# calad0i/da4ml

Measured on AMD Instinct MI355X. Metric: CMVM solves/sec, 256x256 int8 matrix, higher is better.
Workload: dtype u32; 1 GPU; c3_256x256_int8_batch64_single_chain; matrix=256x256 int8 (default_rng(seed).integers(-128,128)), batch_per_gpu=64, parallelism=1 x independent-instance shard, no data-path collective

## Files before the change

da4ml_amd/_binary/__init__.py:

```python

from __future__ import annotations

import ctypes as C
from pathlib import Path
from types import SimpleNamespace

import numpy as np

from .._marshal import pipeline_from_stages, stage_from_arrays

import os as _os

_LIB_PATH = Path(_os.environ['DA4ML_HIP_LIB']).resolve() if _os.environ.get('DA4ML_HIP_LIB') else Path(__file__).resolve().parent.parent / 'libda4ml_hip.so'
_lib = None

_f32p = np.ctypeslib.ndpointer(np.float32, flags='C_CONTIGUOUS')
_i64p = np.ctypeslib.ndpointer(np.int64, flags='C_CONTIGUOUS')
_i32p = np.ctypeslib.ndpointer(np.int32, flags='C_CONTIGUOUS')

EXPORTS = (
    'da_last_error da_last_error_code da_version da_device_count da_set_device da_get_lsb_loc da_iceil_log2 da_cost_add da_int_arr_to_csd '
    'da_csd_decompose da_kernel_decompose da_solve da_solve_batch da_solve_sharded da_rccl_unique_id da_rccl_shutdown da_solve_sharded_rccl da_comm_abort da_shard_exchanged_elements da_n_stages da_picked da_stage_info da_stage_copy '
    'da_result_stats da_free da_timings da_engine_stats da_dais_run da_dais_last_error da_dais_run_on'
).split()
# ... 60 lines not shown
        L.da_shard_exchanged_elements.restype = C.c_int64
        L.da_shard_exchanged_elements.argtypes = []
    L.da_solve_sharded_rccl.restype = C.c_void_p
    L.da_solve_sharded_rccl.argtypes = [_f32p, C.c_int64, C.c_int64, C.c_char_p, C.c_char_p, C.c_int, C.c_int, C.c_void_p, C.c_void_p, C.c_int, C.c_int, C.c_int,
                                        C.c_int, C.c_int, C.c_char_p, _i64p]
    L.da_timings.argtypes = [np.ctypeslib.ndpointer(np.float64, flags='C_CONTIGUOUS'), C.c_int]
    L.da_engine_stats.argtypes = [np.ctypeslib.ndpointer(np.float64, flags='C_CONTIGUOUS'), C.c_int]
    _lib = L
    return L


def _raise(rc: int):
    msg = lib().da_last_error().decode()
    if rc == -2:
        raise ValueError(msg)
    raise RuntimeError(msg)


def _kernel(kernel) -> np.ndarray:
    if not isinstance(kernel, np.ndarray) or kernel.dtype != np.float32:
        raise TypeError('kernel must be a numpy.ndarray of dtype float32 (no implicit conversion)')
    return np.ascontiguousarray(kernel)


def device_count() -> int:
    return int(lib().da_device_count())


def set_device(device: int) -> None:
    if lib().da_set_device(int(device)) != 0:
        _raise(-1)


def get_lsb_loc(x: float) -> int:
    return int(lib().da_get_lsb_loc(float(x)))


def iceil_log2(x: float) -> int:
    return int(lib().da_iceil_log2(float(x)))


def cost_add(q0, q1, shift: int, sub: bool, adder_size: int, carry_size: int) -> tuple[float, float]:
    out = np.zeros(2, np.float32)
    lib().da_cost_add(np.asarray(q0, np.float32), np.asarray(q1, np.float32), int(shift), int(bool(sub)), int(adder_size), int(carry_size), out)
    return float(out[0]), float(out[1])


def int_arr_to_csd(inp) -> np.ndarray:
    if not isinstance(inp, np.ndarray) or inp.dtype != np.int32:
        raise TypeError('inp must be a numpy.ndarray of dtype int32 (no implicit conversion)')
    x = np.ascontiguousarray(inp)
    N = lib().da_int_arr_to_csd(x.ravel(), x.size, None)
    if N < 0:
        _raise(N)
    out = np.zeros(x.shape + (N,), np.int8)
    rc = lib().da_int_arr_to_csd(x.ravel(), x.size, out.ctypes.data)
    if rc < 0:
        _raise(rc)
    return out


def csd_decompose(inp, center: bool = True):
    k = _kernel(inp)
    if k.ndim != 2:
        raise RuntimeError('csd_decompose only supports 2D arrays.')
    n_in, n_out = k.shape
    N = lib().da_csd_decompose(k, n_in, n_out, int(center), None, None, None)
    if N < 0:
        _raise(N)
    csd = np.zeros((n_in, n_out, N), np.int8)
    s0, s1 = np.zeros(n_in, np.int8), np.zeros(n_out, np.int8)
    rc = lib().da_csd_decompose(k, n_in, n_out, int(center), csd.ctypes.data, s0.ctypes.data, s1.ctypes.data)
    if rc < 0:
        _raise(rc)
    return csd, s0, s1


def kernel_decompose(kernel, dc: int = -2):
    k = _kernel(kernel)
    if k.ndim != 2:
        raise RuntimeError('csd_decompose only supports 2D arrays.')
    n_in, n_out = k.shape
    m0, m1 = np.zeros((n_in, n_out), np.float32), np.zeros((n_out, n_out), np.float32)
    rc = lib().da_kernel_decompose(k, n_in, n_out, int(dc), m0, m1)
    if rc < 0:
        _raise(rc)
    return m0, m1


def _collect(h, with_stats=False):
    L = lib()
    try:
        stages = []
        for s in range(L.da_n_stages(h)):
            info = np.zeros(5, np.int64)
            L.da_stage_info(h, s, info)
            n_in, n_out, n_ops, carry, adder = (int(v) for v in info)
            arr = [np.zeros(n, np.int64) for n in (n_in, n_out, n_out, n_out)]
            oi, of = np.zeros((n_ops, 4), np.int64), np.zeros((n_ops, 5), np.float32)
            L.da_stage_copy(h, s, *arr, oi, of)
            stages.append(stage_from_arrays(n_in, n_out, *arr, oi, of, carry, adder))
        pipe = pipeline_from_stages(stages)
        if not with_stats:
            return pipe
        st = np.zeros(8, np.int64)
        L.da_result_stats(h, st)
        names = ('iterations', 'digits0', 'blocks0', 'select_rounds', 'table_peak', 'scan_slots', 'partners', 'matches')
        return pipe, dict(zip(names, st.tolist()), picked=int(L.da_picked(h)))
    finally:
        L.da_free(h)


def _opt_arrays(qintervals, latencies, n_in):
    q = l = None
    if qintervals is not None:
        q = np.ascontiguousarray(np.asarray([tuple(float(v) for v in t) for t in qintervals], np.float32).reshape(n_in, 3))
    if latencies is not None:
        l = np.ascontiguousarray(np.asarray([float(v) for v in latencies], np.float32).reshape(n_in))
    return q, l


def solve(
    kernel,
    method0: str = 'wmc',
    method1: str = 'auto',
    hard_dc: int = -1,
    decompose_dc: int = -2,
    qintervals=None,
    latencies=None,
    adder_size: int = -1,
    carry_size: int = -1,
    search_all_decompose_dc: bool = True,
    _stats: bool = False,
):
    k = _kernel(kernel)
    if k.ndim != 2:
        raise RuntimeError('csd_decompose only supports 2D arrays.')
    n_in, n_out = k.shape
    q, l = _opt_arrays(qintervals, latencies, n_in)
    h = lib().da_solve(k, n_in, n_out, method0.encode(), method1.encode(), int(hard_dc), int(decompose_dc),
                       None if q is None else q.ctypes.data, None if l is None else l.ctypes.data,
                       int(adder_size), int(carry_size), int(bool(search_all_decompose_dc)))
    if not h:
        _raise(lib().da_last_error_code())
    return _collect(h, _stats)


def solve_sharded(kernel, method0: str = 'wmc', method1: str = 'auto', hard_dc: int = -1, decompose_dc: int = -2, qintervals=None, latencies=None,
                  adder_size: int = -1, carry_size: int = -1, search_all_decompose_dc: bool = True, rank: int = 0, world: int = 1, allreduce=None):
    k = _kernel(kernel)
    if k.ndim != 2:
        raise RuntimeError('csd_decompose only supports 2D arrays.')
    n_in, n_out = k.shape
    q, l = _opt_arrays(qintervals, latencies, n_in)
    st = np.zeros(3, np.int64)
    h = lib().da_solve_sharded(k, n_in, n_out, method0.encode(), method1.encode(), int(hard_dc), int(decompose_dc),
                               None if q is None else q.ctypes.data, None if l is None else l.ctypes.data, int(adder_size), int(carry_size),
                               int(bool(search_all_decompose_dc)), int(rank), int(world), C.cast(allreduce, C.c_void_p) if allreduce is not None else None, None, st)
    if not h:
        _raise(lib().da_last_error_code())
    return _collect(h), dict(zip(('sharded_chains', 'greedy_steps', 'allreduce_calls'), st.tolist()))


def rccl_unique_id() -> bytes:
    buf = C.create_string_buffer(128)
    rc = lib().da_rccl_unique_id(buf)
    if rc != 0:
        _raise(rc)
    return buf.raw


def rccl_shutdown() -> int:
    n = lib().da_rccl_shutdown()
    if n < 0:
        _raise(1)
    return n


def solve_sharded_rccl(kernel, unique_id: bytes, method0: str = 'wmc', method1: str = 'auto', hard_dc: int = -1, decompose_dc: int = -2, qintervals=None,
                       latencies=None, adder_size: int = -1, carry_size: int = -1, search_all_decompose_dc: bool = True, rank: int = 0, world: int = 1):
    k = _kernel(kernel)
    if k.ndim != 2:
        raise RuntimeError('csd_decompose only supports 2D arrays.')
    if len(unique_id) != 128:
        raise ValueError('unique_id must be the 128 bytes of rccl_unique_id()')
    n_in, n_out = k.shape
    q, l = _opt_arrays(qintervals, latencies, n_in)
    st = np.zeros(3, np.int64)
    h = lib().da_solve_sharded_rccl(k, n_in, n_out, method0.encode(), method1.encode(), int(hard_dc), int(decompose_dc),
                                    None if q is None else q.ctypes.data, None if l is None else l.ctypes.data, int(adder_size), int(carry_size),
                                    int(bool(search_all_decompose_dc)), int(rank), int(world), unique_id, st)
    if not h:
        _raise(lib().da_last_error_code())
    return _collect(h), dict(zip(('sharded_chains', 'greedy_steps', 'allreduce_calls'), st.tolist()))


def shard_exchanged_elements() -> int:
    return int(lib().da_shard_exchanged_elements())


def comm_abort():
    lib().da_comm_abort()


def solve_many(
    kernels,
    method0: str = 'wmc',
    method1: str = 'auto',
    hard_dc: int = -1,
    decompose_dc: int = -2,
    qintervals=None,
    latencies=None,
    adder_size: int = -1,
    carry_size: int = -1,
    search_all_decompose_dc: bool = True,
    _stats: bool = False,
):
    ks = [_kernel(k) for k in kernels]
    n = len(ks)
    if n == 0:
        return []
    n_in = np.array([k.shape[0] for k in ks], np.int64)
    n_out = np.array([k.shape[1] for k in ks], np.int64)
    kptr = (C.c_void_p * n)(*[k.ctypes.data for k in ks])
    keep, qptr, lptr = [], None, None
    if qintervals is not None or latencies is not None:
        qs, ls = [], []
        for i in range(n):
            q, l = _opt_arrays(None if qintervals is None else qintervals[i], None if latencies is None else latencies[i], int(n_in[i]))
            keep += [q, l]
            qs.append(None if q is None else q.ctypes.data)
            ls.append(None if l is None else l.ctypes.data)
        qptr, lptr = (C.c_void_p * n)(*qs), (C.c_void_p * n)(*ls)
    res = (C.c_void_p * n)()
    rc = lib().da_solve_batch(n, kptr, n_in, n_out, method0.encode(), method1.encode(), int(hard_dc), int(decompose_dc), qptr, lptr,
                              int(adder_size), int(carry_size), int(bool(search_all_decompose_dc)), res)
    if rc != 0:
        _raise(rc)
    return [_collect(res[i], _stats) for i in range(n)]


class RawBatch:

    def __init__(self, handles):
        self.handles = list(handles)

    def __len__(self):
        return len(self.handles)

    def summary(self, i: int) -> dict:
        L, h = lib(), self.handles[i]
        cost, adders, n_ops = 0.0, 0, []
        for s in range(L.da_n_stages(h)):
            info = np.zeros(5, np.int64)
            L.da_stage_info(h, s, info)
            n_in, n_out, n = int(info[0]), int(info[1]), int(info[2])
            arr = [np.zeros(k, np.int64) for k in (n_in, n_out, n_out, n_out)]
            oi, of = np.zeros((n, 4), np.int64), np.zeros((n, 5), np.float32)
            L.da_stage_copy(h, s, *arr, oi, of)
            cost += float(of[:, 4].astype(np.float64).sum())
            adders += int(np.isin(oi[:, 2], (0, 1)).sum())
            n_ops.append(n)
        st = np.zeros(8, np.int64)
        L.da_result_stats(h, st)
        return dict(cost=cost, adders=adders, n_ops=n_ops, iterations=int(st[0]))

    def pipeline(self, i: int):
        h, self.handles[i] = self.handles[i], None
        return _collect(h)

    def free(self):
        for h in self.handles:
            if h:
                lib().da_free(h)
        self.handles = []


def solve_many_raw(kernels, method0='wmc', method1='auto', hard_dc=-1, decompose_dc=-2, adder_size=-1, carry_size=-1,
                   search_all_decompose_dc=True) -> RawBatch:
    ks = [_kernel(k) for k in kernels]
    n = len(ks)
    n_in = np.array([k.shape[0] for k in ks], np.int64)
    n_out = np.array([k.shape[1] for k in ks], np.int64)
    kptr = (C.c_void_p * n)(*[k.ctypes.data for k in ks])
    res = (C.c_void_p * n)()
    rc = lib().da_solve_batch(n, kptr, n_in, n_out, method0.encode(), method1.encode(), int(hard_dc), int(decompose_dc), None, None,
                              int(adder_size), int(carry_size), int(bool(search_all_decompose_dc)), res)
    if rc != 0:
        _raise(rc)
    return RawBatch([res[i] for i in range(n)])


def timings(reset: bool = False) -> dict:
    t = np.zeros(32, np.float64)
    e = np.zeros(16, np.float64)
    lib().da_engine_stats(e, 16)
    rc = lib().da_timings(t, int(reset))
    if rc != 0:
        _raise(rc)
    names = ('loop_ms', 'dist_ms', 'total_ms', 'lockstep_iters', 'iterations', 'rescans', 'partners', 'chains', 'table_bytes', 'arena_bytes',
             'select_ms_sampled', 'update_ms_sampled', 'samples', 'found', 'inserts', 'cell_reads', 'block_bytes', 'cell_bytes',
             'sel_load_bounds', 'sel_argmax', 'sel_newrow', 'sel_substitute', 'sel_prefix', 'sel_claims', 'sel_special',
             'upd_fetch', 'upd_probe', 'upd_cells', 'upd_blocks', 'upd_create', 'retries', 'sampled_chain_launches')
    extra = ('select_bytes', 'host_launch_ms', 'fast_steps', 'search_bounds', 'search_argmax', 'search_excluded', 'search_steps_timed', 'search_stale_rereads', 'search_touch_rereads', 'search_rounds', 'search_long_lists', 'search_longest_list', 'search_full_passes', 'search_list_entries')
    return {**dict(zip(names, t.tolist())), **dict(zip(extra, e.tolist()))}


_DAIS_EXECUTORS = {'host': 0, 'cpu': 0, 'device': 1, 'gpu': 1, 'host-scalar': 2}


def dais_interp_run(bin_logic, data, n_threads: int = 1, executor: str = 'host'):
    prog = np.ascontiguousarray(np.ravel(bin_logic), dtype=np.int32)
    if prog.size < 4:
        raise RuntimeError('Invalid binary logic data')
    n_in, n_out = int(prog[2]), int(prog[3])
    x = np.ascontiguousarray(np.ravel(data), dtype=np.float64)
    assert n_in > 0 and x.size % n_in == 0, f'Input size {x.size} is not divisible by {n_in}'
    n_samples = x.size // n_in
    out = np.zeros((n_samples, max(n_out, 0)), dtype=np.float64)
    L = lib()
    L.da_dais_run_on.argtypes = [C.c_void_p, C.c_int64, C.c_void_p, C.c_int64, C.c_void_p, C.c_int, C.c_int]
    L.da_dais_last_error.restype = C.c_char_p
    if executor not in _DAIS_EXECUTORS:
        raise ValueError(f'unknown DAIS executor {executor!r} (one of {sorted(_DAIS_EXECUTORS)})')
    if L.da_dais_run_on(prog.ctypes.data, prog.size, x.ctypes.data, n_samples, out.ctypes.data, int(n_threads), _DAIS_EXECUTORS[executor]) != 0:
        raise RuntimeError(L.da_dais_last_error().decode())
    return out


cmvm_bin = SimpleNamespace(
    solve=solve, kernel_decompose=kernel_decompose, csd_decompose=csd_decompose, int_arr_to_csd=int_arr_to_csd,
    get_lsb_loc=get_lsb_loc, iceil_log2=iceil_log2, cost_add=cost_add,
)

__all__ = ['dais_interp_run', 'int_arr_to_csd', 'csd_decompose', 'get_lsb_loc', 'kernel_decompose', 'solve', 'iceil_log2', 'solve_many', 'cost_add']
```

da4ml_amd/csrc/cmvm_capi.cc:

```cpp

#include <cstdlib>
#include <chrono>
#include <cstdio>
#include <pthread.h>

#include <algorithm>
#include <atomic>
#include <cstring>
#include <memory>
#include <mutex>
#include <new>
#include <string>
#include <vector>

#include "../../include/da4ml_hip.h"
#include "cmvm_gpu.h"
#include "cmvm_host.h"
#include "cmvm_rccl.h"
#include "cmvm_shard.h"

namespace {

thread_local std::string g_err;
thread_local int g_err_code = DA_OK;
// ... 67 lines not shown
    }
}

}

struct da_result {
    da::PipeResult pipe;
    da::ChainStats stats;
};

extern "C" {

const char *da_last_error(void) { return g_err.c_str(); }
int da_last_error_code(void) { return g_err_code; }
const char *da_version(void) { return "da4ml_hip 0.1 (gfx950)"; }
int da_device_count(void) { return da::gpu::device_count(); }
int da_set_device(int device) {
    std::lock_guard<LibraryMutex> lk(g_mutex);
    if (device < 0 || device >= da::gpu::device_count()) {
        g_err = "invalid device index " + std::to_string(device);
        return g_err_code = DA_ERR_NO_DEVICE;
    }
    g_device = device;
    return DA_OK;
}

int da_get_lsb_loc(float x) { return da::lsb_loc(x); }
int da_iceil_log2(float x) { return da::iceil_log2(x); }
int da_cost_add(const float *q0, const float *q1, int64_t shift, int sub, int adder_size, int carry_size, float *out2) {
    da::cost_add(da::QInt{q0[0], q0[1], q0[2]}, da::QInt{q1[0], q1[1], q1[2]}, shift, sub != 0, adder_size, carry_size, out2[0], out2[1]);
    return DA_OK;
}

int da_int_arr_to_csd(const int32_t *x, int64_t n, int8_t *out) {
    std::lock_guard<LibraryMutex> lk(g_mutex);
    try {
        std::vector<int8_t> csd;
        int N = backend().int_to_csd(x, n, csd);
        if (out) std::memcpy(out, csd.data(), csd.size());
        return N;
    } catch (const std::exception &e) {
        return fail(e);
    }
}

int da_csd_decompose(const float *kernel, int64_t n_in, int64_t n_out, int center, int8_t *csd, int8_t *shift0, int8_t *shift1) {
    std::lock_guard<LibraryMutex> lk(g_mutex);
    try {
        std::vector<int8_t> c, a, b;
        int N = backend().csd_decompose(kernel, (int)n_in, (int)n_out, center != 0, c, a, b);
        if (csd) std::memcpy(csd, c.data(), c.size());
        if (shift0) std::memcpy(shift0, a.data(), a.size());
        if (shift1) std::memcpy(shift1, b.data(), b.size());
        return N;
    } catch (const std::exception &e) {
        return fail(e);
    }
}

int da_kernel_decompose(const float *kernel, int64_t n_in, int64_t n_out, int dc, float *m0, float *m1) {
    std::lock_guard<LibraryMutex> lk(g_mutex);
    try {
        std::vector<float> a, b;
        da::kernel_decompose(backend(), kernel, (int)n_in, (int)n_out, dc, a, b);
        std::memcpy(m0, a.data(), a.size() * 4);
        std::memcpy(m1, b.data(), b.size() * 4);
        return DA_OK;
    } catch (const std::exception &e) {
        return fail(e);
    }
}

int da_solve_batch(int count, const float *const *kernels, const int64_t *n_in, const int64_t *n_out, const char *method0,
                   const char *method1, int hard_dc, int decompose_dc, const float *const *qintervals,
                   const float *const *latencies, int adder_size, int carry_size, int search_all_decompose_dc,
                   da_result **results) {
    std::lock_guard<LibraryMutex> lk(g_mutex);
    try {
        std::vector<da::Problem> probs((size_t)count);
        for (int i = 0; i < count; ++i) {
            da::Problem &p = probs[i];
            p.kernel = kernels[i];
            p.n_in = (int)n_in[i];
            p.n_out = (int)n_out[i];
            if (p.n_in <= 0 || p.n_out <= 0) throw std::invalid_argument("kernel must be a non-empty 2-D matrix");
            p.opt.method0 = method0;
            p.opt.method1 = method1;
            p.opt.hard_dc = hard_dc;
            p.opt.decompose_dc = decompose_dc;
            const float *q = qintervals ? qintervals[i] : nullptr;
            const float *l = latencies ? latencies[i] : nullptr;
            check_dyadic_steps(q, p.n_in);
            if (q)
                for (int r = 0; r < p.n_in; ++r) p.opt.qints.push_back(da::QInt{q[3 * r], q[3 * r + 1], q[3 * r + 2]});
            if (l) p.opt.lats.assign(l, l + p.n_in);
            p.opt.adder_size = adder_size;
            p.opt.carry_size = carry_size;
            p.opt.search_all = search_all_decompose_dc != 0;
        }
        std::vector<da::ChainStats> stats;
        const auto t0 = std::chrono::steady_clock::now();
        std::vector<da::PipeResult> res = da::solve_batch(backend(), probs, &stats);
        for (int i = 0; i < count; ++i) results[i] = new da_result{std::move(res[i]), i < (int)stats.size() ? stats[i] : da::ChainStats{}};
        if (std::getenv("DA4ML_HIP_VERBOSE"))
            std::fprintf(stderr, "[da4ml_hip] da_solve_batch(%d): %.2f ms\n", count, std::chrono::duration<double, std::milli>(std::chrono::steady_clock::now() - t0).count());
        return DA_OK;
    } catch (const std::exception &e) {
        return fail(e);
    }
}

da_result *da_solve(const float *kernel, int64_t n_in, int64_t n_out, const char *method0, const char *method1, int hard_dc,
                    int decompose_dc, const float *qintervals, const float *latencies, int adder_size, int carry_size,
                    int search_all_decompose_dc) {
    da_result *r = nullptr;
    const float *q[1] = {qintervals}, *l[1] = {latencies};
    int rc = da_solve_batch(1, &kernel, &n_in, &n_out, method0, method1, hard_dc, decompose_dc, qintervals ? q : nullptr,
                            latencies ? l : nullptr, adder_size, carry_size, search_all_decompose_dc, &r);
    return rc == DA_OK ? r : nullptr;
}

static std::atomic<int> g_comm_aborted{0};
void da_comm_abort(void) { g_comm_aborted.store(1); }
static std::atomic<long long> g_shard_elements{0};
int64_t da_shard_exchanged_elements(void) { return (int64_t)g_shard_elements.load(); }

static std::unique_ptr<da::ShardEngine> make_hip_shard(const da::ChainJob &job, int c0, int c1, double capacity_scale, void *ctx) {
    return static_cast<da::gpu::HipBackend *>(ctx)->make_shard_engine(job, c0, c1, capacity_scale);
}

static da_result *solve_sharded_impl(const float *kernel, int64_t n_in, int64_t n_out, const char *method0, const char *method1, int hard_dc,
                                     int decompose_dc, const float *qintervals, const float *latencies, int adder_size, int carry_size,
                                     int search_all_decompose_dc, int rank, int world, da_allreduce_i32 allreduce, void *ctx, int64_t *stats3,
                                     bool stream_ordered);

static void rccl_allreduce_cb(void *ctx, void *buf, int64_t count, int on_device) {
    if (!static_cast<da::gpu::RcclTransport *>(ctx)->allreduce(buf, count, on_device != 0)) g_comm_aborted.store(1);
}

int da_rccl_unique_id(void *id128) {
    try {
        if (!id128) throw std::invalid_argument("id128 must point to 128 bytes");
        da::gpu::rccl_unique_id(id128);
        return DA_OK;
    } catch (const std::exception &e) {
        return fail(e);
    }
}

int da_rccl_shutdown(void) {
    std::lock_guard<LibraryMutex> lk(g_mutex);
    try {
        return da::gpu::rccl_shutdown();
    } catch (const std::exception &e) {
        fail(e);
        return -1;
    }
}

da_result *da_solve_sharded_rccl(const float *kernel, int64_t n_in, int64_t n_out, const char *method0, const char *method1, int hard_dc,
                                 int decompose_dc, const float *qintervals, const float *latencies, int adder_size, int carry_size,
                                 int search_all_decompose_dc, int rank, int world, const void *id128, int64_t *stats3) {
    std::shared_ptr<da::gpu::RcclTransport> tr;
    {
        std::lock_guard<LibraryMutex> lk(g_mutex);
        try {
            if (world < 1 || rank < 0 || rank >= world) throw std::invalid_argument("rank must be in [0, world)");
            if (!id128) throw std::invalid_argument("id128 (the 128-byte RCCL unique id of rank 0) must be given");
            da::gpu::HipBackend &inner = backend();
            tr = da::gpu::RcclTransport::open(id128, rank, world, g_device, inner.stream());
        } catch (const std::exception &e) {
            fail(e);
            return nullptr;
        }
    }
    da_result *r = solve_sharded_impl(kernel, n_in, n_out, method0, method1, hard_dc, decompose_dc, qintervals, latencies, adder_size, carry_size,
                                      search_all_decompose_dc, rank, world, rccl_allreduce_cb, tr.get(), stats3, true);
    if (!r && tr->last_error()[0]) g_err += std::string(" [") + tr->last_error() + "]";
    return r;
}

static da_result *solve_sharded_impl(const float *kernel, int64_t n_in, int64_t n_out, const char *method0, const char *method1, int hard_dc,
                                     int decompose_dc, const float *qintervals, const float *latencies, int adder_size, int carry_size,
                                     int search_all_decompose_dc, int rank, int world, da_allreduce_i32 allreduce, void *ctx, int64_t *stats3,
                                     bool stream_ordered) {
    std::lock_guard<LibraryMutex> lk(g_mutex);
    try {
        if (world < 1 || rank < 0 || rank >= world) throw std::invalid_argument("rank must be in [0, world)");
        if (world > 255) throw std::invalid_argument("at most 255 ranks (8-bit flag fields)");
        if (world > 1 && !allreduce) throw std::invalid_argument("an all-reduce callback must be given for world > 1");
        if (n_in <= 0 || n_out <= 0) throw std::invalid_argument("kernel must be a non-empty 2-D matrix");
        da::Problem p;
        p.kernel = kernel;
        p.n_in = (int)n_in;
        p.n_out = (int)n_out;
        p.opt.method0 = method0;
        p.opt.method1 = method1;
        p.opt.hard_dc = hard_dc;
        p.opt.decompose_dc = decompose_dc;
        check_dyadic_steps(qintervals, p.n_in);
        if (qintervals)
            for (int r = 0; r < p.n_in; ++r) p.opt.qints.push_back(da::QInt{qintervals[3 * r], qintervals[3 * r + 1], qintervals[3 * r + 2]});
        if (latencies) p.opt.lats.assign(latencies, latencies + p.n_in);
        p.opt.adder_size = adder_size;
        p.opt.carry_size = carry_size;
        p.opt.search_all = search_all_decompose_dc != 0;
        da::gpu::HipBackend &inner = backend();
        da::ShardComm comm;
        comm.rank = rank;
        comm.world = world;
        comm.allreduce = allreduce;
        comm.ctx = ctx;
        g_comm_aborted.store(0);
        comm.aborted = &g_comm_aborted;
        comm.stream_ordered = stream_ordered || std::getenv("DA4ML_SHARD_STREAM_ORDERED") != nullptr;
        da::ShardedBackend be(inner, comm, make_hip_shard, &inner);
        be.force_single = std::getenv("DA4ML_SHARD_FORCE") != nullptr;
        be.force_comm(std::getenv("DA4ML_SHARD_FORCE_COMM") != nullptr);
        std::vector<da::ChainStats> stats;
        std::vector<da::PipeResult> res = da::solve_batch(be, {p}, &stats);
        if (stats3) {
            stats3[0] = be.sharded_chains;
            stats3[1] = be.sharded_steps;
            stats3[2] = be.comm().calls;
        }
        g_shard_elements.store(be.comm().elements);
        return new da_result{std::move(res[0]), stats.empty() ? da::ChainStats{} : stats[0]};
    } catch (const std::exception &e) {
        fail(e);
        return nullptr;
    }
}

da_result *da_solve_sharded(const float *kernel, int64_t n_in, int64_t n_out, const char *method0, const char *method1, int hard_dc,
                            int decompose_dc, const float *qintervals, const float *latencies, int adder_size, int carry_size,
                            int search_all_decompose_dc, int rank, int world, da_allreduce_i32 allreduce, void *ctx, int64_t *stats3) {
    return solve_sharded_impl(kernel, n_in, n_out, method0, method1, hard_dc, decompose_dc, qintervals, latencies, adder_size, carry_size,
                              search_all_decompose_dc, rank, world, allreduce, ctx, stats3, false);
}

int da_n_stages(const da_result *r) { return (int)r->pipe.stages.size(); }
int da_picked(const da_result *r) { return r->pipe.picked; }
int da_stage_info(const da_result *r, int stage, int64_t *info) {
    const da::StageResult &s = r->pipe.stages[stage];
    info[0] = s.n_in;
    info[1] = s.n_out;
    info[2] = (int64_t)s.ops.size();
    info[3] = s.carry_size;
    info[4] = s.adder_size;
    return DA_OK;
}
int da_stage_copy(const da_result *r, int stage, int64_t *inp_shifts, int64_t *out_idxs, int64_t *out_shifts, int64_t *out_negs,
                  int64_t *ops_i, float *ops_f) {
    const da::StageResult &s = r->pipe.stages[stage];
    std::memcpy(inp_shifts, s.inp_shifts.data(), s.inp_shifts.size() * 8);
    std::memcpy(out_idxs, s.out_idxs.data(), s.out_idxs.size() * 8);
    std::memcpy(out_shifts, s.out_shifts.data(), s.out_shifts.size() * 8);
    std::memcpy(out_negs, s.out_negs.data(), s.out_negs.size() * 8);
    for (size_t k = 0; k < s.ops.size(); ++k) {
        const da::OpRec &o = s.ops[k];
        int64_t *oi = ops_i + 4 * k;
        float *of = ops_f + 5 * k;
        oi[0] = o.id0, oi[1] = o.id1, oi[2] = o.opcode, oi[3] = o.data;
        of[0] = o.q.lo, of[1] = o.q.hi, of[2] = o.q.step, of[3] = o.latency, of[4] = o.cost;
    }
    return DA_OK;
}
int da_result_stats(const da_result *r, int64_t *s) {
    const da::ChainStats &t = r->stats;
    int64_t v[8] = {t.iterations, t.digits0, t.blocks0, t.rebuilds, t.table_peak, t.scan_slots, t.partners, t.matches};
    std::memcpy(s, v, sizeof v);
    return DA_OK;
}
void da_free(da_result *r) {
    if (!r) return;
    for (da::StageResult &st : r->pipe.stages) da::recycle_op_list(std::move(st.ops));
    delete r;
}

int da_timings(double *t, int reset) {
    std::lock_guard<LibraryMutex> lk(g_mutex);
    try {
        da::gpu::HipBackend &be = backend();
        const da::gpu::GpuTimings &g = be.timings();
        double v[32] = {g.loop_ms,          g.dist_ms,         g.total_ms,         (double)g.lockstep_iters, (double)g.iterations,
                        (double)g.rescans, (double)g.partners, (double)g.chains, g.table_bytes,            g.arena_bytes,
                        g.select_ms_sampled, g.update_ms_sampled, (double)g.samples, (double)g.found, (double)g.inserts,
                        (double)g.cell_reads, g.key_bytes, g.cell_bytes};
        for (int q = 0; q < 12; ++q) v[18 + q] = g.phase_cycles[q];
        v[30] = (double)g.retries;
        v[31] = g.sampled_chain_launches;
        std::memcpy(t, v, sizeof v);
        if (reset) be.reset_timings();
        return DA_OK;
    } catch (const std::exception &e) {
        return fail(e);
    }
}

int da_engine_stats(double *out, int n) {
    std::lock_guard<LibraryMutex> lk(g_mutex);
    try {
        const da::gpu::GpuTimings &g = backend().timings();
        const double v[16] = {g.select_bytes, g.host_launch_ms, (double)g.fast_steps, g.search_cycles[0], g.search_cycles[1], g.search_cycles[2], g.search_cycles[3], g.search_diag[0], g.search_diag[1], g.search_diag[2], g.search_diag[3], g.search_diag[4], g.search_diag[5], g.search_diag[6], 0.0, 0.0};
        const int m = n < 16 ? (n < 0 ? 0 : n) : 16;
        for (int i = 0; i < m; ++i) out[i] = v[i];
        return m;
    } catch (const std::exception &e) {
        fail(e);
        return 0;
    }
}

}
```

da4ml_amd/csrc/cmvm_engine.hip:

```cpp

#include <hip/hip_runtime.h>

#include <algorithm>
#include <atomic>
#include <chrono>
#include <cmath>
#include <cstdio>
#include <cstdlib>
#include <cstring>
#include <memory>
#include <mutex>
#include <numeric>
#include <stdexcept>
#include <string>
#include <thread>
#include <vector>

#include "cmvm_core.h"
#include "cmvm_geometry.h"
#include "cmvm_gpu.h"
#include "cmvm_host.h"

namespace da {
namespace gpu {

#define HIP_CHECK(expr)                                                                                          \
    do {                                                                                                         \
        hipError_t _e = (expr);                                                                                  \
        if (_e != hipSuccess)                                                                                    \
            throw std::runtime_error(std::string("HIP error: ") + hipGetErrorString(_e) + " at " #expr);         \
    } while (0)

constexpr uint64_t KEY_EMPTY = ~0ull;
constexpr uint64_t KEY_TOMB = ~0ull - 1;
constexpr uint64_t KEY_TOMB_LO = KEY_TOMB - 3;
constexpr int WAVE = 64;
constexpr int UPD_THREADS = 256;
constexpr int UPD_WAVES = UPD_THREADS / WAVE;
#ifndef DA_MAX_GROUPS
#define DA_MAX_GROUPS 2048
#endif
constexpr int MAX_GROUPS = DA_MAX_GROUPS;
#ifndef DA_IDS_LDS
#define DA_IDS_LDS 2048
#endif

#ifdef DA_PHASE_TIMERS
#define UPD_TIMER_DECL long long up[5] = {0, 0, 0, 0, 0}, u0 = clock64(), u1;
#define UPD_TIMER_MARK(i) \
    u1 = clock64();       \
    up[i] += u1 - u0;     \
    u0 = u1;
#ifndef DA_TIMER_STEP_LO
#define DA_TIMER_STEP_LO 0
#endif
#ifndef DA_TIMER_STEP_HI
#define DA_TIMER_STEP_HI 0x7FFFFFFF
#endif
#define DA_TIMED_STEP(t) ((t) >= DA_TIMER_STEP_LO && (t) < DA_TIMER_STEP_HI)
#define UPD_TIMER_FLUSH \
    if (lane == 0 && DA_TIMED_STEP(g->iter - 1))      \
        for (int q = 0; q < 5; ++q) atomicAdd(&g->st_phase[7 + q], (unsigned long long)up[q]);
#define SEL_TIMER_DECL long long tp[8];
#define SEL_TIMER_MARK(i) tp[i] = clock64();
#define SEL_TIMER_FLUSH \
    if (DA_TIMED_STEP(iter)) for (int q = 0; q < 7; ++q) g->st_phase[q] += (unsigned long long)(tp[q + 1] - tp[q]);
#define UPD_TIMER_PASS_END UPD_TIMER_MARK(4)
#elif defined(DA_UPD_TAIL)
#ifndef DA_TIMER_STEP_LO
#define DA_TIMER_STEP_LO 0
#endif
#ifndef DA_TIMER_STEP_HI
#define DA_TIMER_STEP_HI 0x7FFFFFFF
#endif
#define DA_TIMED_STEP(t) ((t) >= DA_TIMER_STEP_LO && (t) < DA_TIMER_STEP_HI)
#define UPD_TIMER_DECL long long up[9] = {0, 0, 0, 0, 0, 0, 0, 0, 0}, u0 = clock64(), u1;
#define UPD_TIMER_MARK(i)
#define UPD_TIMER_PASS_END                                                        \
    {                                                                             \
        u1 = clock64();                                                           \
        const long long dt = u1 - u0;                                             \
        const bool cr = __ballot(gnew) != 0;                                      \
        up[0] += dt, up[1] += 1;                                                  \
        if (rare) up[2] += dt, up[3] += 1, up[8] += __popcll(rare);               \
        if (!rare && cr) up[4] += 1, up[5] += dt;                                 \
        up[6] += dt > 20000, up[7] += dt > 40000;                                 \
        u0 = clock64();                                                           \
    }
#define UPD_TIMER_FLUSH                                                           \
    if (lane == 0 && DA_TIMED_STEP(g->iter - 1)) {                                \
        for (int q = 0; q < 5; ++q) atomicAdd(&g->st_phase[7 + q], (unsigned long long)up[q]); \
        atomicAdd(&g->st_qdiag[0], (unsigned long long)up[5]);                    \
        atomicAdd(&g->st_qdiag[1], (unsigned long long)up[6]);                    \
        atomicAdd(&g->st_qdiag[4], (unsigned long long)up[7]);                    \
        atomicAdd(&g->st_qdiag[5], (unsigned long long)up[8]);                    \
    }
#define SEL_TIMER_DECL
#define SEL_TIMER_MARK(i)
#define SEL_TIMER_FLUSH
#else
#define UPD_TIMER_DECL
#define UPD_TIMER_MARK(i)
#define UPD_TIMER_PASS_END
#define UPD_TIMER_FLUSH
#define SEL_TIMER_DECL
#define SEL_TIMER_MARK(i)
#define SEL_TIMER_FLUSH
#endif

#ifdef DA_STEP_CLOCKS
#define CLK_NOW() ((unsigned long long)__builtin_amdgcn_s_memrealtime())
#define CLK_MARK(g, par, slot, inverted) atomicMax(&(g)->clk[par][slot], (inverted) ? ~CLK_NOW() : CLK_NOW())
#ifndef DA_CLK_STEP_LO
#define DA_CLK_STEP_LO 0
#endif
#ifndef DA_CLK_STEP_HI
#define DA_CLK_STEP_HI 0x7FFFFFFF
#endif
#define CLK_TIMED_STEP(t) ((t) >= DA_CLK_STEP_LO && (t) < DA_CLK_STEP_HI)
#else
#define CLK_MARK(g, par, slot, inverted)
#endif

struct BlkHdr {
    int ov;
    float dl;
    uint32_t rank;
    uint32_t idx;
};

#define DA_GLOBAL __attribute__((address_space(1)))
template <class T> __device__ __forceinline__ T *gen(DA_GLOBAL T *p) { return (T *)p; }
template <class T> __device__ __forceinline__ T da_uniform(T v) {
    static_assert(sizeof(T) == 4 || sizeof(T) == 8, "pinned descriptor fields are 32- or 64-bit values");
    if constexpr (sizeof(T) == 4) {
        const int r = __builtin_amdgcn_readfirstlane(__builtin_bit_cast(int, v));
        return __builtin_bit_cast(T, r);
    } else {
        const unsigned long long u = __builtin_bit_cast(unsigned long long, v);
        const unsigned int lo = (unsigned int)__builtin_amdgcn_readfirstlane((int)(unsigned int)u), hi = (unsigned int)__builtin_amdgcn_readfirstlane((int)(unsigned int)(u >> 32));
        return __builtin_bit_cast(T, ((unsigned long long)hi << 32) | lo);
    }
}
#define DA_PIN_ASM(x) do { x = da_uniform(x); asm volatile("" : "+s"(x)); } while (0)
template <class T> __device__ __forceinline__ void pin_one(T &v) { DA_PIN_ASM(v); }
template <class... T> __device__ __forceinline__ void pin_sgpr(T &...v) { (pin_one(v), ...); }
#define DA_PIN_VASM(x) asm volatile("" : "+v"(x))
template <class T> __device__ __forceinline__ void pin_vone(T &v) { DA_PIN_VASM(v); }
template <class... T> __device__ __forceinline__ void pin_vgpr(T &...v) { (pin_vone(v), ...); }
__device__ __forceinline__ void load_fence() {
    asm volatile("" ::: "memory");
    __builtin_amdgcn_sched_barrier(0);
}
__host__ __device__ __forceinline__ size_t align16(size_t v) { return (v + 15) & ~(size_t)15; }
typedef float da_f4 __attribute__((ext_vector_type(4)));
typedef int da_i4 __attribute__((ext_vector_type(4)));
typedef unsigned int da_u2 __attribute__((ext_vector_type(2)));
typedef unsigned long long da_ul2 __attribute__((ext_vector_type(2)));
__device__ __forceinline__ RowInfo load_row(const DA_GLOBAL RowInfo *rows, size_t i) {
    const da_f4 v = *reinterpret_cast<const DA_GLOBAL da_f4 *>(rows + i);
    return RowInfo{v.x, v.y, v.z, v.w};
}
__device__ __forceinline__ RowInfo pick_row(bool first, const RowInfo &a, const RowInfo &b) {
    return RowInfo{first ? a.lo : b.lo, first ? a.hi : b.hi, first ? a.step : b.step, first ? a.lat : b.lat};
}
__device__ __forceinline__ void store_row(DA_GLOBAL RowInfo *rows, size_t i, const RowInfo &r) {
    *reinterpret_cast<DA_GLOBAL da_f4 *>(rows + i) = da_f4{r.lo, r.hi, r.step, r.lat};
}

template <class Cell> struct RowFmt;
template <> struct RowFmt<uint32_t> {
    using Entry = uint32_t;
    static __device__ __forceinline__ Entry pack(uint32_t col, uint32_t cell) { return (col << 24) | ((cell >> 16) << 12) | (cell & 0xFFFu); }
    static __device__ __forceinline__ uint32_t col(Entry e) { return e >> 24; }
    static __device__ __forceinline__ uint32_t cell(Entry e) { return (((e >> 12) & 0xFFFu) << 16) | (e & 0xFFFu); }
    static __device__ __forceinline__ Entry none() { return 0u; }
};
template <> struct RowFmt<uint64_t> {
    using Entry = da_ul2;
    static __device__ __forceinline__ Entry pack(uint32_t col, uint64_t cell) { return Entry{(unsigned long long)cell, (unsigned long long)col}; }
    static __device__ __forceinline__ uint32_t col(Entry e) { return (uint32_t)e.y; }
    static __device__ __forceinline__ uint64_t cell(Entry e) { return (uint64_t)e.x; }
    static __device__ __forceinline__ Entry none() { return Entry{0ull, 0ull}; }
};
constexpr int REF_ROW_BITS = 24, REF_LEN_BITS = 12, REF_OFF_BITS = 28;
__host__ __device__ __forceinline__ unsigned long long ref_pack(uint32_t row, uint32_t len, uint32_t off) {
    return (unsigned long long)row | ((unsigned long long)len << REF_ROW_BITS) | ((unsigned long long)off << (REF_ROW_BITS + REF_LEN_BITS));
}
__device__ __forceinline__ uint32_t ref_row(unsigned long long r) { return (uint32_t)r & ((1u << REF_ROW_BITS) - 1u); }
__device__ __forceinline__ uint32_t ref_len(unsigned long long r) { return (uint32_t)(r >> REF_ROW_BITS) & ((1u << REF_LEN_BITS) - 1u); }
__device__ __forceinline__ uint32_t ref_off(unsigned long long r) { return (uint32_t)(r >> (REF_ROW_BITS + REF_LEN_BITS)); }

struct SpecPick {
    unsigned long long word;
    unsigned long long tie;
    da_u2 refA, refB;
    RowInfo ra, rb;
};
static_assert(sizeof(SpecPick) == 64, "SpecPick is read as sixteen words");
struct CandEntry {
    unsigned long long rank, tie;
};
#ifndef DA_CAND_CAP
#define DA_CAND_CAP 16
#endif
constexpr int CAND_CAP = DA_CAND_CAP, TOUCH_CAP = DA_CAND_CAP;

struct alignas(32) GroupRec {
    unsigned long long ub;
    unsigned long long glow;
    unsigned long long gtie;
    uint32_t dirty;
    uint32_t pad;
};
static_assert(sizeof(GroupRec) == 32, "group record");
struct ChainDev {
    int n_in, n_out, n_bits, K, Kpad, method, adder_size, carry_size;
    int rcap, lcap, gs_log2, n_groups;
    uint32_t C, cmask;
    const float *kernel;
    const float *qints;
    const float *lats;
    int32_t *xint;
    int8_t *shift0, *shift1;
    void *rlist;
    da_u2 *rowoff;
    uint32_t rl_cap, rl_used;
    RowInfo *rows;
    uint32_t *stamp;
    unsigned long long *collist;
    int *collen;
    unsigned long long *hkey;
    uint32_t *hrank;
    unsigned char *hblk;
    int pb_log2;
    GroupRec *grec;
    int *mcol;
    uint16_t *cmap;
    uint32_t *colbits;
    int cb_words;
    uint32_t *pl_ids;
    void *mA, *mB;
    unsigned long long *plist;
    int m, n_partners;
    int claim_words;
    uint32_t A, B, Nw;
    int pk_shift, pk_sub;
    int n_rows, iter, done, error, unknown_hit;
    unsigned int n_live, n_used, live_peak;
    int4 *picks;
    int prep_nbits, prep_maxdcol;
    long long prep_digits, prep_pairs;
    uint32_t *fin_row;
    unsigned long long *fin_cell;
    uint32_t *fin_count;
    uint32_t *fin_start;
    uint32_t *pk_row;
    unsigned long long *pk_cell;
    float *pk_lat;
    int pk_cap;
    uint32_t pk_total;
    int pn_out, col0;
    int32_t *cs_init;
    int32_t *cs_flags;
    uint32_t *cs_uni;
    int cs_nuni;
    int32_t *cs_slab;
    unsigned long long st_rescans, st_partners, st_matches, st_found, st_inserts, st_cells;
    const uint32_t *step_mant;
    const float *step_tab;
    int n_step_mant;
    unsigned long long st_sel_bytes;
    unsigned long long st_phase[12];
    SpecPick spec[2];
    unsigned int c_n[2], l_n[2];
    CandEntry c_list[2][CAND_CAP];
    CandEntry l_list[2][TOUCH_CAP];
    uint32_t *sp_cnt;
    unsigned long long st_fast;
    unsigned long long st_qphase[4];
#ifdef DA_STEP_CLOCKS
    unsigned long long clk[2][4];
#endif
    unsigned long long st_qdiag[9];
};

__constant__ Log2Table c_log2;

__device__ __forceinline__ int lane_id() { return threadIdx.x & (WAVE - 1); }
__device__ __forceinline__ int wave_id() { return threadIdx.x / WAVE; }

template <int CTRL, int ROW_MASK> __device__ __forceinline__ uint32_t dpp_u32(uint32_t identity, uint32_t v) {
    return (uint32_t)__builtin_amdgcn_update_dpp((int)identity, (int)v, CTRL, ROW_MASK, 0xF, false);
}
constexpr int DPP_ROW_SHR1 = 0x111, DPP_ROW_SHR2 = 0x112, DPP_ROW_SHR4 = 0x114, DPP_ROW_SHR8 = 0x118, DPP_ROW_BCAST15 = 0x142, DPP_ROW_BCAST31 = 0x143;
#define DA_DPP_REDUCE32(v, ident, OP)                                   \
    v = OP(v, dpp_u32<DPP_ROW_SHR1, 0xF>(ident, v));                    \
    v = OP(v, dpp_u32<DPP_ROW_SHR2, 0xF>(ident, v));                    \
    v = OP(v, dpp_u32<DPP_ROW_SHR4, 0xF>(ident, v));                    \
    v = OP(v, dpp_u32<DPP_ROW_SHR8, 0xF>(ident, v));                    \
    v = OP(v, dpp_u32<DPP_ROW_BCAST15, 0xA>(ident, v));                 \
    v = OP(v, dpp_u32<DPP_ROW_BCAST31, 0xC>(ident, v));
__device__ __forceinline__ uint32_t uadd32(uint32_t a, uint32_t b) { return a + b; }
__device__ __forceinline__ uint32_t wave_scan_add_u32(uint32_t v) {
    DA_DPP_REDUCE32(v, 0u, uadd32)
    return v;
}
__device__ __forceinline__ uint32_t umax32(uint32_t a, uint32_t b) { return a > b ? a : b; }
__device__ __forceinline__ uint32_t smin32(uint32_t a, uint32_t b) { return (int)a < (int)b ? a : b; }
__device__ __forceinline__ int wave_min_i32(int v) {
    uint32_t x = (uint32_t)v;
    DA_DPP_REDUCE32(x, 0x7FFFFFFFu, smin32)
// ... 1823 lines not shown
        else
            for_pairs_part<Cell>(mb, x, B < r, nb, [&](int k) { atomicAdd(&dB[k], 1u); });
        for_pairs_cross<Cell>(x, ma, nb, [&](int k) { atomicAdd(&cN[k], 1u); });
    }
    lds_fence();
    int32_t *out = g->cs_slab + (size_t)(6 + 3 * u) * K;
    for (int k = lane; k < K; k += WAVE) {
        out[k] = (int32_t)dA[k];
        out[K + k] = (int32_t)dB[k];
        out[2 * K + k] = (int32_t)cN[k];
    }
}

template <class Cell> __global__ void __launch_bounds__(256) k_cs_apply(ChainDev *g) {
    Ctx c = make_ctx(g, 2 * g->iter - 1);
    c.rword = g->spec[(g->iter - 1) & 1].word;
    c.cn = &g->c_n[(g->iter - 1) & 1];
    c.cl = &g->c_list[(g->iter - 1) & 1][0];
    const int K = c.K;
    const int w = (int)blockIdx.x * 4 + wave_id();
    const uint32_t A = g->A, B = g->B, Nw = g->Nw;
    const bool same = A == B;
    if (w == 5 && c.rword) {
        const int nl = (int)g->l_n[(g->iter - 1) & 1];
        const CandEntry *ll = &g->l_list[(g->iter - 1) & 1][0];
        if (lane_id() == 0)
            for (int e = 0; e < nl; ++e) {
                const unsigned long long tw = ll[e].tie;
                const uint32_t i0 = (uint32_t)((tw >> 7) & 0xFFFFFFu), i1 = (uint32_t)(tw >> 31);
                const uint32_t r = (i0 == A || i0 == B) ? i1 : i0;
                if (((g->cs_flags[r >> 2] >> (8 * (r & 3))) & 0xFF) == 0) fold_entry(c, (uint32_t)ll[e].rank, tw);
            }
    }
    if (w < 6) {
        uint32_t lo = A, hi = A;
        bool active = true, existed = false;
        switch (w) {
        case 0: lo = A, hi = A, existed = true; break;
        case 1: lo = A, hi = B, existed = true, active = !same; break;
        case 2: lo = B, hi = B, existed = true, active = !same; break;
        case 3: lo = A, hi = Nw; break;
        case 4: lo = B, hi = Nw, active = !same; break;
        default: lo = Nw, hi = Nw; break;
        }
        if (!active) return;
        const int32_t *cnt = g->cs_slab + (size_t)w * K;
        const unsigned long long key = pack_pair(lo, hi);
        const int slot = existed ? table_find(c, key, hash_pair(lo, hi)) : -1;
        if (slot >= 0)
            table_update(c, slot, key, [&](int k, uint32_t) { return (uint32_t)cnt[k]; });
        else {
            int f = 0;
            for (int k = lane_id(); k < K; k += WAVE) f |= cnt[k] >= 2;
            if (__any(f)) table_insert(c, lo, hi, load_row(c.rows, lo), load_row(c.rows, hi), [&](int k) { return (uint32_t)cnt[k]; });
        }
        return;
    }
    const int u = w - 6;
    if (u >= g->cs_nuni) return;
    const uint32_t r = g->cs_uni[u];
    const int32_t *dA = g->cs_slab + (size_t)(6 + 3 * u) * K, *dB = dA + K, *cN = dB + K;
    {
        const uint32_t lo = min(A, r), hi = max(A, r);
        const int slot = table_find(c, pack_pair(lo, hi), hash_pair(lo, hi));
        if (slot >= 0) table_update(c, slot, pack_pair(lo, hi), [&](int k, uint32_t old) { return old - (uint32_t)dA[k]; });
    }
    if (!same) {
        const uint32_t lo = min(B, r), hi = max(B, r);
        const int slot = table_find(c, pack_pair(lo, hi), hash_pair(lo, hi));
        if (slot >= 0) table_update(c, slot, pack_pair(lo, hi), [&](int k, uint32_t old) { return old - (uint32_t)dB[k]; });
    }
    int f = 0;
    for (int k = lane_id(); k < K; k += WAVE) f |= cN[k] >= 2;
    if (__any(f)) table_insert(c, r, Nw, load_row(c.rows, r), load_row(c.rows, Nw), [&](int k) { return (uint32_t)cN[k]; });
    if (lane_id() == 0) atomicAdd(&g->st_partners, 1ull);
}

template <class Cell> __global__ void __launch_bounds__(256) k_extract(ChainDev *chains) {
    using O = CellOps<Cell>;
    using F = RowFmt<Cell>;
    ChainDev &ch = chains[blockIdx.y];
    int j = blockIdx.x * (blockDim.x / WAVE) + wave_id();
    if (j >= ch.n_out) return;
    const auto *rl = reinterpret_cast<const typename F::Entry *>(ch.rlist);
    int lane = lane_id(), len = ch.collen[j], out = 0;
    for (int base = 0; base < len; base += WAVE) {
        int e = base + lane;
        Cell c = 0;
        uint32_t r = 0;
        if (e < len) {
            const unsigned long long ref = ch.collist[(size_t)j * ch.lcap + e];
            r = ref_row(ref);
            const auto *row = rl + ref_off(ref);
            if ((int)r < ch.n_in)
                c = F::cell(row[j]);
            else {
                int lo = 0, hi = (int)ref_len(ref) - 1;
                while (lo < hi) {
                    int mid = (lo + hi) >> 1;
                    if (F::col(row[mid]) < (uint32_t)j)
                        lo = mid + 1;
                    else
                        hi = mid;
                }
                const auto en = row[lo];
                c = F::col(en) == (uint32_t)j ? F::cell(en) : (Cell)0;
            }
        }
        unsigned long long nz = __ballot(c != 0);
        if (c != 0) {
            size_t at = (size_t)j * ch.lcap + out + __popcll(nz & ((1ull << lane) - 1));
            ch.fin_row[at] = r;
            ch.fin_cell[at] = (unsigned long long)O::plus(c) | ((unsigned long long)O::minus(c) << 32);
        }
        out += __popcll(nz);
    }
    if (lane == 0) ch.fin_count[j] = (uint32_t)out;
}

__global__ void __launch_bounds__(256) k_pack(ChainDev *chains) {
    ChainDev &ch = chains[blockIdx.x];
    __shared__ uint32_t s_total;
    const int n_out = ch.n_out, tid = threadIdx.x, lane = lane_id(), nw = blockDim.x / WAVE;
    if (tid < WAVE) {
        uint32_t run = 0;
        for (int base = 0; base < n_out; base += WAVE) {
            int j = base + lane;
            uint32_t v = j < n_out ? ch.fin_count[j] : 0u, inc = v;
            for (int o = 1; o < WAVE; o <<= 1) {
                uint32_t t = (uint32_t)__shfl_up((int)inc, o);
                if (lane >= o) inc += t;
            }
            if (j < n_out) ch.fin_start[j] = run + inc - v;
            run += (uint32_t)__shfl((int)inc, WAVE - 1);
        }
        if (lane == 0) {
            ch.fin_start[n_out] = run;
            ch.pk_total = run;
            s_total = run;
        }
    }
    __syncthreads();
    if (s_total > (uint32_t)ch.pk_cap) {
        if (tid == 0) ch.error = E_LIST_CAPACITY;
        return;
    }
    for (int j = wave_id(); j < n_out; j += nw) {
        const uint32_t cnt = ch.fin_count[j], dst = ch.fin_start[j];
        const size_t src = (size_t)j * ch.lcap;
        for (uint32_t e = lane; e < cnt; e += WAVE) {
            ch.pk_row[dst + e] = ch.fin_row[src + e];
            ch.pk_cell[dst + e] = ch.fin_cell[src + e];
        }
    }
    for (int r = tid; r < ch.n_rows; r += blockDim.x) ch.pk_lat[r] = ch.rows[r].lat;
}

struct GatherPiece {
    const void *src;
    unsigned long long dst_off, bytes;
};
__global__ void __launch_bounds__(256) k_gather(const GatherPiece *pieces, unsigned char *dst) {
    const GatherPiece pc = pieces[blockIdx.y];
    const size_t t0 = (size_t)blockIdx.x * blockDim.x + threadIdx.x, stride = (size_t)gridDim.x * blockDim.x;
    const size_t n16 = (size_t)pc.bytes / 16;
    const da_i4 *s16 = reinterpret_cast<const da_i4 *>(pc.src);
    da_i4 *d16 = reinterpret_cast<da_i4 *>(dst + pc.dst_off);
    for (size_t i = t0; i < n16; i += stride) d16[i] = s16[i];
    const unsigned char *s1 = reinterpret_cast<const unsigned char *>(pc.src);
    unsigned char *d1 = dst + pc.dst_off;
    for (size_t i = n16 * 16 + t0; i < (size_t)pc.bytes; i += stride) d1[i] = s1[i];
}

__global__ void __launch_bounds__(256) k_col_dist(const int32_t *aug, int n_in, int W, long long *d0, long long *d1) {
    __shared__ int32_t sa[64][17], sb[64][17];
    int ta = threadIdx.y, tb = threadIdx.x;
    int a = blockIdx.y * 16 + ta, b = blockIdx.x * 16 + tb;
    int tid = ta * 16 + tb;
    long long acc0 = 0, acc1 = 0;
    for (int base = 0; base < n_in; base += 64) {
        for (int q = tid; q < 64 * 16; q += 256) {
            int i = base + q / 16, c = q % 16;
            int ca = blockIdx.y * 16 + c, cb = blockIdx.x * 16 + c;
            sa[q / 16][c] = (i < n_in && ca < W) ? aug[(size_t)i * W + ca] : 0;
            sb[q / 16][c] = (i < n_in && cb < W) ? aug[(size_t)i * W + cb] : 0;
        }
        __syncthreads();
        int rows = min(64, n_in - base);
        for (int i = 0; i < rows; ++i) {
            int32_t x = sa[i][ta], y = sb[i][tb];
            acc0 += naf_weight(x - y);
            acc1 += naf_weight(x + y);
        }
        __syncthreads();
    }
    if (a < W && b < W) {
        d0[(size_t)a * W + b] = acc0;
        d1[(size_t)a * W + b] = acc1;
    }
}

__global__ void __launch_bounds__(256) k_naf_digits(const int32_t *x, long long n, int N, int8_t *out) {
    long long i = (long long)blockIdx.x * blockDim.x + threadIdx.x;
    if (i >= n) return;
    uint32_t p, m;
    naf_masks(x[i], p, m);
    for (int b = 0; b < N; ++b) out[i * N + b] = (int8_t)(((p >> b) & 1) - ((m >> b) & 1));
}
__global__ void __launch_bounds__(256) k_absmax(const int32_t *x, long long n, unsigned int *out) {
    unsigned int mx = 0;
    for (long long i = (long long)blockIdx.x * blockDim.x + threadIdx.x; i < n; i += (long long)gridDim.x * blockDim.x) {
        int32_t v = x[i];
        mx = max(mx, (unsigned int)(v < 0 ? -v : v));
    }
    mx = wave_max_u32(mx);
    if (lane_id() == 0) atomicMax(out, mx);
}


namespace {

struct DeviceBuffer {
    void *ptr = nullptr;
    size_t cap = 0;
    void *get(size_t bytes) {
        if (bytes > cap) {
            if (ptr) (void)hipFree(ptr);
            ptr = nullptr;
            cap = 0;
            size_t want = bytes + bytes / 8;
            HIP_CHECK(hipMalloc(&ptr, want));
            cap = want;
        }
        return ptr;
    }
    ~DeviceBuffer() {
        if (ptr) (void)hipFree(ptr);
    }
};

inline size_t align_up(size_t v, size_t a) { return (v + a - 1) / a * a; }

inline void spin_wait_step(unsigned &polls) {
    if (++polls < 4096u) {
#if defined(__x86_64__) || defined(__i386__)
        __builtin_ia32_pause();
#elif defined(__aarch64__)
        asm volatile("yield");
#endif
    } else if (polls < 8192u)
        std::this_thread::yield();
    else
        std::this_thread::sleep_for(std::chrono::microseconds(50));
}

struct EventGuard {
    std::vector<hipEvent_t> all;
    hipEvent_t make(unsigned flags = 0) {
        hipEvent_t e = nullptr;
        HIP_CHECK(flags ? hipEventCreateWithFlags(&e, flags) : hipEventCreate(&e));
        all.push_back(e);
        return e;
    }
    ~EventGuard() {
        for (hipEvent_t e : all) (void)hipEventDestroy(e);
    }
};

struct Carver {
    unsigned char *base;
    size_t off = 0;
    explicit Carver(unsigned char *b) : base(b) {}
    template <class T> T *take(size_t count) {
        off = align_up(off, 256);
        T *p = base ? reinterpret_cast<T *>(base + off) : nullptr;
        off += count * sizeof(T);
        return p;
    }
};

}

struct PinnedBuffer {
    void *ptr = nullptr;
    size_t cap = 0;
    void *get(size_t bytes) {
        if (bytes > cap) {
            if (ptr) (void)hipHostFree(ptr);
            ptr = nullptr;
            cap = 0;
            size_t want = bytes + bytes / 4 + 4096;
            HIP_CHECK(hipHostMalloc(&ptr, want, hipHostMallocDefault));
            cap = want;
        }
        return ptr;
    }
    ~PinnedBuffer() {
        if (ptr) (void)hipHostFree(ptr);
    }
};

struct HipBackend::Impl {
    int device = 0;
    PinnedBuffer pinned, pinned_up;
    hipStream_t stream = nullptr;
    static constexpr int MAX_LANES = 8;
    hipStream_t lanes[MAX_LANES] = {nullptr, nullptr, nullptr, nullptr, nullptr, nullptr, nullptr, nullptr};
    int launch_threads = 2;
    int n_lanes = 4;
    int upd_total_blocks = 2560;
    DeviceBuffer arena, desc_buf, io_buf, gather_buf, piece_buf;
    unsigned int *d_done = nullptr;
    unsigned int *h_done = nullptr;
    hipStream_t poll_stream = nullptr;
    GpuTimings timings;
    double table_scale = 1.0;
};

HipBackend::HipBackend(int device) : impl_(new Impl) {
    impl_->device = device;
    HIP_CHECK(hipSetDevice(device));
    HIP_CHECK(hipStreamCreateWithFlags(&impl_->stream, hipStreamNonBlocking));
    impl_->lanes[0] = impl_->stream;
    for (int l = 1; l < Impl::MAX_LANES; ++l) HIP_CHECK(hipStreamCreateWithFlags(&impl_->lanes[l], hipStreamNonBlocking));
    if (const char *e = std::getenv("DA4ML_HIP_TABLE_SCALE")) impl_->table_scale = std::max(1e-4, std::atof(e));
    if (const char *e = std::getenv("DA4ML_HIP_ROW_SCALE")) row_scale_ = std::max(1e-4, std::atof(e));
    if (const char *e = std::getenv("DA4ML_HIP_UPD_BLOCKS")) impl_->upd_total_blocks = std::max(2, std::atoi(e));
    if (const char *e = std::getenv("DA4ML_HIP_LAUNCH_THREADS")) impl_->launch_threads = std::max(1, std::atoi(e));
    if (const char *e = std::getenv("DA4ML_HIP_LANES")) impl_->n_lanes = std::max(1, std::min((int)Impl::MAX_LANES, std::atoi(e)));
    HIP_CHECK(hipMalloc(&impl_->d_done, sizeof(unsigned int)));
    HIP_CHECK(hipHostMalloc(&impl_->h_done, 2 * sizeof(unsigned int), hipHostMallocDefault));
    HIP_CHECK(hipStreamCreateWithFlags(&impl_->poll_stream, hipStreamNonBlocking));
    Log2Table t = measure_log2_table();
    HIP_CHECK(hipMemcpyToSymbol(HIP_SYMBOL(c_log2), &t, sizeof t));
}
HipBackend::~HipBackend() {
    (void)hipSetDevice(impl_->device);
    if (impl_->d_done) (void)hipFree(impl_->d_done);
    if (impl_->h_done) (void)hipHostFree(impl_->h_done);
    if (impl_->poll_stream) (void)hipStreamDestroy(impl_->poll_stream);
    if (impl_->stream) (void)hipStreamDestroy(impl_->stream);
    for (int l = 1; l < Impl::MAX_LANES; ++l)
        if (impl_->lanes[l]) (void)hipStreamDestroy(impl_->lanes[l]);
}
const GpuTimings &HipBackend::timings() const { return impl_->timings; }
void HipBackend::reset_timings() { impl_->timings = GpuTimings{}; }
void *HipBackend::stream() const { return impl_->stream; }

namespace {

struct Geometry {
    bool wide;
    int n_mant = 0;
    int n_bits, K, Kpad, rcap, lcap, gs_log2, n_groups, pk_cap, pb_log2;
    uint32_t C, rl_cap;
};

size_t sel2_fixed_lds(const ChainJob &job, const Geometry &g) {
    const size_t no = (size_t)job.n_out, entb = g.wide ? 16 : 4;
    return no * entb + 6 * (size_t)g.Kpad * 4 + (5 * no + 1) * 4;
}
size_t sel2_lds_budget(int device, bool wide) {
    static std::mutex mu;
    static size_t cached[2] = {0, 0};
    std::lock_guard<std::mutex> lk(mu);
    if (!cached[wide]) {
        hipFuncAttributes fa;
        const void *fn = wide ? reinterpret_cast<const void *>(&k_iter_select2<uint64_t>) : reinterpret_cast<const void *>(&k_iter_select2<uint32_t>);
        HIP_CHECK(hipFuncGetAttributes(&fa, fn));
        int limit = 0;
        HIP_CHECK(hipDeviceGetAttribute(&limit, hipDeviceAttributeMaxSharedMemoryPerBlock, device));
        if (limit < 64 * 1024) limit = 64 * 1024;
        const size_t used = fa.sharedSizeBytes + 256;
        cached[wide] = (size_t)limit > used ? (size_t)limit - used : 1;
    }
    return cached[wide];
}
int claim_words_for(const ChainJob &job, const Geometry &g, size_t budget) {
    const size_t words = ((size_t)g.rcap + 31) / 32, fixed = align_up(sel2_fixed_lds(job, g), 16);
    return words * 4 <= 64 * 1024 && fixed + words * 4 + 16 <= budget ? (int)words : 0;
}

size_t carve_chain(unsigned char *base, const ChainJob &job, const Geometry &g, ChainDev &d) {
    Carver c(base);
    size_t cell = g.wide ? 8 : 4, entry = g.wide ? 16 : 4;
    size_t n_out = job.n_out;
    d.rlist = c.take<unsigned char>((size_t)g.rl_cap * entry);
    d.rowoff = c.take<da_u2>(g.rcap);
    d.rows = c.take<RowInfo>(g.rcap);
    d.stamp = c.take<uint32_t>(g.rcap);
    d.collist = c.take<unsigned long long>(n_out * (size_t)g.lcap);
    d.collen = c.take<int>(n_out);
    d.hkey = c.take<unsigned long long>(g.C);
    d.hrank = c.take<uint32_t>((size_t)g.C + ((size_t)g.C + 3) / 4);
    d.hblk = c.take<unsigned char>((size_t)g.C << g.pb_log2);
    d.grec = c.take<GroupRec>(g.n_groups);
    d.mcol = c.take<int>(n_out);
    d.cmap = c.take<uint16_t>(n_out);
    d.colbits = c.take<uint32_t>(n_out * (size_t)((g.rcap + 31) / 32));
    d.pl_ids = c.take<uint32_t>(g.rcap);
    d.mA = c.take<unsigned char>(n_out * cell);
    d.mB = c.take<unsigned char>(n_out * cell);
    d.plist = c.take<unsigned long long>(g.rcap);
    d.sp_cnt = c.take<uint32_t>((size_t)6 * g.Kpad);
    d.picks = c.take<int4>(g.rcap);
    d.fin_row = c.take<uint32_t>(n_out * (size_t)g.lcap);
    d.fin_cell = c.take<unsigned long long>(n_out * (size_t)g.lcap);
    d.fin_count = c.take<uint32_t>(n_out);
    d.fin_start = c.take<uint32_t>(n_out + 1);
    d.pk_cap = g.pk_cap;
    d.pk_row = c.take<uint32_t>((size_t)g.pk_cap);
    d.pk_cell = c.take<unsigned long long>((size_t)g.pk_cap);
    d.pk_lat = c.take<float>(g.rcap);
    d.step_mant = c.take<uint32_t>((size_t)std::max(g.n_mant, 1));
    d.step_tab = c.take<float>((size_t)std::max(g.n_mant, 1) * 256);
    return align_up(c.off, 256);
}

}

void HipBackend::run_chains(const ChainJob *jobs, ChainOut *outs, int n) {
    if (n <= 0) return;
    Impl &im = *impl_;
    HIP_CHECK(hipSetDevice(im.device));
    hipStream_t st = im.stream;
    auto t_begin = std::chrono::steady_clock::now();
    const bool verbose = std::getenv("DA4ML_HIP_VERBOSE") != nullptr;
    auto lap = [&, last = t_begin](const char *what) mutable {
        auto now = std::chrono::steady_clock::now();
        if (verbose) std::fprintf(stderr, "[da4ml_hip] %-28s %8.2f ms\n", what, std::chrono::duration<double, std::milli>(now - last).count());
        last = now;
    };

    std::vector<size_t> in_off(n);
    size_t in_bytes = 0;
    for (int i = 0; i < n; ++i) {
        in_off[i] = in_bytes;
        size_t e = (size_t)jobs[i].n_in * jobs[i].n_out;
        in_bytes += align_up(e * 4, 256) + align_up((size_t)jobs[i].n_in * 12, 256) + align_up((size_t)jobs[i].n_in * 4, 256) +
                    align_up(e * 4, 256) + align_up(jobs[i].n_in, 256) + align_up(jobs[i].n_out, 256);
    }
    unsigned char *io = static_cast<unsigned char *>(im.io_buf.get(std::max<size_t>(in_bytes, 256)));
    std::vector<ChainDev> desc(n);
    unsigned char *stage_ptr = static_cast<unsigned char *>(im.pinned_up.get(std::max<size_t>(in_bytes, 256)));
    for (int i = 0; i < n; ++i) {
        const ChainJob &j = jobs[i];
        size_t e = (size_t)j.n_in * j.n_out, o = in_off[i];
        ChainDev &d = desc[i];
        std::memset(&d, 0, sizeof d);
        d.n_in = j.n_in;
        d.n_out = j.n_out;
        d.pn_out = j.n_out;
        d.method = j.method;
        d.adder_size = j.adder_size;
        d.carry_size = j.carry_size;
        d.kernel = reinterpret_cast<const float *>(io + o);
        o += align_up(e * 4, 256);
        d.qints = reinterpret_cast<const float *>(io + o);
        o += align_up((size_t)j.n_in * 12, 256);
        d.lats = reinterpret_cast<const float *>(io + o);
        o += align_up((size_t)j.n_in * 4, 256);
        d.xint = reinterpret_cast<int32_t *>(io + o);
        o += align_up(e * 4, 256);
        d.shift0 = reinterpret_cast<int8_t *>(io + o);
        o += align_up(j.n_in, 256);
        d.shift1 = reinterpret_cast<int8_t *>(io + o);
    }
    {
        auto stage = [&](int i) {
            const ChainJob &j = jobs[i];
            const size_t e = (size_t)j.n_in * j.n_out;
            size_t o = in_off[i];
            std::memcpy(stage_ptr + o, j.kernel, e * 4);
            o += align_up(e * 4, 256);
            std::memcpy(stage_ptr + o, j.qints, (size_t)j.n_in * 12);
            o += align_up((size_t)j.n_in * 12, 256);
            std::memcpy(stage_ptr + o, j.lats, (size_t)j.n_in * 4);
        };
        const int workers = (int)std::min<size_t>({(size_t)n, (size_t)8, in_bytes / (1u << 20) + 1});
        std::atomic<int> next{0};
        auto work = [&] {
            for (int i = next++; i < n; i = next++) stage(i);
        };
        std::vector<std::thread> pool;
        for (int t = 1; t < workers; ++t) pool.emplace_back(work);
        work();
        for (auto &t : pool) t.join();
    }
    HIP_CHECK(hipMemcpyAsync(io, stage_ptr, in_bytes, hipMemcpyHostToDevice, st));
    ChainDev *d_desc = static_cast<ChainDev *>(im.desc_buf.get(sizeof(ChainDev) * (size_t)n));
    HIP_CHECK(hipMemcpyAsync(d_desc, desc.data(), sizeof(ChainDev) * (size_t)n, hipMemcpyHostToDevice, st));
    int max_n_out = 0, max_n_in = 0;
    for (int i = 0; i < n; ++i) {
        max_n_out = std::max(max_n_out, jobs[i].n_out);
        max_n_in = std::max(max_n_in, jobs[i].n_in);
    }
    hipLaunchKernelGGL(k_prepare, dim3(n), dim3(256), (size_t)max_n_out * 4, st, d_desc);
    HIP_CHECK(hipGetLastError());
    HIP_CHECK(hipMemcpyAsync(desc.data(), d_desc, sizeof(ChainDev) * (size_t)n, hipMemcpyDeviceToHost, st));
    HIP_CHECK(hipStreamSynchronize(st));

    lap("upload + k_prepare");
    std::vector<StepLog2Host> step_tabs(n);
    for (int i = 0; i < n; ++i)
        if (jobs[i].adder_size >= 0 || jobs[i].carry_size >= 0) step_tabs[i].build(jobs[i].qints, jobs[i].n_in);
    std::vector<Geometry> geo(n);
    std::vector<size_t> a_off(n);
    size_t arena_bytes = 0;
    for (int i = 0; i < n; ++i) {
        const ChainDev &d = desc[i];
        Geometry &g = geo[i];
        g.n_bits = d.prep_nbits;
        if (g.n_bits > 30) throw std::runtime_error("kernel needs more than 30 CSD digits per entry (the reference overflows int32 there); unsupported");
        g.wide = g.n_bits > 12 || jobs[i].n_out > 256;
        g.n_mant = (int)step_tabs[i].mant.size();
        g.K = key_count(g.n_bits);
        g.Kpad = (g.K + 3) & ~3;
        g.pb_log2 = 5;
        while ((1 << g.pb_log2) < 16 + 2 * g.Kpad) ++g.pb_log2;
        long long D0 = d.prep_digits;
        const TableGeometry tg = table_geometry(jobs[i], d.prep_pairs, D0, im.table_scale, row_scale_, MAX_GROUPS);
        g.rcap = tg.rcap < (1 << REF_ROW_BITS) ? (int)tg.rcap : (1 << REF_ROW_BITS);
        g.lcap = jobs[i].n_in + d.prep_maxdcol + 1;
        g.pk_cap = (int)std::min<long long>(D0 + 1, (long long)1 << 30);
        const long long rl_want = (long long)jobs[i].n_in * jobs[i].n_out + D0 + jobs[i].n_out + 64;
        if (rl_want >= (1ll << REF_OFF_BITS) || g.rcap >= (1 << REF_ROW_BITS) || jobs[i].n_out >= (1 << REF_LEN_BITS))
            throw std::runtime_error("problem too large for the row-reference format (rows < 2^24, columns < 4096, list entries < 2^28)");
        g.rl_cap = (uint32_t)rl_want;
        g.C = tg.C;
        g.gs_log2 = tg.gs_log2;
        g.n_groups = tg.n_groups;
        ChainDev tmp;
        a_off[i] = arena_bytes;
        arena_bytes += carve_chain(nullptr, jobs[i], g, tmp);
    }
    {
        size_t free_b = 0, total_b = 0;
        HIP_CHECK(hipMemGetInfo(&free_b, &total_b));
        size_t budget = (size_t)(0.85 * (double)(free_b + im.arena.cap));
        if (const char *e = std::getenv("DA4ML_HIP_MEM_BUDGET_MB")) budget = (size_t)std::atoll(e) << 20;
        if (arena_bytes > budget) {
            if (n == 1)
                throw std::runtime_error("a single chain needs " + std::to_string(arena_bytes >> 20) + " MiB of device memory (pair table of " +
                                         std::to_string(geo[0].C) + " slots), " + std::to_string(free_b >> 20) + " MiB are free (budget " +
                                         std::to_string(budget >> 20) + " MiB)");
            const int half_n = n / 2;
            run_chains(jobs, outs, half_n);
            run_chains(jobs + half_n, outs + half_n, n - half_n);
            return;
        }
    }
    unsigned char *arena = static_cast<unsigned char *>(im.arena.get(arena_bytes));
    for (int i = 0; i < n; ++i) {
        ChainDev &d = desc[i];
        const Geometry &g = geo[i];
        carve_chain(arena + a_off[i], jobs[i], g, d);
        d.n_bits = g.n_bits;
        d.K = g.K;
        d.Kpad = g.Kpad;
        d.rcap = g.rcap;
        d.lcap = g.lcap;
        d.gs_log2 = g.gs_log2;
        d.n_groups = g.n_groups;
        d.C = g.C;
        d.cmask = g.C - 1;
        d.pb_log2 = g.pb_log2;
        d.rl_cap = g.rl_cap;
        d.rl_used = (uint32_t)jobs[i].n_in * (uint32_t)jobs[i].n_out;
        d.n_rows = jobs[i].n_in;
        d.claim_words = claim_words_for(jobs[i], g, sel2_lds_budget(im.device, g.wide));
        d.iter = 0;
        d.done = (jobs[i].method == M_DUMMY || jobs[i].method < 0) ? 1 : 0;
        d.cb_words = (g.rcap + 31) / 32;
    }
    for (int i = 0; i < n; ++i) {
        desc[i].n_step_mant = (int)step_tabs[i].mant.size();
        if (desc[i].n_step_mant) {
            HIP_CHECK(hipMemcpyAsync(const_cast<uint32_t *>(desc[i].step_mant), step_tabs[i].mant.data(), step_tabs[i].mant.size() * 4, hipMemcpyHostToDevice, st));
            HIP_CHECK(hipMemcpyAsync(const_cast<float *>(desc[i].step_tab), step_tabs[i].tab.data(), step_tabs[i].tab.size() * 4, hipMemcpyHostToDevice, st));
        }
    }
    HIP_CHECK(hipMemcpyAsync(d_desc, desc.data(), sizeof(ChainDev) * (size_t)n, hipMemcpyHostToDevice, st));
    HIP_CHECK(hipMemsetAsync(im.d_done, 0, sizeof(unsigned int), st));
    hipLaunchKernelGGL(k_init_state, dim3(128, n), dim3(256), 0, st, d_desc);
    HIP_CHECK(hipGetLastError());

    std::vector<int> order(n);
    std::iota(order.begin(), order.end(), 0);
    std::stable_sort(order.begin(), order.end(), [&](int a, int b) { return geo[a].wide < geo[b].wide; });
    bool permuted = false;
    for (int i = 0; i < n; ++i) permuted |= order[i] != i;
    if (permuted) {
        std::vector<ChainDev> sorted(n);
        for (int i = 0; i < n; ++i) sorted[i] = desc[order[i]];
        HIP_CHECK(hipMemcpyAsync(d_desc, sorted.data(), sizeof(ChainDev) * (size_t)n, hipMemcpyHostToDevice, st));
        HIP_CHECK(hipStreamSynchronize(st));
    }
    int n_narrow = 0;
    for (int i = 0; i < n; ++i) n_narrow += !geo[i].wide;
    struct Range {
        int first, count;
        bool wide;
    } ranges[2] = {{0, n_narrow, false}, {n_narrow, n - n_narrow, true}};
    int active = 0;
    for (int i = 0; i < n; ++i) active += desc[i].done ? 0 : 1;

    size_t sel_lds[2] = {0, 0}, upd_lds[2] = {0, 0}, pair_lds[2] = {0, 0};
    int upd_blocks[2] = {1, 1};
    long long max_pairs[2] = {0, 0};
    for (int i = 0; i < n; ++i) {
        int w = geo[i].wide;
        const size_t no = (size_t)jobs[i].n_out, cellb = geo[i].wide ? 8 : 4;
        const size_t s = align_up(sel2_fixed_lds(jobs[i], geo[i]) + (size_t)desc[i].claim_words * 4, 16);
        if (s > sel2_lds_budget(im.device, geo[i].wide))
            throw std::runtime_error("selection kernel needs " + std::to_string(s) + " bytes of dynamic LDS, the device leaves it " + std::to_string(sel2_lds_budget(im.device, geo[i].wide)) +
                                     " beside the kernel's static arrays (n_out too large)");
        sel_lds[w] = std::max(sel_lds[w], s);
        upd_lds[w] = std::max(upd_lds[w], align_up(2 * no * cellb + no * 6, 16) + align_up((size_t)UPD_WAVES * (QN * 3 + 1) * (size_t)geo[i].Kpad * 4, 16));
        pair_lds[w] = std::max(pair_lds[w], (size_t)4 * geo[i].Kpad * 4);
        max_pairs[w] = std::max(max_pairs[w], (long long)jobs[i].n_in * (jobs[i].n_in + 1) / 2);
    }
    for (int w = 0; w < 2; ++w) {
        int cnt = ranges[w].count;
        if (cnt == 0) continue;
        upd_blocks[w] = std::max(2, std::min(64, (im.upd_total_blocks + cnt - 1) / std::max(cnt, 1)));
    }
    for (int w = 0; w < 2; ++w) {
        const Range &r = ranges[w];
        if (r.count == 0) continue;
        ChainDev *base = d_desc + r.first;
        dim3 colgrid((max_n_out + 3) / 4, r.count);
        dim3 pairgrid((unsigned)((max_pairs[w] + 3) / 4), r.count);
        if (!r.wide) {
            hipLaunchKernelGGL(k_init_cells<uint32_t>, colgrid, dim3(256), 0, st, base);
            hipLaunchKernelGGL(k_init_pairs<uint32_t>, pairgrid, dim3(256), pair_lds[w], st, base);
        } else {
            hipLaunchKernelGGL(k_init_cells<uint64_t>, colgrid, dim3(256), 0, st, base);
            hipLaunchKernelGGL(k_init_pairs<uint64_t>, pairgrid, dim3(256), pair_lds[w], st, base);
        }
        HIP_CHECK(hipGetLastError());
    }
    if (ranges[0].count)
        HIP_CHECK(hipFuncSetAttribute(reinterpret_cast<const void *>(&k_iter_select2<uint32_t>), hipFuncAttributeMaxDynamicSharedMemorySize, (int)sel_lds[0]));
    if (ranges[1].count)
        HIP_CHECK(hipFuncSetAttribute(reinterpret_cast<const void *>(&k_iter_select2<uint64_t>), hipFuncAttributeMaxDynamicSharedMemorySize, (int)sel_lds[1]));

    HIP_CHECK(hipStreamSynchronize(st));
    lap("arena + init kernels");
    EventGuard events;
    hipEvent_t ev0 = events.make(), ev1 = events.make();
    HIP_CHECK(hipEventRecord(ev0, st));
    HIP_CHECK(hipStreamSynchronize(st));
    struct Group {
        int first, count, w;
        hipStream_t stream;
    };
    std::vector<Group> groups;
    for (int w = 0; w < 2; ++w) {
        const Range &r = ranges[w];
        if (r.count == 0) continue;
        int parts = std::max(1, std::min(im.n_lanes, r.count / 8));
        if (ranges[0].count && ranges[1].count) parts = std::max(1, parts / 2);
        for (int p = 0; p < parts; ++p) {
            int lo = r.first + (int)((long long)r.count * p / parts), hi = r.first + (int)((long long)r.count * (p + 1) / parts);
            groups.push_back(Group{lo, hi - lo, w, im.lanes[groups.size() % Impl::MAX_LANES]});
        }
    }
    const char *stats_env = std::getenv("DA4ML_HIP_STATS");
    const bool with_stats = stats_env && std::atoi(stats_env) != 0;
    auto launch_pair = [&](const Group &gr, hipEvent_t *se, int step) {
        ChainDev *base = d_desc + gr.first;
        const dim3 sel_grid((gr.count + 7) & ~7, 2);
        if (se) HIP_CHECK(hipEventRecord(se[0], gr.stream));
        if (gr.w == 0)
            hipLaunchKernelGGL(k_iter_select2<uint32_t>, sel_grid, dim3(SEL2_THREADS), sel_lds[0], gr.stream, base, gr.count, im.d_done, step);
        else
            hipLaunchKernelGGL(k_iter_select2<uint64_t>, sel_grid, dim3(SEL2_THREADS), sel_lds[1], gr.stream, base, gr.count, im.d_done, step);
        if (se) HIP_CHECK(hipEventRecord(se[1], gr.stream));
        const dim3 upd_grid((gr.count + 7) & ~7, upd_blocks[gr.w] + 2);
        if (gr.w == 0 && !with_stats)
            hipLaunchKernelGGL((k_iter_update<uint32_t, false>), upd_grid, dim3(UPD_THREADS), upd_lds[0], gr.stream, base, gr.count);
        else if (gr.w == 0)
            hipLaunchKernelGGL((k_iter_update<uint32_t, true>), upd_grid, dim3(UPD_THREADS), upd_lds[0], gr.stream, base, gr.count);
        else if (!with_stats)
            hipLaunchKernelGGL((k_iter_update<uint64_t, false>), upd_grid, dim3(UPD_THREADS), upd_lds[1], gr.stream, base, gr.count);
        else
            hipLaunchKernelGGL((k_iter_update<uint64_t, true>), upd_grid, dim3(UPD_THREADS), upd_lds[1], gr.stream, base, gr.count);
        if (se) HIP_CHECK(hipEventRecord(se[2], gr.stream));
    };
    constexpr int WINDOW_ITERS = 63, MAX_SAMPLES = 4096;
    std::vector<hipEvent_t> sample_ev;
    int n_samples = 0;
    long long launched_iters = 0, iter_cap = 0;
    for (int i = 0; i < n; ++i) iter_cap = std::max<long long>(iter_cap, geo[i].rcap - jobs[i].n_in + 2);
    const int poll_every = WINDOW_ITERS + 1;
    int pre_done = 0;
    for (int i = 0; i < n; ++i) pre_done += (jobs[i].method == M_DUMMY || jobs[i].method < 0) ? 1 : 0;
    hipEvent_t win_ev[2][Impl::MAX_LANES], copy_ev[2];
    for (int p = 0; p < 2; ++p) {
        copy_ev[p] = events.make(hipEventDisableTiming);
        for (size_t gi = 0; gi < groups.size(); ++gi) win_ev[p][gi] = events.make(hipEventDisableTiming);
    }
    im.h_done[0] = im.h_done[1] = 0;
    long long window = 0;
    double host_launch_ms = 0;
    struct DrainOnError {
        const std::vector<Group> &g;
        hipStream_t poll;
        bool armed = true;
        ~DrainOnError() {
            if (!armed) return;
            for (const Group &gr : g) (void)hipStreamSynchronize(gr.stream);
            (void)hipStreamSynchronize(poll);
        }
    } drain{groups, im.poll_stream};
    struct Helper {
        std::atomic<long long> seq{0}, ack{0};
        std::atomic<bool> quit{false};
        long long first_step = 0;
        int iters = 0, parity = 0;
        std::exception_ptr err;
        std::thread th;
    } helper;
    const bool two_threads = im.launch_threads >= 2 && groups.size() >= 2;
    auto mine = [&](size_t gi, int who) { return !two_threads || (int)(gi & 1) == who; };
    auto window_launches = [&](int who, long long first_step, int iters, int parity, hipEvent_t *se0) {
        for (int it = 0; it < iters; ++it)
            for (size_t gi = 0; gi < groups.size(); ++gi)
                if (mine(gi, who)) launch_pair(groups[gi], it == 0 && gi == 0 ? se0 : nullptr, (int)(first_step + it));
        HIP_CHECK(hipGetLastError());
        for (size_t gi = 0; gi < groups.size(); ++gi)
            if (mine(gi, who)) HIP_CHECK(hipEventRecord(win_ev[parity][gi], groups[gi].stream));
    };
    if (two_threads)
        helper.th = std::thread([&] {
            long long seen = 0;
            try {
                HIP_CHECK(hipSetDevice(im.device));
                while (true) {
                    long long s;
                    unsigned polls = 0;
                    while ((s = helper.seq.load(std::memory_order_acquire)) == seen && !helper.quit.load(std::memory_order_acquire)) spin_wait_step(polls);
                    if (s == seen) break;
                    seen = s;
                    if (!helper.err) window_launches(1, helper.first_step, helper.iters, helper.parity, nullptr);
                    helper.ack.store(seen, std::memory_order_release);
                }
            } catch (...) {
                helper.err = std::current_exception();
                helper.ack.store(helper.seq.load(), std::memory_order_release);
                unsigned polls = 0;
                while (!helper.quit.load(std::memory_order_acquire)) {
                    helper.ack.store(helper.seq.load(), std::memory_order_release);
                    spin_wait_step(polls);
                }
            }
        });
    struct JoinHelper {
        Helper &h;
        ~JoinHelper() {
            h.quit.store(true, std::memory_order_release);
            if (h.th.joinable()) h.th.join();
        }
    } join_helper{helper};
    while (active > 0) {
        const auto t_q0 = std::chrono::steady_clock::now();
        if (launched_iters > iter_cap + 2 * poll_every) throw std::runtime_error("greedy loop did not terminate within its row capacity (internal error)");
        const int this_window = (int)std::min<long long>(WINDOW_ITERS, (8ll << std::min<long long>(window, 8)) - 1);
        const int p = (int)(window & 1);
        if (two_threads) {
            helper.first_step = launched_iters, helper.iters = this_window + 1, helper.parity = p;
            helper.seq.fetch_add(1, std::memory_order_release);
        }
        hipEvent_t se[3];
        const bool sample = n_samples < MAX_SAMPLES;
        if (sample) {
            for (auto &e : se) {
                e = events.make();
                sample_ev.push_back(e);
            }
            ++n_samples;
        }
        window_launches(0, launched_iters, this_window + 1, p, sample ? se : nullptr);
        launched_iters += this_window + 1;
        if (two_threads) {
            const long long want = helper.seq.load(std::memory_order_relaxed);
            unsigned polls = 0;
            while (helper.ack.load(std::memory_order_acquire) != want) spin_wait_step(polls);
            if (helper.err) std::rethrow_exception(helper.err);
        }
        for (size_t gi = 0; gi < groups.size(); ++gi) HIP_CHECK(hipStreamWaitEvent(im.poll_stream, win_ev[p][gi], 0));
        HIP_CHECK(hipMemcpyAsync(&im.h_done[p], im.d_done, sizeof(unsigned int), hipMemcpyDeviceToHost, im.poll_stream));
        HIP_CHECK(hipEventRecord(copy_ev[p], im.poll_stream));
        host_launch_ms += std::chrono::duration<double, std::milli>(std::chrono::steady_clock::now() - t_q0).count();
        if (window > 0) {
            HIP_CHECK(hipEventSynchronize(copy_ev[p ^ 1]));
            active = n - pre_done - (int)im.h_done[p ^ 1];
        }
        ++window;
    }
    for (const Group &gr : groups) HIP_CHECK(hipStreamSynchronize(gr.stream));
    HIP_CHECK(hipStreamSynchronize(im.poll_stream));
    drain.armed = false;
    HIP_CHECK(hipEventRecord(ev1, st));

    lap("greedy loop");
    for (int w = 0; w < 2; ++w) {
        const Range &r = ranges[w];
        if (r.count == 0) continue;
        dim3 colgrid((max_n_out + 3) / 4, r.count);
        if (!r.wide)
            hipLaunchKernelGGL(k_extract<uint32_t>, colgrid, dim3(256), 0, st, d_desc + r.first);
        else
            hipLaunchKernelGGL(k_extract<uint64_t>, colgrid, dim3(256), 0, st, d_desc + r.first);
    }
    hipLaunchKernelGGL(k_pack, dim3(n), dim3(256), 0, st, d_desc);
    HIP_CHECK(hipGetLastError());
    std::vector<ChainDev> fin(n);
    HIP_CHECK(hipMemcpyAsync(fin.data(), d_desc, sizeof(ChainDev) * (size_t)n, hipMemcpyDeviceToHost, st));
    HIP_CHECK(hipStreamSynchronize(st));
    float loop_ms = 0;
    HIP_CHECK(hipEventElapsedTime(&loop_ms, ev0, ev1));
    for (int k = 0; k < n_samples; ++k) {
        float a = 0, b = 0;
        HIP_CHECK(hipEventElapsedTime(&a, sample_ev[3 * k], sample_ev[3 * k + 1]));
        HIP_CHECK(hipEventElapsedTime(&b, sample_ev[3 * k + 1], sample_ev[3 * k + 2]));
        im.timings.select_ms_sampled += a;
        im.timings.update_ms_sampled += b;
    }
    im.timings.samples += n_samples;
    im.timings.sampled_chain_launches += (double)n_samples * (groups.empty() ? 0 : groups[0].count);

    bool need_retry = false;
    for (int s = 0; s < n; ++s) {
        const ChainDev &d = fin[s];
        int i = order[s];
        ChainOut &o = outs[i];
        o = ChainOut{};
        o.error = d.error;
        o.unknown_method_hit = d.unknown_hit != 0;
        o.n_bits = d.n_bits;
        if (d.error == E_TABLE_CAPACITY || d.error == E_ROW_CAPACITY) need_retry = true;
    }
    if (need_retry && retry_depth_ < 4) {
        ++retry_depth_;
        im.timings.retries += 1;
        double keep_t = im.table_scale, keep_r = row_scale_;
        im.table_scale *= 4.0;
        row_scale_ *= 4.0;
        try {
            run_chains(jobs, outs, n);
        } catch (...) {
            im.table_scale = keep_t;
            row_scale_ = keep_r;
            --retry_depth_;
            throw;
        }
        im.table_scale = keep_t;
        row_scale_ = keep_r;
        --retry_depth_;
        return;
    }
    struct ResultOffsets {
        size_t st, s0, s1, pk, lat, row, cell;
        uint32_t total;
    };
    std::vector<ResultOffsets> roff(n);
    std::vector<GatherPiece> pieces;
    pieces.reserve((size_t)n * 7);
    size_t gather_bytes = 0;
    auto piece = [&](const void *src, size_t bytes) {
        const size_t at = gather_bytes;
        if (bytes) pieces.push_back(GatherPiece{src, (unsigned long long)at, (unsigned long long)bytes});
        gather_bytes += align_up(bytes, 64);
        return at;
    };
    for (int s = 0; s < n; ++s) {
        const ChainDev &d = fin[s];
        const ChainJob &j = jobs[order[s]];
        ResultOffsets &ro = roff[s];
        ro.total = d.error == E_OK ? d.pk_total : 0u;
        ro.st = piece(d.fin_start, ((size_t)j.n_out + 1) * 4);
        ro.s0 = piece(d.shift0, (size_t)j.n_in);
        ro.s1 = piece(d.shift1, (size_t)j.n_out);
        ro.pk = piece(d.picks, (size_t)d.iter * sizeof(int4));
        ro.lat = piece(d.pk_lat, (size_t)d.n_rows * 4);
        ro.row = piece(d.pk_row, (size_t)ro.total * 4);
        ro.cell = piece(d.pk_cell, (size_t)ro.total * 8);
    }
    unsigned char *pin = static_cast<unsigned char *>(im.pinned.get(std::max<size_t>(gather_bytes, 64)));
    {
        unsigned char *gbuf = static_cast<unsigned char *>(im.gather_buf.get(std::max<size_t>(gather_bytes, 64)));
        GatherPiece *d_pieces = static_cast<GatherPiece *>(im.piece_buf.get(std::max<size_t>(pieces.size(), 1) * sizeof(GatherPiece)));
        HIP_CHECK(hipMemcpyAsync(d_pieces, pieces.data(), pieces.size() * sizeof(GatherPiece), hipMemcpyHostToDevice, st));
        for (size_t first = 0; first < pieces.size(); first += 32768) {
            const unsigned cnt = (unsigned)std::min<size_t>(32768, pieces.size() - first);
            hipLaunchKernelGGL(k_gather, dim3(16, cnt), dim3(256), 0, st, d_pieces + first, gbuf);
        }
        HIP_CHECK(hipGetLastError());
        HIP_CHECK(hipMemcpyAsync(pin, gbuf, gather_bytes, hipMemcpyDeviceToHost, st));
        HIP_CHECK(hipStreamSynchronize(st));
    }
    auto unpack = [&](int s) {
        const ChainDev &d = fin[s];
        const ChainJob &j = jobs[order[s]];
        const ResultOffsets &ro = roff[s];
        ChainOut &o = outs[order[s]];
        const uint32_t *cs = reinterpret_cast<const uint32_t *>(pin + ro.st);
        o.col_start.assign(cs, cs + j.n_out + 1);
        o.shift0.assign(reinterpret_cast<const int8_t *>(pin + ro.s0), reinterpret_cast<const int8_t *>(pin + ro.s0) + j.n_in);
        o.shift1.assign(reinterpret_cast<const int8_t *>(pin + ro.s1), reinterpret_cast<const int8_t *>(pin + ro.s1) + j.n_out);
        const int32_t *pk = reinterpret_cast<const int32_t *>(pin + ro.pk);
        o.picks.assign(pk, pk + (size_t)d.iter * 4);
        const float *lat = reinterpret_cast<const float *>(pin + ro.lat);
        o.row_lat.assign(lat, lat + d.n_rows);
        const uint32_t *pr = reinterpret_cast<const uint32_t *>(pin + ro.row);
        const unsigned long long *pc = reinterpret_cast<const unsigned long long *>(pin + ro.cell);
        o.dig_row.assign(pr, pr + ro.total);
        o.dig_cell.assign(pc, pc + ro.total);
    };
    {
        const int workers = (int)std::min<size_t>({(size_t)n, (size_t)8, gather_bytes / (1u << 20) + 1});
        std::atomic<int> next{0};
        std::exception_ptr err;
        std::mutex err_mu;
        auto work = [&] {
            try {
                for (int s = next++; s < n; s = next++) unpack(s);
            } catch (...) {
                std::lock_guard<std::mutex> lk(err_mu);
                if (!err) err = std::current_exception();
            }
        };
        std::vector<std::thread> pool;
        for (int t = 1; t < workers; ++t) pool.emplace_back(work);
        work();
        for (auto &t : pool) t.join();
        if (err) std::rethrow_exception(err);
    }
    for (int s = 0; s < n; ++s) {
        const ChainDev &d = fin[s];
        const int i = order[s];
        ChainOut &o = outs[i];
        o.stats.iterations = d.iter;
        o.stats.digits0 = d.prep_digits;
        o.stats.table_peak = d.live_peak;
        o.stats.scan_slots = (long long)d.st_rescans << d.gs_log2;
        o.stats.partners = (long long)d.st_partners;
        o.stats.matches = (long long)d.st_matches;
        for (int q = 0; q < 12; ++q) im.timings.phase_cycles[q] += (double)d.st_phase[q];
        for (int q = 0; q < 4; ++q) im.timings.search_cycles[q] += (double)d.st_qphase[q];
        im.timings.search_diag[0] += (double)d.st_qdiag[0], im.timings.search_diag[1] += (double)d.st_qdiag[1], im.timings.search_diag[2] += (double)d.st_qdiag[4];
        im.timings.search_diag[3] += (double)d.st_qdiag[5], im.timings.search_diag[4] = std::max(im.timings.search_diag[4], (double)d.st_qdiag[6]), im.timings.search_diag[5] += (double)d.st_qdiag[7], im.timings.search_diag[6] += (double)d.st_qdiag[8];
        im.timings.fast_steps += (long long)d.st_fast;
        im.timings.found += (long long)d.st_found;
        im.timings.inserts += (long long)d.st_inserts;
        im.timings.cell_reads += (long long)d.st_cells;
        im.timings.key_bytes += 2.0 * d.K * (double)(d.st_found + d.st_inserts);
        im.timings.cell_bytes += (geo[i].wide ? 8.0 : 4.0) * (double)d.st_cells;
        im.timings.iterations += d.iter;
        im.timings.rescans += (long long)d.st_rescans;
        im.timings.select_bytes += (double)d.st_sel_bytes + 32.0 * (double)d.n_groups * (double)d.iter + (double)d.st_rescans * ((double)(4u << d.gs_log2) + 24.0);
        im.timings.partners += (long long)d.st_partners;
        im.timings.table_bytes += (double)d.C * (8.0 + 4.0 + (double)(1 << d.pb_log2));
    }
    lap("extract + download + unpack");
    im.timings.loop_ms += loop_ms;
    im.timings.host_launch_ms += host_launch_ms;
    im.timings.lockstep_iters += launched_iters;
    im.timings.chains += n;
    im.timings.arena_bytes = std::max(im.timings.arena_bytes, (double)arena_bytes);
    im.timings.total_ms += std::chrono::duration<double, std::milli>(std::chrono::steady_clock::now() - t_begin).count();
    (void)max_n_in;
}

namespace {

class HipShardEngine : public ShardEngine {
  public:
    HipShardEngine(hipStream_t st, int device, const ChainJob &job, int c0, int c1, double table_scale, double row_scale)
        : st_(st), device_(device), job_(job), n_loc_(c1 - c0) {
        HIP_CHECK(hipSetDevice(device_));
        const size_t e = (size_t)job.n_in * job.n_out;
        const size_t kb = align_up(e * 4, 256), qb = align_up((size_t)job.n_in * 12, 256), lb = align_up((size_t)job.n_in * 4, 256);
        io_.get(2 * kb + qb + lb + align_up(job.n_in, 256) + align_up(job.n_out, 256) + 256);
        unsigned char *io = static_cast<unsigned char *>(io_.ptr);
        std::memset(&d_, 0, sizeof d_);
        d_.n_in = job.n_in;
        d_.n_out = n_loc_;
        d_.pn_out = job.n_out;
        d_.col0 = c0;
        d_.method = job.method;
        d_.adder_size = job.adder_size;
        d_.carry_size = job.carry_size;
        d_.kernel = reinterpret_cast<const float *>(io);
        d_.qints = reinterpret_cast<const float *>(io + kb);
        d_.lats = reinterpret_cast<const float *>(io + kb + qb);
        d_.xint = reinterpret_cast<int32_t *>(io + kb + qb + lb);
        d_.shift0 = reinterpret_cast<int8_t *>(io + 2 * kb + qb + lb);
        d_.shift1 = d_.shift0 + align_up(job.n_in, 256);
        HIP_CHECK(hipMemcpyAsync(io, job.kernel, e * 4, hipMemcpyHostToDevice, st_));
        HIP_CHECK(hipMemcpyAsync(io + kb, job.qints, (size_t)job.n_in * 12, hipMemcpyHostToDevice, st_));
        HIP_CHECK(hipMemcpyAsync(io + kb + qb, job.lats, (size_t)job.n_in * 4, hipMemcpyHostToDevice, st_));
        desc_.get(sizeof(ChainDev));
        dd_ = static_cast<ChainDev *>(desc_.ptr);
        push();
        hipLaunchKernelGGL(k_prepare, dim3(1), dim3(256), (size_t)job.n_out * 4, st_, dd_);
        HIP_CHECK(hipGetLastError());
        pull();
        Geometry &g = geo_;
        g.n_bits = d_.prep_nbits;
        if (g.n_bits > 30) throw std::runtime_error("kernel needs more than 30 CSD digits per entry; unsupported");
        g.wide = g.n_bits > 12 || n_loc_ > 256;
        if (job.adder_size >= 0 || job.carry_size >= 0) step_tab_.build(job.qints, job.n_in);
        g.n_mant = (int)step_tab_.mant.size();
        g.K = key_count(g.n_bits);
        g.Kpad = (g.K + 3) & ~3;
        g.pb_log2 = 5;
        while ((1 << g.pb_log2) < 16 + 2 * g.Kpad) ++g.pb_log2;
        const long long D0 = d_.prep_digits;
        const TableGeometry tg = table_geometry(job, d_.prep_pairs, D0, table_scale, row_scale, MAX_GROUPS);
        g.rcap = tg.rcap < (1 << REF_ROW_BITS) ? (int)tg.rcap : (1 << REF_ROW_BITS);
        g.lcap = job.n_in + d_.prep_maxdcol + 1;
        g.pk_cap = (int)std::min<long long>(D0 + 1, (long long)1 << 30);
        const long long rl_want = (long long)job.n_in * n_loc_ + D0 + n_loc_ + 64;
        if (rl_want >= (1ll << REF_OFF_BITS) || g.rcap >= (1 << REF_ROW_BITS) || n_loc_ >= (1 << REF_LEN_BITS))
            throw std::runtime_error("problem too large for the row-reference format");
        g.rl_cap = (uint32_t)rl_want;
        g.C = tg.C;
        g.gs_log2 = tg.gs_log2;
        g.n_groups = tg.n_groups;
        n_pairs_ = (long long)job.n_in * (job.n_in + 1) / 2;
        ChainJob local = job;
        local.n_out = n_loc_;
        ChainDev tmp;
        const size_t chain_bytes = carve_chain(nullptr, local, g, tmp);
        const size_t init_b = align_up((size_t)n_pairs_ * g.K * 4, 256), flag_b = align_up((((size_t)g.rcap + 3) / 4 + SHARD_TRAILER) * 4 + 64, 256),
                     uni_b = align_up((size_t)g.rcap * 4, 256), slab_b = align_up((size_t)(6 + 3 * (size_t)g.rcap) * g.K * 4, 256);
        const size_t need = chain_bytes + init_b + flag_b + uni_b + slab_b;
        {
            size_t free_b = 0, total_b = 0;
            HIP_CHECK(hipMemGetInfo(&free_b, &total_b));
            if (need > free_b)
                throw std::runtime_error("a column-sharded chain needs " + std::to_string(need >> 20) + " MiB of device memory (pair table of " +
                                         std::to_string(g.C) + " slots), " + std::to_string(free_b >> 20) + " MiB are free");
        }
        arena_.get(need);
        unsigned char *a = static_cast<unsigned char *>(arena_.ptr);
        carve_chain(a, local, g, d_);
        d_.cs_init = reinterpret_cast<int32_t *>(a + chain_bytes);
        d_.cs_flags = reinterpret_cast<int32_t *>(a + chain_bytes + init_b);
        d_.cs_uni = reinterpret_cast<uint32_t *>(a + chain_bytes + init_b + flag_b);
        d_.cs_slab = reinterpret_cast<int32_t *>(a + chain_bytes + init_b + flag_b + uni_b);
        d_.n_bits = g.n_bits;
        d_.K = g.K;
        d_.Kpad = g.Kpad;
        d_.rcap = g.rcap;
        d_.lcap = g.lcap;
        d_.gs_log2 = g.gs_log2;
        d_.n_groups = g.n_groups;
        d_.C = g.C;
        d_.cmask = g.C - 1;
        d_.pb_log2 = g.pb_log2;
        d_.rl_cap = g.rl_cap;
        d_.rl_used = (uint32_t)job.n_in * (uint32_t)n_loc_;
        d_.n_rows = job.n_in;
        d_.claim_words = claim_words_for(local_job(), g, sel2_lds_budget(device_, g.wide));
        HIP_CHECK(hipMemsetAsync(d_.stamp, 0, sizeof(uint32_t) * (size_t)g.rcap, st_));
        HIP_CHECK(hipMemsetAsync(d_.hkey, 0xFF, sizeof(unsigned long long) * (size_t)g.C, st_));
        HIP_CHECK(hipMemsetAsync(d_.hrank, 0, sizeof(uint32_t) * (size_t)g.C, st_));
        HIP_CHECK(hipMemsetAsync(d_.grec, 0, sizeof(GroupRec) * (size_t)g.n_groups, st_));
        d_.cb_words = (g.rcap + 31) / 32;
        HIP_CHECK(hipMemsetAsync(d_.colbits, 0, sizeof(uint32_t) * (size_t)n_loc_ * d_.cb_words, st_));
        {
            d_.n_step_mant = (int)step_tab_.mant.size();
            if (d_.n_step_mant) {
                HIP_CHECK(hipMemcpyAsync(const_cast<uint32_t *>(d_.step_mant), step_tab_.mant.data(), step_tab_.mant.size() * 4, hipMemcpyHostToDevice, st_));
                HIP_CHECK(hipMemcpyAsync(const_cast<float *>(d_.step_tab), step_tab_.tab.data(), step_tab_.tab.size() * 4, hipMemcpyHostToDevice, st_));
            }
        }
        push();
        report_ = static_cast<volatile int *>(report_buf_.get(64));
        for (int q = 0; q < 5; ++q) report_[q] = 0;
        d_done_ = static_cast<unsigned int *>(done_buf_.get(sizeof(unsigned int)));
        HIP_CHECK(hipMemsetAsync(d_done_, 0, sizeof(unsigned int), st_));
        dim3 colgrid((n_loc_ + 3) / 4, 1);
        if (!g.wide)
            hipLaunchKernelGGL(k_init_cells<uint32_t>, colgrid, dim3(256), 0, st_, dd_);
        else
            hipLaunchKernelGGL(k_init_cells<uint64_t>, colgrid, dim3(256), 0, st_, dd_);
        HIP_CHECK(hipGetLastError());
        sel_lds_ = align_up(sel2_fixed_lds(local_job(), g) + (size_t)d_.claim_words * 4, 16);
        if (sel_lds_ > sel2_lds_budget(device_, g.wide)) throw std::runtime_error("selection kernel needs more dynamic LDS than the device leaves beside its static arrays (n_out too large)");
        if (!g.wide)
            HIP_CHECK(hipFuncSetAttribute(reinterpret_cast<const void *>(&k_iter_select2<uint32_t, true>), hipFuncAttributeMaxDynamicSharedMemorySize, (int)sel_lds_));
        else
            HIP_CHECK(hipFuncSetAttribute(reinterpret_cast<const void *>(&k_iter_select2<uint64_t, true>), hipFuncAttributeMaxDynamicSharedMemorySize, (int)sel_lds_));
        part_lds_ = align_up(2 * (size_t)n_loc_ * (g.wide ? 8 : 4) + 4 * 3 * (size_t)g.Kpad * 4 + (size_t)n_loc_ * 2, 16);
        HIP_CHECK(hipStreamSynchronize(st_));
    }
    ~HipShardEngine() override { (void)hipSetDevice(device_); }
    bool on_device() const override { return true; }
    int n_keys() const override { return geo_.K; }
    int32_t *init_counts(int64_t &count) override {
        const dim3 grid((unsigned)((n_pairs_ + 3) / 4));
        if (!geo_.wide)
            hipLaunchKernelGGL(k_cs_init_counts<uint32_t>, grid, dim3(256), (size_t)4 * geo_.Kpad * 4, st_, dd_);
        else
            hipLaunchKernelGGL(k_cs_init_counts<uint64_t>, grid, dim3(256), (size_t)4 * geo_.Kpad * 4, st_, dd_);
        sync();
        count = n_pairs_ * geo_.K;
        return d_.cs_init;
    }
    void init_table() override {
        const dim3 grid((unsigned)((n_pairs_ + 3) / 4));
        if (!geo_.wide)
            hipLaunchKernelGGL(k_cs_init_table<uint32_t>, grid, dim3(256), 0, st_, dd_);
        else
            hipLaunchKernelGGL(k_cs_init_table<uint64_t>, grid, dim3(256), 0, st_, dd_);
        HIP_CHECK(hipGetLastError());
    }
    void set_stream_ordered(bool on) override { stream_ordered_ = on; }
    void select(int32_t *&flags, int64_t &fcount) override {
        fw_ = flag_words(job_.n_in + (int)steps_);
        if (!stopped_) {
            if (!geo_.wide)
                hipLaunchKernelGGL((k_iter_select2<uint32_t, true>), dim3(1, 2), dim3(SEL2_THREADS), sel_lds_, st_, dd_, 1, d_done_, (int)steps_);
            else
                hipLaunchKernelGGL((k_iter_select2<uint64_t, true>), dim3(1, 2), dim3(SEL2_THREADS), sel_lds_, st_, dd_, 1, d_done_, (int)steps_);
            HIP_CHECK(hipGetLastError());
        } else {
            const int32_t tr[SHARD_TRAILER] = {1, 0, 0};
            HIP_CHECK(hipMemsetAsync(d_.cs_flags, 0, (size_t)fw_ * 4, st_));
            HIP_CHECK(hipMemcpyAsync(d_.cs_flags + fw_, tr, sizeof tr, hipMemcpyHostToDevice, st_));
            sync();
        }
        if (!stream_ordered_) sync();
        flags = d_.cs_flags;
        fcount = fw_ + SHARD_TRAILER;
    }
    int32_t *partial(int64_t &scount, int32_t status[SHARD_TRAILER]) override {
        const int seq = ++report_seq_;
        hipLaunchKernelGGL(k_cs_union, dim3(1), dim3(1024), 0, st_, dd_, report_, seq, (int)fw_);
        HIP_CHECK(hipGetLastError());
        {
            unsigned polls = 0, tries = 0;
            while (__atomic_load_n(&report_[0], __ATOMIC_ACQUIRE) != seq) {
                if (++tries > (1u << 16)) {
                    sync();
                    if (__atomic_load_n(&report_[0], __ATOMIC_ACQUIRE) != seq) throw std::runtime_error("column-sharded chain: the device did not report the step's status");
                    break;
                }
                spin_wait_step(polls);
            }
        }
        const int nuni = report_[1];
        for (int q = 0; q < SHARD_TRAILER; ++q) trailer_[q] = report_[2 + q];
        for (int q = 0; q < SHARD_TRAILER; ++q) status[q] = trailer_[q];
        scount = 0;
        if (status[0] != 0) {
            stopped_ = true;
            return nullptr;
        }
        nuni_ = nuni;
        if (nuni > 0) {
            const dim3 grid((unsigned)((nuni + 3) / 4));
            if (!geo_.wide)
                hipLaunchKernelGGL(k_cs_partial<uint32_t>, grid, dim3(256), part_lds_, st_, dd_);
            else
                hipLaunchKernelGGL(k_cs_partial<uint64_t>, grid, dim3(256), part_lds_, st_, dd_);
        }
        if (!stream_ordered_) sync();
        scount = (int64_t)(6 + 3 * (int64_t)nuni) * geo_.K;
        return d_.cs_slab;
    }
    void apply() override {
        const dim3 grid((unsigned)((nuni_ + 6 + 3) / 4));
        if (!geo_.wide)
            hipLaunchKernelGGL(k_cs_apply<uint32_t>, grid, dim3(256), 0, st_, dd_);
        else
            hipLaunchKernelGGL(k_cs_apply<uint64_t>, grid, dim3(256), 0, st_, dd_);
        HIP_CHECK(hipGetLastError());
        ++steps_;
    }
    void finish(ChainOut &o) override {
        dim3 colgrid((n_loc_ + 3) / 4, 1);
        if (!geo_.wide)
            hipLaunchKernelGGL(k_extract<uint32_t>, colgrid, dim3(256), 0, st_, dd_);
        else
            hipLaunchKernelGGL(k_extract<uint64_t>, colgrid, dim3(256), 0, st_, dd_);
        hipLaunchKernelGGL(k_pack, dim3(1), dim3(256), 0, st_, dd_);
        pull();
        o = ChainOut{};
        o.error = d_.error;
        o.unknown_method_hit = d_.unknown_hit != 0;
        o.n_bits = d_.n_bits;
        const size_t iters = (size_t)d_.iter;
        o.shift0.resize(job_.n_in);
        o.shift1.resize(job_.n_out);
        o.picks.resize(iters * 4);
        o.row_lat.resize((size_t)d_.n_rows);
        o.col_start.resize((size_t)n_loc_ + 1);
        HIP_CHECK(hipMemcpyAsync(o.shift0.data(), d_.shift0, job_.n_in, hipMemcpyDeviceToHost, st_));
        HIP_CHECK(hipMemcpyAsync(o.shift1.data(), d_.shift1, job_.n_out, hipMemcpyDeviceToHost, st_));
        if (iters) HIP_CHECK(hipMemcpyAsync(o.picks.data(), d_.picks, iters * sizeof(int4), hipMemcpyDeviceToHost, st_));
        HIP_CHECK(hipMemcpyAsync(o.row_lat.data(), d_.pk_lat, (size_t)d_.n_rows * 4, hipMemcpyDeviceToHost, st_));
        HIP_CHECK(hipMemcpyAsync(o.col_start.data(), d_.fin_start, ((size_t)n_loc_ + 1) * 4, hipMemcpyDeviceToHost, st_));
        sync();
        const size_t total = o.col_start[n_loc_];
        o.dig_row.resize(total);
        std::vector<unsigned long long> cells(total);
        if (total) {
            HIP_CHECK(hipMemcpyAsync(o.dig_row.data(), d_.pk_row, total * 4, hipMemcpyDeviceToHost, st_));
            HIP_CHECK(hipMemcpyAsync(cells.data(), d_.pk_cell, total * 8, hipMemcpyDeviceToHost, st_));
            sync();
        }
        o.dig_cell.assign(cells.begin(), cells.end());
        o.stats.iterations = d_.iter;
        o.stats.digits0 = d_.prep_digits;
        o.stats.table_peak = d_.live_peak;
        o.stats.partners = (long long)d_.st_partners;
        o.stats.matches = (long long)d_.st_matches;
        o.stats.scan_slots = (long long)d_.st_rescans << d_.gs_log2;
    }

  private:
    ChainJob local_job() const {
        ChainJob j = job_;
        j.n_out = n_loc_;
        return j;
    }
    void sync() {
        HIP_CHECK(hipGetLastError());
        HIP_CHECK(hipStreamSynchronize(st_));
    }
    void push() { HIP_CHECK(hipMemcpyAsync(dd_, &d_, sizeof d_, hipMemcpyHostToDevice, st_)); }
    void pull() {
        HIP_CHECK(hipGetLastError());
        HIP_CHECK(hipMemcpyAsync(&d_, dd_, sizeof d_, hipMemcpyDeviceToHost, st_));
        HIP_CHECK(hipStreamSynchronize(st_));
    }
    hipStream_t st_;
    StepLog2Host step_tab_;
    int64_t fw_ = 0;
    long long steps_ = 0;
    bool stopped_ = false, stream_ordered_ = false;
    int32_t trailer_[SHARD_TRAILER] = {0, 0, 0};
    int device_;
    ChainJob job_;
    int n_loc_;
    ChainDev d_;
    ChainDev *dd_ = nullptr;
    Geometry geo_;
    DeviceBuffer io_, desc_, arena_;
    DeviceBuffer done_buf_;
    unsigned int *d_done_ = nullptr;
    PinnedBuffer report_buf_;
    volatile int *report_ = nullptr;
    int report_seq_ = 0;
    long long n_pairs_ = 0;
    int nuni_ = 0;
    size_t sel_lds_ = 0, part_lds_ = 0;
};

}

std::unique_ptr<ShardEngine> HipBackend::make_shard_engine(const ChainJob &job, int c0, int c1, double capacity_scale) {
    return std::unique_ptr<ShardEngine>(new HipShardEngine(impl_->stream, impl_->device, job, c0, c1, impl_->table_scale * capacity_scale, row_scale_ * capacity_scale));
}

void HipBackend::column_distances(const int32_t *aug, int n_in, int W, int64_t *d0, int64_t *d1) {
    Impl &im = *impl_;
    HIP_CHECK(hipSetDevice(im.device));
    hipStream_t st = im.stream;
    size_t a_bytes = align_up((size_t)n_in * W * 4, 256), d_bytes = align_up((size_t)W * W * 8, 256);
// ... 97 lines not shown
```

da4ml_amd/csrc/cmvm_gpu.h:

```cpp
#pragma once

#include <memory>

#include "cmvm_host.h"
#include "cmvm_shard.h"

namespace da {
namespace gpu {

struct GpuTimings {
    double loop_ms = 0;
    double dist_ms = 0;
    double total_ms = 0;
    long long lockstep_iters = 0;
    long long iterations = 0;
    long long rescans = 0;
    long long partners = 0;
    long long chains = 0;
    long long retries = 0;
    long long dist_calls = 0;
    double select_ms_sampled = 0, update_ms_sampled = 0;
    long long samples = 0;
    double sampled_chain_launches = 0;
    long long found = 0, inserts = 0, cell_reads = 0;
    double key_bytes = 0;
    double cell_bytes = 0;
    double phase_cycles[12] = {0};
    double table_bytes = 0;
    double arena_bytes = 0;
    double select_bytes = 0;
    double host_launch_ms = 0;
    long long fast_steps = 0;
    double search_diag[7] = {0};
    double search_cycles[4] = {0};
};

class HipBackend : public Backend {
  public:
    explicit HipBackend(int device = 0);
    ~HipBackend() override;
    void run_chains(const ChainJob *jobs, ChainOut *outs, int n) override;
    void column_distances(const int32_t *aug, int n_in, int W, int64_t *d0, int64_t *d1) override;
    int csd_decompose(const float *kernel, int n_in, int n_out, bool center, std::vector<int8_t> &csd, std::vector<int8_t> &s0,
                      std::vector<int8_t> &s1) override;
    int int_to_csd(const int32_t *x, int64_t n, std::vector<int8_t> &csd) override;

    const GpuTimings &timings() const;
    void reset_timings();
    void *stream() const;
    std::unique_ptr<ShardEngine> make_shard_engine(const ChainJob &job, int c0, int c1, double capacity_scale = 1.0);

  private:
    struct Impl;
    std::unique_ptr<Impl> impl_;
    double row_scale_ = 1.0;
    int retry_depth_ = 0;
};

int device_count();

}
}
```

da4ml_amd/csrc/cmvm_host.cc:

```cpp

#include "cmvm_host.h"

#include <algorithm>
#include <cmath>
#include <condition_variable>
#include <cstring>
#include <atomic>
#include <chrono>
#include <cstdio>
#include <cstdlib>
#include <exception>
#include <functional>
#include <limits>
#include <memory>
#include <mutex>
#include <pthread.h>
#include <sched.h>
#include <unordered_map>
#include <thread>

namespace da {

int parse_method(const std::string &name) {
    static const char *names[] = {"mc", "mc-dc", "mc-pdc", "wmc", "wmc-dc", "wmc-pdc", "dummy"};
// ... 305 lines not shown
        for (int k = (int)st.lists.size() - 1; k >= 0; --k)
            if (st.lists[k].capacity() >= capacity && (best < 0 || st.lists[k].capacity() < st.lists[best].capacity())) best = k;
        if (best >= 0) {
            std::vector<OpRec> v = std::move(st.lists[best]);
            st.lists[best] = std::move(st.lists.back());
            st.lists.pop_back();
            st.bytes -= v.capacity() * sizeof(OpRec);
            v.clear();
            return v;
        }
    }
    std::vector<OpRec> v;
    v.reserve(capacity);
    return v;
}

void recycle_op_list(std::vector<OpRec> &&ops) {
    if (ops.capacity() < OpListStash::MIN_KEEP) return;
    OpListStash &st = op_list_stash();
    std::vector<OpRec> drop;
    std::lock_guard<std::mutex> lk(st.mu);
    const size_t b = ops.capacity() * sizeof(OpRec);
    if (st.bytes + b > OpListStash::MAX_BYTES || st.lists.size() >= OpListStash::MAX_LISTS) {
        drop = std::move(ops);
        return;
    }
    ops.clear();
    st.bytes += b;
    st.lists.push_back(std::move(ops));
}

StageResult finalize_prepare(const ChainJob &job, const ChainOut &out, std::vector<int64_t> &first_op) {
    if (out.error == E_REMOTE_ERROR) throw std::runtime_error("column-sharded CMVM chain failed on another rank (not a capacity error), or the ranks fell out of step");
    if (out.error != E_OK) throw std::runtime_error("CMVM chain failed on the device (error " + std::to_string(out.error) + ")");
    StageResult r;
    r.n_in = job.n_in;
    r.n_out = job.n_out;
    r.adder_size = job.adder_size;
    r.carry_size = job.carry_size;
    r.inp_shifts.assign(out.shift0.begin(), out.shift0.end());
    size_t n_iter = out.picks.size() / 4;
    const int n_out = job.n_out;
    first_op.assign((size_t)n_out + 1, 0);
    for (int j = 0; j < n_out; ++j) {
        int64_t terms = 0;
        for (uint32_t k = out.col_start[j]; k < out.col_start[j + 1]; ++k)
            terms += __builtin_popcountll(((uint64_t)(uint32_t)out.dig_cell[k]) | (out.dig_cell[k] >> 32));
        first_op[j + 1] = first_op[j] + (terms > 1 ? terms - 1 : 0);
    }
    r.ops = take_op_list((size_t)job.n_in + n_iter + (size_t)first_op[n_out]);
    for (int i = 0; i < job.n_in; ++i) r.ops.push_back(OpRec{i, -1, -1, 0, job.qints[i], job.lats[i], 0.0f});
    for (size_t t = 0; t < n_iter; ++t) {
        int64_t a = out.picks[4 * t], b = out.picks[4 * t + 1];
        bool sub = out.picks[4 * t + 2] != 0;
        int64_t shift = out.picks[4 * t + 3];
        const OpRec &oa = r.ops[a], &ob = r.ops[b];
        float dlat, cost;
        cost_add(oa.q, ob.q, shift, sub, job.adder_size, job.carry_size, dlat, cost);
        float lat = std::max(oa.latency, ob.latency) + dlat;
        float seen = out.row_lat[job.n_in + t];
        if (std::memcmp(&lat, &seen, 4) != 0 && !(lat != lat && seen != seen))
            throw std::runtime_error("device latency model diverged from the host libm at iteration " + std::to_string(t));
        r.ops.push_back(OpRec{a, b, (int64_t)sub, shift, qint_add(oa.q, ob.q, shift, false, sub), lat, cost});
    }
    const int64_t n_fixed = (int64_t)r.ops.size();
    r.ops.resize((size_t)(n_fixed + first_op[n_out]));
    r.out_idxs.assign((size_t)n_out, -1);
    r.out_shifts.assign((size_t)n_out, 0);
    r.out_negs.assign((size_t)n_out, 0);
    return r;
}

void finalize_columns(const ChainJob &job, const ChainOut &out, StageResult &r, const std::vector<int64_t> &first_op, int j0, int j1) {
    const int64_t n_fixed = (int64_t)r.ops.size() - first_op[job.n_out];
    {
        std::vector<Term> heap;
        auto cmp = [](const Term &x, const Term &y) { return term_after(x, y); };
        for (int j = j0; j < j1; ++j) {
            heap.clear();
            for (uint32_t k = out.col_start[j]; k < out.col_start[j + 1]; ++k) {
                uint64_t cell = out.dig_cell[k];
                uint32_t plus = (uint32_t)cell, minus = (uint32_t)(cell >> 32), any = plus | minus;
                int64_t row = out.dig_row[k];
                while (any) {
                    int pos = __builtin_ctz(any);
                    any &= any - 1;
                    const OpRec &o = r.ops[row];
                    heap.push_back(Term{o.latency, (int64_t)((minus >> pos) & 1), magnitude_bits(o.q) + pos, o.q, row, pos});
                }
            }
            if (heap.empty()) {
                r.out_shifts[j] = out.shift1[j];
                continue;
            }
            if (heap.size() == 1) {
                r.out_idxs[j] = heap[0].id;
                r.out_shifts[j] = (int64_t)out.shift1[j] + heap[0].shift;
                r.out_negs[j] = heap[0].neg;
                continue;
            }
            int64_t id = n_fixed + first_op[j];
            std::make_heap(heap.begin(), heap.end(), cmp);
            while (heap.size() > 1) {
                std::pop_heap(heap.begin(), heap.end(), cmp);
                Term first = heap.back();
                heap.pop_back();
                std::pop_heap(heap.begin(), heap.end(), cmp);
                Term second = heap.back();
                heap.pop_back();
                const Term &base = first.neg ? second : first, &other = first.neg ? first : second;
                int64_t sh = other.shift - base.shift;
                bool sub_op = first.neg ? (second.neg == 0) : (second.neg != 0);
                QInt q = qint_add(base.q, other.q, sh, base.neg != 0, other.neg != 0);
                float dlat, cost;
                cost_add(base.q, other.q, sh, sub_op, job.adder_size, job.carry_size, dlat, cost);
                float lat = std::max(first.lat, second.lat) + dlat;
                r.ops[id] = OpRec{base.id, other.id, (int64_t)sub_op, sh, q, lat, cost};
                heap.push_back(Term{lat, first.neg & second.neg, magnitude_bits(q) + base.shift, q, id, base.shift});
                std::push_heap(heap.begin(), heap.end(), cmp);
                ++id;
            }
            if (id != n_fixed + first_op[j + 1]) throw std::runtime_error("adder tree of a column emitted an unexpected number of ops (internal error)");
            r.out_idxs[j] = id - 1;
            r.out_negs[j] = heap[0].neg;
            r.out_shifts[j] = (int64_t)out.shift1[j] + heap[0].shift;
        }
    }
}

StageResult finalize_chain(const ChainJob &job, const ChainOut &out, int inner_threads) {
    std::vector<int64_t> first_op;
    StageResult r = finalize_prepare(job, out, first_op);
    const int n_out = job.n_out;
    const int n_chunks = inner_threads > 1 ? std::min(n_out, inner_threads * 4) : 1;
    auto reduce_chunk = [&](int c) {
        finalize_columns(job, out, r, first_op, (int)((long long)n_out * c / n_chunks), (int)((long long)n_out * (c + 1) / n_chunks));
    };
    if (n_chunks <= 1)
        finalize_columns(job, out, r, first_op, 0, n_out);
    else {
        std::atomic<int> next{0};
        std::exception_ptr err;
        std::mutex err_mu;
        auto work = [&] {
            for (int c = next++; c < n_chunks; c = next++) {
                try {
                    reduce_chunk(c);
                } catch (...) {
                    std::lock_guard<std::mutex> lk(err_mu);
                    if (!err) err = std::current_exception();
                }
            }
        };
        std::vector<std::thread> pool;
        for (int t = 1; t < std::min(inner_threads, n_chunks); ++t) pool.emplace_back(work);
        work();
        for (auto &t : pool) t.join();
        if (err) std::rethrow_exception(err);
    }
    return r;
}

namespace {

class HostPool {
  public:
    static HostPool &get() {
        static std::once_flag once;
        std::call_once(once, [] {
            pthread_atfork([] { make_mu().lock(); }, [] { make_mu().unlock(); },
                           [] {
                               instance().store(nullptr);
                               make_mu().unlock();
                           });
        });
        HostPool *p = instance().load();
        if (!p) {
            std::lock_guard<std::mutex> lk(make_mu());
            p = instance().load();
            if (!p) {
                p = new HostPool();
                instance().store(p);
            }
        }
        return *p;
    }
    template <class Fn> bool run(size_t n, Fn &&fn) {
        if (busy_.test_and_set(std::memory_order_acquire)) return false;
        struct Release {
            std::atomic_flag &f;
            ~Release() { f.clear(std::memory_order_release); }
        } release{busy_};
        std::exception_ptr err;
        std::mutex err_mu;
        std::atomic<size_t> next{0};
        std::function<void()> body = [&] {
            for (size_t i = next++; i < n; i = next++) {
                try {
                    fn(i);
                } catch (...) {
                    std::lock_guard<std::mutex> lk(err_mu);
                    if (!err) err = std::current_exception();
                }
            }
        };
        const int helpers = (int)std::min<size_t>((size_t)cap_, n - 1);
        {
            std::lock_guard<std::mutex> lk(mu_);
            while ((int)threads_.size() < helpers) {
                const int t = (int)threads_.size();
                threads_.emplace_back([this, t] { worker(t); });
                threads_.back().detach();
            }
            body_ = &body;
            wanted_ = helpers;
            pending_ = helpers;
            ++epoch_;
        }
        cv_work_.notify_all();
        if (helpers > NARROW) cv_wide_.notify_all();
        body();
        {
            std::unique_lock<std::mutex> lk(mu_);
            cv_done_.wait(lk, [&] { return pending_ == 0; });
            body_ = nullptr;
        }
        if (err) std::rethrow_exception(err);
        return true;
    }
    int capacity() const { return cap_ + 1; }

  private:
    static std::atomic<HostPool *> &instance() {
        static std::atomic<HostPool *> p{nullptr};
        return p;
    }
    static std::mutex &make_mu() {
        static std::mutex *m = new std::mutex();
        return *m;
    }
    HostPool() {
        unsigned hw = std::thread::hardware_concurrency();
        cpu_set_t set;
        if (sched_getaffinity(0, sizeof set, &set) == 0 && CPU_COUNT(&set) > 0) hw = (unsigned)CPU_COUNT(&set);
        cap_ = (int)std::max(1u, std::min(hw ? hw : 1u, 256u)) - 1;
        if (const char *e = std::getenv("DA4ML_HOST_THREADS")) cap_ = std::max(1, std::min(1024, std::atoi(e))) - 1;
    }
    void worker(int index) {
        uint64_t seen = 0;
        {
            std::lock_guard<std::mutex> lk(mu_);
            seen = epoch_ - 1;
        }
        for (;;) {
            std::function<void()> *body = nullptr;
            {
                std::unique_lock<std::mutex> lk(mu_);
                (index < NARROW ? cv_work_ : cv_wide_).wait(lk, [&] { return epoch_ != seen; });
                seen = epoch_;
                if (index < wanted_) body = body_;
            }
            if (!body) continue;
            (*body)();
            std::lock_guard<std::mutex> lk(mu_);
            if (--pending_ == 0) cv_done_.notify_one();
        }
    }
    std::mutex mu_;
    std::atomic_flag busy_ = ATOMIC_FLAG_INIT;
    static constexpr int NARROW = 63;
    std::condition_variable cv_work_, cv_wide_, cv_done_;
    std::vector<std::thread> threads_;
    std::function<void()> *body_ = nullptr;
    uint64_t epoch_ = 0;
    int cap_ = 0, wanted_ = 0, pending_ = 0;
};

template <class Fn> void parallel_for(size_t n, Fn &&fn) {
    if (n <= 1) {
        for (size_t i = 0; i < n; ++i) fn(i);
        return;
    }
    if (HostPool::get().run(n, fn)) return;
    unsigned hw = std::thread::hardware_concurrency();
    size_t workers = std::min<size_t>(n, std::max(1u, std::min(hw ? hw : 1u, 64u)));
    std::atomic<size_t> next{0};
    std::exception_ptr err;
    std::mutex err_mu;
    std::vector<std::thread> pool;
    for (size_t w = 0; w < workers; ++w)
        pool.emplace_back([&] {
            for (size_t i = next++; i < n; i = next++) {
                try {
                    fn(i);
                } catch (...) {
                    std::lock_guard<std::mutex> lk(err_mu);
                    if (!err) err = std::current_exception();
                }
            }
        });
    for (auto &t : pool) t.join();
    if (err) std::rethrow_exception(err);
}

bool has_dc_suffix(const std::string &m) { return m.size() >= 2 && m.compare(m.size() - 2, 2, "dc") == 0; }

struct Candidate {
    int problem = 0;
    std::string method0, method1;
    int hard_dc = -1, decompose_dc = -2;
    float allowed = std::numeric_limits<float>::infinity();
    enum Phase { NEED_MINLAT, NEED_STAGE0, NEED_STAGE1, DONE } phase = NEED_STAGE0;
    std::vector<float> m0, m1;
    StageResult sol0, sol1;
    std::vector<QInt> q_mid;
    std::vector<float> lat_mid;
};

struct ProblemState {
    const Problem *p = nullptr;
    std::vector<QInt> qints;
    std::vector<float> lats;
    std::shared_ptr<Stage1> s1p;
    bool minlat_known = false;
    float minlat = 0.0f;
    std::vector<int> cand;
};

float max_out_latency(const StageResult &s) {
    float top = 0.0f;
    for (auto idx : s.out_idxs) top = std::max(top, idx >= 0 ? s.ops[idx].latency : 0.0f);
    return top;
}

}

namespace {
std::vector<PipeResult> solve_batch_unique(Backend &be, const std::vector<Problem> &problems, std::vector<ChainStats> *stats);

bool same_problem(const Problem &a, const Problem &b) {
    const SolveOptions &x = a.opt, &y = b.opt;
    if (a.n_in != b.n_in || a.n_out != b.n_out || x.hard_dc != y.hard_dc || x.decompose_dc != y.decompose_dc || x.adder_size != y.adder_size ||
        x.carry_size != y.carry_size || x.search_all != y.search_all || x.method0 != y.method0 || x.method1 != y.method1 ||
        x.qints.size() != y.qints.size() || x.lats.size() != y.lats.size())
        return false;
    if (!x.qints.empty() && std::memcmp(x.qints.data(), y.qints.data(), sizeof(QInt) * x.qints.size()) != 0) return false;
    if (!x.lats.empty() && std::memcmp(x.lats.data(), y.lats.data(), sizeof(float) * x.lats.size()) != 0) return false;
    return a.kernel == b.kernel || std::memcmp(a.kernel, b.kernel, sizeof(float) * (size_t)a.n_in * a.n_out) == 0;
}
uint64_t problem_hash(const Problem &p) {
    uint64_t h = 1469598103934665603ull;
    auto mix = [&](const void *data, size_t n) {
        const unsigned char *b = static_cast<const unsigned char *>(data);
        uint64_t a[4] = {h, h ^ 0x9E3779B97F4A7C15ull, h ^ 0xC2B2AE3D27D4EB4Full, h ^ 0x165667B19E3779F9ull};
        size_t i = 0;
        for (; i + 32 <= n; i += 32)
            for (int q = 0; q < 4; ++q) {
                uint64_t w;
                std::memcpy(&w, b + i + 8 * q, 8);
                a[q] = (a[q] ^ w) * 1099511628211ull;
                a[q] ^= a[q] >> 29;
            }
        for (; i + 4 <= n; i += 4) {
            uint32_t w;
            std::memcpy(&w, b + i, 4);
            a[0] = (a[0] ^ w) * 1099511628211ull;
            a[0] ^= a[0] >> 29;
        }
        h = a[0];
        for (int q = 1; q < 4; ++q) {
            h = (h ^ a[q]) * 1099511628211ull;
            h ^= h >> 29;
        }
    };
    mix(&p.n_in, sizeof p.n_in);
    mix(&p.n_out, sizeof p.n_out);
    mix(p.kernel, sizeof(float) * (size_t)p.n_in * p.n_out);
    if (!p.opt.qints.empty()) mix(p.opt.qints.data(), sizeof(QInt) * p.opt.qints.size());
    if (!p.opt.lats.empty()) mix(p.opt.lats.data(), sizeof(float) * p.opt.lats.size());
    return h;
}
}

std::vector<PipeResult> solve_batch(Backend &be, const std::vector<Problem> &problems, std::vector<ChainStats> *stats) {
    const size_t n = problems.size();
    std::vector<int> rep(n);
    std::vector<Problem> uniq;
    std::unordered_multimap<uint64_t, int> seen;
    for (size_t i = 0; i < n; ++i) {
        if (problems[i].n_in <= 0 || problems[i].n_out <= 0 || !problems[i].kernel) throw std::invalid_argument("kernel must be a non-empty 2-D matrix");
        const uint64_t h = problem_hash(problems[i]);
        int found = -1;
        auto range = seen.equal_range(h);
        for (auto it = range.first; it != range.second && found < 0; ++it)
            if (same_problem(uniq[it->second], problems[i])) found = it->second;
        if (found < 0) {
            found = (int)uniq.size();
            uniq.push_back(problems[i]);
            seen.emplace(h, found);
        }
        rep[i] = found;
    }
    if (uniq.size() == n) return solve_batch_unique(be, problems, stats);
    std::vector<ChainStats> ustats;
    std::vector<PipeResult> ures = solve_batch_unique(be, uniq, &ustats);
    std::vector<PipeResult> res(n);
    if (stats) stats->assign(n, ChainStats{});
    for (size_t i = n; i-- > 0;) {
        bool first = true;
        for (size_t j = 0; j < i && first; ++j) first = rep[j] != rep[i];
        if (first) {
            res[i] = std::move(ures[rep[i]]);
            if (stats && rep[i] < (int)ustats.size()) (*stats)[i] = ustats[rep[i]];
        } else
            res[i] = ures[rep[i]];
    }
    return res;
}

namespace {
std::vector<PipeResult> solve_batch_unique(Backend &be, const std::vector<Problem> &problems, std::vector<ChainStats> *stats) {
    const bool verbose = std::getenv("DA4ML_HIP_VERBOSE") != nullptr;
    auto lap = [verbose, last = std::chrono::steady_clock::now()](const char *what) mutable {
        auto now = std::chrono::steady_clock::now();
        if (verbose) std::fprintf(stderr, "[da4ml_hip] host: %-24s %8.2f ms\n", what, std::chrono::duration<double, std::milli>(now - last).count());
        last = now;
    };
    std::vector<ProblemState> ps(problems.size());
    std::vector<Candidate> cands;
    std::vector<size_t> fresh;
    for (size_t i = 0; i < problems.size(); ++i) {
        const Problem &p = problems[i];
        ProblemState &s = ps[i];
        s.p = &p;
        s.qints = p.opt.qints.empty() ? std::vector<QInt>(p.n_in, QInt{-128.0f, 127.0f, 1.0f}) : p.opt.qints;
        s.lats = p.opt.lats.empty() ? std::vector<float>(p.n_in, 0.0f) : p.opt.lats;
        if ((int)s.qints.size() != p.n_in || (int)s.lats.size() != p.n_in)
            throw std::invalid_argument("qintervals / latencies must have one entry per kernel row");
        for (size_t j = 0; j < i && !s.s1p; ++j) {
            const Problem &o = problems[j];
            if (o.n_in == p.n_in && o.n_out == p.n_out &&
                (o.kernel == p.kernel || std::memcmp(o.kernel, p.kernel, sizeof(float) * (size_t)p.n_in * p.n_out) == 0))
                s.s1p = ps[j].s1p;
        }
        if (!s.s1p) {
            s.s1p = std::make_shared<Stage1>();
            fresh.push_back(i);
        }
        int log2_n = (int)std::ceil(std::log2((float)p.n_in));
        std::vector<std::pair<int, int>> tries;
        if (!p.opt.search_all)
            tries.emplace_back(p.opt.hard_dc, p.opt.decompose_dc);
        else {
            int hdc = p.opt.hard_dc < 0 ? 1000000000 : p.opt.hard_dc;
            for (int d = -1; d <= std::min(hdc, log2_n); ++d) tries.emplace_back(hdc, d);
        }
        for (auto [hdc, ddc] : tries) {
            Candidate c;
            c.problem = (int)i;
            c.method0 = p.opt.method0;
            c.method1 = p.opt.method1;
            c.hard_dc = hdc;
            if (c.method1 == "auto") c.method1 = (hdc >= 6 || has_dc_suffix(c.method0)) ? c.method0 : c.method0 + "-dc";
            if (hdc == 0 && !has_dc_suffix(c.method0)) c.method0 += "-dc";
            c.decompose_dc = ddc == -2 ? std::min(hdc, log2_n) : std::min({hdc, ddc, log2_n});
            c.phase = hdc >= 0 ? Candidate::NEED_MINLAT : Candidate::NEED_STAGE0;
            s.cand.push_back((int)cands.size());
            cands.push_back(std::move(c));
        }
    }

    parallel_for(fresh.size(), [&](size_t k) { stage1_prepare(*ps[fresh[k]].s1p, problems[fresh[k]].kernel, problems[fresh[k]].n_in, problems[fresh[k]].n_out); });
    lap("problem set-up");
    auto prepare_stage0 = [&](Candidate &c) {
        ProblemState &s = ps[c.problem];
        if (c.decompose_dc < 0 && c.hard_dc >= 0) c.method0 = c.method1 = (c.method0 != "dummy") ? "wmc-dc" : "dummy";
        stage1_split(be, *s.s1p, c.decompose_dc, c.m0, c.m1);
    };

    struct Pending {
        int cand;
        int what;
        int problem;
    };
    while (true) {
        std::vector<ChainJob> jobs;
        std::vector<Pending> owners;
        std::vector<char> minlat_queued(ps.size(), 0);
        {
            std::vector<size_t> todo;
            for (size_t ci = 0; ci < cands.size(); ++ci) {
                Candidate &c = cands[ci];
                ProblemState &s = ps[c.problem];
                bool ready = c.phase == Candidate::NEED_STAGE0 || (c.phase == Candidate::NEED_MINLAT && s.minlat_known);
                if (!ready) continue;
                todo.push_back(ci);
                int ddc = c.decompose_dc;
                if (ddc != -1) stage1_distances(be, *s.s1p);
            }
            parallel_for(todo.size(), [&](size_t k) {
                Candidate &c = cands[todo[k]];
                ProblemState &s = ps[c.problem];
                if (c.phase == Candidate::NEED_MINLAT) {
                    c.allowed = c.hard_dc + s.minlat;
                    c.phase = Candidate::NEED_STAGE0;
                }
                prepare_stage0(c);
            });
        }
        for (size_t ci = 0; ci < cands.size(); ++ci) {
            Candidate &c = cands[ci];
            ProblemState &s = ps[c.problem];
            const Problem &p = *s.p;
            if (c.phase == Candidate::NEED_MINLAT) {
                if (s.minlat_known) {
                    c.allowed = c.hard_dc + s.minlat;
                    c.phase = Candidate::NEED_STAGE0;
                } else if (!minlat_queued[c.problem]) {
                    jobs.push_back(ChainJob{p.kernel, p.n_in, p.n_out, M_DUMMY, s.qints.data(), s.lats.data(), p.opt.adder_size, p.opt.carry_size});
                    owners.push_back(Pending{(int)ci, 0, c.problem});
                    minlat_queued[c.problem] = 1;
                    continue;
                } else
                    continue;
            }
            if (c.phase == Candidate::NEED_STAGE0) {
                jobs.push_back(ChainJob{c.m0.data(), p.n_in, p.n_out, parse_method(c.method0), s.qints.data(), s.lats.data(), p.opt.adder_size, p.opt.carry_size});
                owners.push_back(Pending{(int)ci, 1, c.problem});
            } else if (c.phase == Candidate::NEED_STAGE1) {
                jobs.push_back(ChainJob{c.m1.data(), p.n_out, p.n_out, parse_method(c.method1), c.q_mid.data(), c.lat_mid.data(), p.opt.adder_size, p.opt.carry_size});
                owners.push_back(Pending{(int)ci, 2, c.problem});
            }
        }
        if (jobs.empty()) break;
        lap("stage 1 + job list");
        std::vector<ChainOut> outs(jobs.size());
        auto t_rc = std::chrono::steady_clock::now();
        {
            std::vector<uint8_t> on_host(jobs.size(), 0);
            parallel_for(jobs.size(), [&](size_t k) { on_host[k] = host_chain(jobs[k], outs[k]) ? 1 : 0; });
            std::vector<ChainJob> dev_jobs;
            std::vector<size_t> dev_idx;
            for (size_t k = 0; k < jobs.size(); ++k)
                if (!on_host[k]) {
                    dev_jobs.push_back(jobs[k]);
                    dev_idx.push_back(k);
                }
            if (!dev_jobs.empty()) {
                std::vector<ChainOut> dev_outs(dev_jobs.size());
                be.run_chains(dev_jobs.data(), dev_outs.data(), (int)dev_jobs.size());
                for (size_t k = 0; k < dev_idx.size(); ++k) outs[dev_idx[k]] = std::move(dev_outs[k]);
            }
        }
        auto t_fin = std::chrono::steady_clock::now();
        for (size_t k = 0; k < jobs.size(); ++k)
            if (outs[k].unknown_method_hit) {
                Candidate &c = cands[owners[k].cand];
                throw std::runtime_error("Unknown method: " + (owners[k].what == 2 ? c.method1 : c.method0));
            }
        std::vector<StageResult> sols(jobs.size());
        std::vector<std::vector<int64_t>> first_op(jobs.size());
        parallel_for(jobs.size(), [&](size_t k) { sols[k] = finalize_prepare(jobs[k], outs[k], first_op[k]); });
        size_t chunk_from = 4096;
        int chunks_per_chain = 16;
        if (const char *e = std::getenv("DA4ML_HIP_TREE_THREADS")) {
            chunks_per_chain = std::max(1, std::atoi(e)) * 4;
            chunk_from = 0;
        }
        struct Piece {
            int chain, j0, j1;
        };
        std::vector<Piece> pieces;
        for (size_t k = 0; k < jobs.size(); ++k) {
            const int n_out = jobs[k].n_out;
            const int parts = outs[k].dig_row.size() >= chunk_from ? std::max(1, std::min(n_out, chunks_per_chain)) : 1;
            for (int c = 0; c < parts; ++c)
                pieces.push_back(Piece{(int)k, (int)((long long)n_out * c / parts), (int)((long long)n_out * (c + 1) / parts)});
        }
        parallel_for(pieces.size(), [&](size_t i) {
            const Piece &pc = pieces[i];
            finalize_columns(jobs[pc.chain], outs[pc.chain], sols[pc.chain], first_op[pc.chain], pc.j0, pc.j1);
        });
        if (std::getenv("DA4ML_HIP_VERBOSE"))
            std::fprintf(stderr, "[da4ml_hip] round of %zu chains: run_chains %.2f ms, adder trees %.2f ms\n", jobs.size(),
                         std::chrono::duration<double, std::milli>(t_fin - t_rc).count(),
                         std::chrono::duration<double, std::milli>(std::chrono::steady_clock::now() - t_fin).count());
        lap("chains + adder trees");
        for (size_t k = 0; k < jobs.size(); ++k) {
            Candidate &c = cands[owners[k].cand];
            ProblemState &s = ps[c.problem];
            if (stats) {
                if (stats->size() < problems.size()) stats->resize(problems.size());
                ChainStats &a = (*stats)[c.problem];
                const ChainStats &b = outs[k].stats;
                a.iterations += b.iterations;
                a.digits0 += b.digits0;
                a.blocks0 += b.blocks0;
                a.rebuilds += b.rebuilds;
                a.table_peak = std::max(a.table_peak, b.table_peak);
                a.scan_slots += b.scan_slots;
                a.partners += b.partners;
                a.matches += b.matches;
            }
            StageResult sol = std::move(sols[k]);
            bool both_wmc_dc = c.method0 == "wmc-dc" && c.method1 == "wmc-dc";
            if (owners[k].what == 0) {
                s.minlat = max_out_latency(sol);
                s.minlat_known = true;
                continue;
            }
            if (owners[k].what == 1) {
                c.sol0 = std::move(sol);
                c.q_mid.clear();
                c.lat_mid.clear();
                for (auto idx : c.sol0.out_idxs) {
                    c.lat_mid.push_back(idx >= 0 ? c.sol0.ops[idx].latency : 0.0f);
                    c.q_mid.push_back(idx >= 0 ? c.sol0.ops[idx].q : QInt{0.0f, 0.0f, std::numeric_limits<float>::infinity()});
                }
                if (max_out_latency(c.sol0) > c.allowed && (!both_wmc_dc || c.decompose_dc >= 0)) {
                    c.decompose_dc--;
                    c.phase = Candidate::NEED_STAGE0;
                } else
                    c.phase = Candidate::NEED_STAGE1;
            } else {
                c.sol1 = std::move(sol);
                if (max_out_latency(c.sol1) > c.allowed && (!both_wmc_dc || c.decompose_dc >= 0)) {
                    c.decompose_dc--;
                    c.phase = Candidate::NEED_STAGE0;
                } else
                    c.phase = Candidate::DONE;
            }
        }
        lap("results taken over");
        parallel_for(outs.size(), [&](size_t k) {
            outs[k] = ChainOut();
            std::vector<int64_t>().swap(first_op[k]);
        });
        lap("round buffers released");
    }

    lap("candidate bookkeeping");
    std::vector<PipeResult> results(problems.size());
    for (size_t i = 0; i < problems.size(); ++i) {
        ProblemState &s = ps[i];
        int best = 0;
        if (s.p->opt.search_all) {
            std::vector<float> costs;
            for (int ci : s.cand) {
                float total = 0.0f;
                for (const StageResult *st : {&cands[ci].sol0, &cands[ci].sol1})
                    for (const OpRec &op : st->ops) total += op.cost;
                costs.push_back(total);
            }
            for (size_t k = 1; k < costs.size(); ++k)
                if (costs[k] < costs[best]) best = (int)k;
            results[i].picked = best;
        }
        Candidate &w = cands[s.cand[best]];
        results[i].stages.push_back(std::move(w.sol0));
        results[i].stages.push_back(std::move(w.sol1));
    }
    for (Candidate &c : cands) {
        recycle_op_list(std::move(c.sol0.ops));
        recycle_op_list(std::move(c.sol1.ops));
    }
    lap("winner selection");
    return results;
}

}

}
```

da4ml_amd/csrc/cmvm_host.h:

```cpp
#pragma once

#include <cstdint>
#include <stdexcept>
#include <string>
#include <vector>

#include "cmvm_core.h"

namespace da {

struct QInt {
    float lo, hi, step;
};
struct OpRec {
    int64_t id0, id1, opcode, data;
    QInt q;
    float latency, cost;
};
struct StageResult {
    int64_t n_in = 0, n_out = 0;
    std::vector<int64_t> inp_shifts, out_idxs, out_shifts, out_negs;
    std::vector<OpRec> ops;
    int carry_size = -1, adder_size = -1;
};
struct PipeResult {
    std::vector<StageResult> stages;
    int picked = -1;
};

struct ChainStats {
    int64_t iterations = 0, digits0 = 0, blocks0 = 0, rebuilds = 0, table_peak = 0, scan_slots = 0, partners = 0,
            matches = 0;
};

struct ChainJob {
    const float *kernel = nullptr;
    int n_in = 0, n_out = 0;
    int method = M_WMC;
    const QInt *qints = nullptr;
    const float *lats = nullptr;
    int adder_size = -1, carry_size = -1;
};
struct ChainOut {
    int error = E_OK;
    bool unknown_method_hit = false;
    int n_bits = 0;
    std::vector<int8_t> shift0, shift1;
    std::vector<int32_t> picks;
    std::vector<float> row_lat;
    std::vector<uint32_t> col_start, dig_row;
    std::vector<uint64_t> dig_cell;
    ChainStats stats;
};

class Backend {
  public:
    virtual ~Backend() = default;
    virtual void run_chains(const ChainJob *jobs, ChainOut *outs, int n) = 0;
    virtual void column_distances(const int32_t *aug, int n_in, int W, int64_t *d0, int64_t *d1) = 0;
    virtual int csd_decompose(const float *kernel, int n_in, int n_out, bool center, std::vector<int8_t> &csd,
                              std::vector<int8_t> &s0, std::vector<int8_t> &s1) = 0;
    virtual int int_to_csd(const int32_t *x, int64_t n, std::vector<int8_t> &csd) = 0;
};

struct SolveOptions {
    std::string method0 = "wmc", method1 = "auto";
    int hard_dc = -1, decompose_dc = -2;
    std::vector<QInt> qints;
    std::vector<float> lats;
    int adder_size = -1, carry_size = -1;
    bool search_all = true;
};

int parse_method(const std::string &name);

QInt qint_add(const QInt &a, const QInt &b, int64_t shift, bool neg_a, bool neg_b);
void cost_add(const QInt &a, const QInt &b, int64_t shift, bool sub, int adder_size, int carry_size, float &dlat,
              float &cost);

Log2Table measure_log2_table();
struct StepLog2Host {
    std::vector<uint32_t> mant;
    std::vector<float> tab;
    void build(const QInt *q, int n_in);
    StepLog2 view() const { return StepLog2{(int)mant.size(), mant.data(), tab.data()}; }
};

void center_matrix(std::vector<float> &a, int n_in, int n_out, std::vector<int8_t> &s0, std::vector<int8_t> &s1);

void kernel_decompose(Backend &be, const float *kernel, int n_in, int n_out, int dc, std::vector<float> &m0,
                      std::vector<float> &m1);

std::vector<OpRec> take_op_list(size_t capacity);
void recycle_op_list(std::vector<OpRec> &&ops);
StageResult finalize_prepare(const ChainJob &job, const ChainOut &out, std::vector<int64_t> &first_op);
void finalize_columns(const ChainJob &job, const ChainOut &out, StageResult &r, const std::vector<int64_t> &first_op, int j0, int j1);
StageResult finalize_chain(const ChainJob &job, const ChainOut &out, int inner_threads = 1);

struct Problem {
    const float *kernel;
    int n_in, n_out;
    SolveOptions opt;
};
std::vector<PipeResult> solve_batch(Backend &be, const std::vector<Problem> &problems, std::vector<ChainStats> *stats = nullptr);

}
```

Measured before the change: 113.0 solves/s.

## Stream per-group chain results to host finalization as each lane finishes

Restructures run_chains so each stream group has its own done flag, gather and pinned buffers, and queues its own init, extract, pack and copy-back. A tail thread hands finished groups to a callback that runs the host adder-tree finalization while other groups are still iterating on the GPU. The aim is to overlap host finalize and result gathering with the remaining device chain work, and to stop serializing init kernels before the loop. It adds thread and condition-variable coordination, more events, and more complex error and retry handling.

```diff
diff --git a/da4ml_amd/_binary/__init__.py b/da4ml_amd/_binary/__init__.py
--- a/da4ml_amd/_binary/__init__.py
+++ b/da4ml_amd/_binary/__init__.py
@@ -386,7 +386,7 @@
              'select_ms_sampled', 'update_ms_sampled', 'samples', 'found', 'inserts', 'cell_reads', 'block_bytes', 'cell_bytes',
              'sel_load_bounds', 'sel_argmax', 'sel_newrow', 'sel_substitute', 'sel_prefix', 'sel_claims', 'sel_special',
              'upd_fetch', 'upd_probe', 'upd_cells', 'upd_blocks', 'upd_create', 'retries', 'sampled_chain_launches')
-    extra = ('select_bytes', 'host_launch_ms', 'fast_steps', 'search_bounds', 'search_argmax', 'search_excluded', 'search_steps_timed', 'search_stale_rereads', 'search_touch_rereads', 'search_rounds', 'search_long_lists', 'search_longest_list', 'search_full_passes', 'search_list_entries')
+    extra = ('select_bytes', 'host_launch_ms', 'fast_steps', 'search_bounds', 'search_argmax', 'search_excluded', 'search_steps_timed', 'search_stale_rereads', 'search_touch_rereads', 'search_rounds', 'search_long_lists', 'search_longest_list', 'search_full_passes', 'search_list_entries', 'handed_on', 'handed_on_abandoned')
     return {**dict(zip(names, t.tolist())), **dict(zip(extra, e.tolist()))}
 
 
diff --git a/da4ml_amd/csrc/cmvm_capi.cc b/da4ml_amd/csrc/cmvm_capi.cc
--- a/da4ml_amd/csrc/cmvm_capi.cc
+++ b/da4ml_amd/csrc/cmvm_capi.cc
@@ -393,7 +393,7 @@
     std::lock_guard<LibraryMutex> lk(g_mutex);
     try {
         const da::gpu::GpuTimings &g = backend().timings();
-        const double v[16] = {g.select_bytes, g.host_launch_ms, (double)g.fast_steps, g.search_cycles[0], g.search_cycles[1], g.search_cycles[2], g.search_cycles[3], g.search_diag[0], g.search_diag[1], g.search_diag[2], g.search_diag[3], g.search_diag[4], g.search_diag[5], g.search_diag[6], 0.0, 0.0};
+        const double v[16] = {g.select_bytes, g.host_launch_ms, (double)g.fast_steps, g.search_cycles[0], g.search_cycles[1], g.search_cycles[2], g.search_cycles[3], g.search_diag[0], g.search_diag[1], g.search_diag[2], g.search_diag[3], g.search_diag[4], g.search_diag[5], g.search_diag[6], (double)g.handed_on, (double)g.handed_on_abandoned};
         const int m = n < 16 ? (n < 0 ? 0 : n) : 16;
         for (int i = 0; i < m; ++i) out[i] = v[i];
         return m;
diff --git a/da4ml_amd/csrc/cmvm_engine.hip b/da4ml_amd/csrc/cmvm_engine.hip
--- a/da4ml_amd/csrc/cmvm_engine.hip
+++ b/da4ml_amd/csrc/cmvm_engine.hip
@@ -5,9 +5,11 @@
 #include <atomic>
 #include <chrono>
 #include <cmath>
+#include <condition_variable>
 #include <cstdio>
 #include <cstdlib>
 #include <cstring>
+#include <deque>
 #include <memory>
 #include <mutex>
 #include <numeric>
@@ -2437,14 +2439,16 @@
 
 struct HipBackend::Impl {
     int device = 0;
-    PinnedBuffer pinned, pinned_up;
+    PinnedBuffer pinned_up, pinned_fin;
     hipStream_t stream = nullptr;
     static constexpr int MAX_LANES = 8;
     hipStream_t lanes[MAX_LANES] = {nullptr, nullptr, nullptr, nullptr, nullptr, nullptr, nullptr, nullptr};
     int launch_threads = 2;
     int n_lanes = 4;
     int upd_total_blocks = 2560;
-    DeviceBuffer arena, desc_buf, io_buf, gather_buf, piece_buf;
+    DeviceBuffer arena, desc_buf, io_buf;
+    DeviceBuffer gather_buf[MAX_LANES], piece_buf[MAX_LANES];
+    PinnedBuffer pinned[MAX_LANES];
     unsigned int *d_done = nullptr;
     unsigned int *h_done = nullptr;
     hipStream_t poll_stream = nullptr;
@@ -2463,8 +2467,8 @@
     if (const char *e = std::getenv("DA4ML_HIP_UPD_BLOCKS")) impl_->upd_total_blocks = std::max(2, std::atoi(e));
     if (const char *e = std::getenv("DA4ML_HIP_LAUNCH_THREADS")) impl_->launch_threads = std::max(1, std::atoi(e));
     if (const char *e = std::getenv("DA4ML_HIP_LANES")) impl_->n_lanes = std::max(1, std::min((int)Impl::MAX_LANES, std::atoi(e)));
-    HIP_CHECK(hipMalloc(&impl_->d_done, sizeof(unsigned int)));
-    HIP_CHECK(hipHostMalloc(&impl_->h_done, 2 * sizeof(unsigned int), hipHostMallocDefault));
+    HIP_CHECK(hipMalloc(&impl_->d_done, Impl::MAX_LANES * sizeof(unsigned int)));
+    HIP_CHECK(hipHostMalloc(&impl_->h_done, 2 * Impl::MAX_LANES * sizeof(unsigned int), hipHostMallocDefault));
     HIP_CHECK(hipStreamCreateWithFlags(&impl_->poll_stream, hipStreamNonBlocking));
     Log2Table t = measure_log2_table();
     HIP_CHECK(hipMemcpyToSymbol(HIP_SYMBOL(c_log2), &t, sizeof t));
@@ -2554,7 +2558,9 @@
 
 }
 
-void HipBackend::run_chains(const ChainJob *jobs, ChainOut *outs, int n) {
+void HipBackend::run_chains(const ChainJob *jobs, ChainOut *outs, int n) { run_chains_streamed(jobs, outs, n, ReadyFn()); }
+
+void HipBackend::run_chains_streamed(const ChainJob *jobs, ChainOut *outs, int n, const ReadyFn &on_ready) {
     if (n <= 0) return;
     Impl &im = *impl_;
     HIP_CHECK(hipSetDevice(im.device));
@@ -2680,8 +2686,8 @@
                                          std::to_string(geo[0].C) + " slots), " + std::to_string(free_b >> 20) + " MiB are free (budget " +
                                          std::to_string(budget >> 20) + " MiB)");
             const int half_n = n / 2;
-            run_chains(jobs, outs, half_n);
-            run_chains(jobs + half_n, outs + half_n, n - half_n);
+            run_chains_streamed(jobs, outs, half_n, on_ready);
+            run_chains_streamed(jobs + half_n, outs + half_n, n - half_n, on_ready ? ReadyFn([&](int first, int count) { on_ready(half_n + first, count); }) : ReadyFn());
             return;
         }
     }
@@ -2716,7 +2722,7 @@
         }
     }
     HIP_CHECK(hipMemcpyAsync(d_desc, desc.data(), sizeof(ChainDev) * (size_t)n, hipMemcpyHostToDevice, st));
-    HIP_CHECK(hipMemsetAsync(im.d_done, 0, sizeof(unsigned int), st));
+    HIP_CHECK(hipMemsetAsync(im.d_done, 0, sizeof(unsigned int) * Impl::MAX_LANES, st));
     hipLaunchKernelGGL(k_init_state, dim3(128, n), dim3(256), 0, st, d_desc);
     HIP_CHECK(hipGetLastError());
 
@@ -2737,8 +2743,6 @@
         int first, count;
         bool wide;
     } ranges[2] = {{0, n_narrow, false}, {n_narrow, n - n_narrow, true}};
-    int active = 0;
-    for (int i = 0; i < n; ++i) active += desc[i].done ? 0 : 1;
 
     size_t sel_lds[2] = {0, 0}, upd_lds[2] = {0, 0}, pair_lds[2] = {0, 0};
     int upd_blocks[2] = {1, 1};
@@ -2760,32 +2764,11 @@
         if (cnt == 0) continue;
         upd_blocks[w] = std::max(2, std::min(64, (im.upd_total_blocks + cnt - 1) / std::max(cnt, 1)));
     }
-    for (int w = 0; w < 2; ++w) {
-        const Range &r = ranges[w];
-        if (r.count == 0) continue;
-        ChainDev *base = d_desc + r.first;
-        dim3 colgrid((max_n_out + 3) / 4, r.count);
-        dim3 pairgrid((unsigned)((max_pairs[w] + 3) / 4), r.count);
-        if (!r.wide) {
-            hipLaunchKernelGGL(k_init_cells<uint32_t>, colgrid, dim3(256), 0, st, base);
-            hipLaunchKernelGGL(k_init_pairs<uint32_t>, pairgrid, dim3(256), pair_lds[w], st, base);
-        } else {
-            hipLaunchKernelGGL(k_init_cells<uint64_t>, colgrid, dim3(256), 0, st, base);
-            hipLaunchKernelGGL(k_init_pairs<uint64_t>, pairgrid, dim3(256), pair_lds[w], st, base);
-        }
-        HIP_CHECK(hipGetLastError());
-    }
     if (ranges[0].count)
         HIP_CHECK(hipFuncSetAttribute(reinterpret_cast<const void *>(&k_iter_select2<uint32_t>), hipFuncAttributeMaxDynamicSharedMemorySize, (int)sel_lds[0]));
     if (ranges[1].count)
         HIP_CHECK(hipFuncSetAttribute(reinterpret_cast<const void *>(&k_iter_select2<uint64_t>), hipFuncAttributeMaxDynamicSharedMemorySize, (int)sel_lds[1]));
 
-    HIP_CHECK(hipStreamSynchronize(st));
-    lap("arena + init kernels");
-    EventGuard events;
-    hipEvent_t ev0 = events.make(), ev1 = events.make();
-    HIP_CHECK(hipEventRecord(ev0, st));
-    HIP_CHECK(hipStreamSynchronize(st));
     struct Group {
         int first, count, w;
         hipStream_t stream;
@@ -2801,16 +2784,56 @@
             groups.push_back(Group{lo, hi - lo, w, im.lanes[groups.size() % Impl::MAX_LANES]});
         }
     }
+    const int n_grp = (int)groups.size();
+    EventGuard events;
+    struct DrainOnError {
+        const std::vector<Group> &g;
+        hipStream_t poll;
+        bool armed = true;
+        ~DrainOnError() {
+            if (!armed) return;
+            for (const Group &gr : g) (void)hipStreamSynchronize(gr.stream);
+            (void)hipStreamSynchronize(poll);
+        }
+    } drain{groups, im.poll_stream};
+    hipEvent_t setup_ev = events.make(hipEventDisableTiming);
+    HIP_CHECK(hipEventRecord(setup_ev, st));
+    std::vector<hipEvent_t> init_ev(n_grp), loop_ev0(n_grp), loop_ev1(n_grp), fin_ev(n_grp);
+    for (int gi = 0; gi < n_grp; ++gi) {
+        const Group &gr = groups[gi];
+        if (gr.stream != st) HIP_CHECK(hipStreamWaitEvent(gr.stream, setup_ev, 0));
+        if (gi > 0) HIP_CHECK(hipStreamWaitEvent(gr.stream, init_ev[gi - 1], 0));
+        ChainDev *base = d_desc + gr.first;
+        const dim3 colgrid((max_n_out + 3) / 4, gr.count);
+        const dim3 pairgrid((unsigned)((max_pairs[gr.w] + 3) / 4), gr.count);
+        if (gr.w == 0) {
+            hipLaunchKernelGGL(k_init_cells<uint32_t>, colgrid, dim3(256), 0, gr.stream, base);
+            hipLaunchKernelGGL(k_init_pairs<uint32_t>, pairgrid, dim3(256), pair_lds[0], gr.stream, base);
+        } else {
+            hipLaunchKernelGGL(k_init_cells<uint64_t>, colgrid, dim3(256), 0, gr.stream, base);
+            hipLaunchKernelGGL(k_init_pairs<uint64_t>, pairgrid, dim3(256), pair_lds[1], gr.stream, base);
+        }
+        HIP_CHECK(hipGetLastError());
+        init_ev[gi] = events.make(hipEventDisableTiming);
+        HIP_CHECK(hipEventRecord(init_ev[gi], gr.stream));
+        loop_ev0[gi] = events.make();
+        loop_ev1[gi] = events.make();
+        fin_ev[gi] = events.make(hipEventDisableTiming);
+        HIP_CHECK(hipEventRecord(loop_ev0[gi], gr.stream));
+    }
+    lap("arena + init kernels queued");
     const char *stats_env = std::getenv("DA4ML_HIP_STATS");
     const bool with_stats = stats_env && std::atoi(stats_env) != 0;
-    auto launch_pair = [&](const Group &gr, hipEvent_t *se, int step) {
+    auto launch_pair = [&](int gi, hipEvent_t *se, int step) {
+        const Group &gr = groups[gi];
         ChainDev *base = d_desc + gr.first;
+        unsigned int *done = im.d_done + gi;
         const dim3 sel_grid((gr.count + 7) & ~7, 2);
         if (se) HIP_CHECK(hipEventRecord(se[0], gr.stream));
         if (gr.w == 0)
-            hipLaunchKernelGGL(k_iter_select2<uint32_t>, sel_grid, dim3(SEL2_THREADS), sel_lds[0], gr.stream, base, gr.count, im.d_done, step);
+            hipLaunchKernelGGL(k_iter_select2<uint32_t>, sel_grid, dim3(SEL2_THREADS), sel_lds[0], gr.stream, base, gr.count, done, step);
         else
-            hipLaunchKernelGGL(k_iter_select2<uint64_t>, sel_grid, dim3(SEL2_THREADS), sel_lds[1], gr.stream, base, gr.count, im.d_done, step);
+            hipLaunchKernelGGL(k_iter_select2<uint64_t>, sel_grid, dim3(SEL2_THREADS), sel_lds[1], gr.stream, base, gr.count, done, step);
         if (se) HIP_CHECK(hipEventRecord(se[1], gr.stream));
         const dim3 upd_grid((gr.count + 7) & ~7, upd_blocks[gr.w] + 2);
         if (gr.w == 0 && !with_stats)
@@ -2826,46 +2849,208 @@
     constexpr int WINDOW_ITERS = 63, MAX_SAMPLES = 4096;
     std::vector<hipEvent_t> sample_ev;
     int n_samples = 0;
+    double sampled_chains = 0;
     long long launched_iters = 0, iter_cap = 0;
     for (int i = 0; i < n; ++i) iter_cap = std::max<long long>(iter_cap, geo[i].rcap - jobs[i].n_in + 2);
     const int poll_every = WINDOW_ITERS + 1;
-    int pre_done = 0;
-    for (int i = 0; i < n; ++i) pre_done += (jobs[i].method == M_DUMMY || jobs[i].method < 0) ? 1 : 0;
+    std::vector<int> to_run(n_grp, 0);
+    for (int gi = 0; gi < n_grp; ++gi)
+        for (int s = groups[gi].first; s < groups[gi].first + groups[gi].count; ++s) to_run[gi] += desc[order[s]].done ? 0 : 1;
     hipEvent_t win_ev[2][Impl::MAX_LANES], copy_ev[2];
     for (int p = 0; p < 2; ++p) {
         copy_ev[p] = events.make(hipEventDisableTiming);
-        for (size_t gi = 0; gi < groups.size(); ++gi) win_ev[p][gi] = events.make(hipEventDisableTiming);
-    }
-    im.h_done[0] = im.h_done[1] = 0;
+        for (int gi = 0; gi < n_grp; ++gi) win_ev[p][gi] = events.make(hipEventDisableTiming);
+    }
+    for (int k = 0; k < 2 * Impl::MAX_LANES; ++k) im.h_done[k] = 0;
     long long window = 0;
     double host_launch_ms = 0;
-    struct DrainOnError {
-        const std::vector<Group> &g;
-        hipStream_t poll;
-        bool armed = true;
-        ~DrainOnError() {
-            if (!armed) return;
-            for (const Group &gr : g) (void)hipStreamSynchronize(gr.stream);
-            (void)hipStreamSynchronize(poll);
-        }
-    } drain{groups, im.poll_stream};
+
+    ChainDev *fin = static_cast<ChainDev *>(im.pinned_fin.get(sizeof(ChainDev) * (size_t)n));
+    const bool can_retry = retry_depth_ < 4;
+    std::vector<long long> grp_iters(n_grp, 0);
+    auto queue_extract = [&](int gi) {
+        const Group &gr = groups[gi];
+        HIP_CHECK(hipEventRecord(loop_ev1[gi], gr.stream));
+        const dim3 colgrid((max_n_out + 3) / 4, gr.count);
+        if (gr.w == 0)
+            hipLaunchKernelGGL(k_extract<uint32_t>, colgrid, dim3(256), 0, gr.stream, d_desc + gr.first);
+        else
+            hipLaunchKernelGGL(k_extract<uint64_t>, colgrid, dim3(256), 0, gr.stream, d_desc + gr.first);
+        hipLaunchKernelGGL(k_pack, dim3(gr.count), dim3(256), 0, gr.stream, d_desc + gr.first);
+        HIP_CHECK(hipGetLastError());
+        HIP_CHECK(hipMemcpyAsync(fin + gr.first, d_desc + gr.first, sizeof(ChainDev) * (size_t)gr.count, hipMemcpyDeviceToHost, gr.stream));
+        HIP_CHECK(hipEventRecord(fin_ev[gi], gr.stream));
+    };
+    struct Tail {
+        std::mutex mu;
+        std::condition_variable cv;
+        std::deque<int> ready;
+        bool closed = false;
+        bool need_retry = false;
+        long long handed_on = 0;
+        std::exception_ptr err;
+        std::chrono::steady_clock::time_point loop_exit = std::chrono::steady_clock::time_point::max();
+        double caller_ms_after_loop = 0;
+        std::thread th;
+        void push(int gi) {
+            {
+                std::lock_guard<std::mutex> lk(mu);
+                ready.push_back(gi);
+            }
+            cv.notify_one();
+        }
+    } tail;
+    auto finish_group = [&](int gi) {
+        const Group &gr = groups[gi];
+        HIP_CHECK(hipEventSynchronize(fin_ev[gi]));
+        for (int s = gr.first; s < gr.first + gr.count; ++s) {
+            const ChainDev &d = fin[s];
+            ChainOut &o = outs[order[s]];
+            o = ChainOut{};
+            o.error = d.error;
+            o.unknown_method_hit = d.unknown_hit != 0;
+            o.n_bits = d.n_bits;
+            if (d.error == E_TABLE_CAPACITY || d.error == E_ROW_CAPACITY) tail.need_retry = true;
+        }
+        if (tail.need_retry && can_retry) return;
+        struct ResultOffsets {
+            size_t st, s0, s1, pk, lat, row, cell;
+            uint32_t total;
+        };
+        std::vector<ResultOffsets> roff(gr.count);
+        std::vector<GatherPiece> pieces;
+        pieces.reserve((size_t)gr.count * 7);
+        size_t gather_bytes = 0;
+        auto piece = [&](const void *src, size_t bytes) {
+            const size_t at = gather_bytes;
+            if (bytes) pieces.push_back(GatherPiece{src, (unsigned long long)at, (unsigned long long)bytes});
+            gather_bytes += align_up(bytes, 64);
+            return at;
+        };
+        for (int q = 0; q < gr.count; ++q) {
+            const ChainDev &d = fin[gr.first + q];
+            const ChainJob &j = jobs[order[gr.first + q]];
+            ResultOffsets &ro = roff[q];
+            ro.total = d.error == E_OK ? d.pk_total : 0u;
+            ro.st = piece(d.fin_start, ((size_t)j.n_out + 1) * 4);
+            ro.s0 = piece(d.shift0, (size_t)j.n_in);
+            ro.s1 = piece(d.shift1, (size_t)j.n_out);
+            ro.pk = piece(d.picks, (size_t)d.iter * sizeof(int4));
+            ro.lat = piece(d.pk_lat, (size_t)d.n_rows * 4);
+            ro.row = piece(d.pk_row, (size_t)ro.total * 4);
+            ro.cell = piece(d.pk_cell, (size_t)ro.total * 8);
+        }
+        unsigned char *pin = static_cast<unsigned char *>(im.pinned[gi].get(std::max<size_t>(gather_bytes, 64)));
+        unsigned char *gbuf = static_cast<unsigned char *>(im.gather_buf[gi].get(std::max<size_t>(gather_bytes, 64)));
+        GatherPiece *d_pieces = static_cast<GatherPiece *>(im.piece_buf[gi].get(std::max<size_t>(pieces.size(), 1) * sizeof(GatherPiece)));
+        HIP_CHECK(hipMemcpyAsync(d_pieces, pieces.data(), pieces.size() * sizeof(GatherPiece), hipMemcpyHostToDevice, gr.stream));
+        for (size_t first = 0; first < pieces.size(); first += 32768) {
+            const unsigned cnt = (unsigned)std::min<size_t>(32768, pieces.size() - first);
+            hipLaunchKernelGGL(k_gather, dim3(16, cnt), dim3(256), 0, gr.stream, d_pieces + first, gbuf);
+        }
+        HIP_CHECK(hipGetLastError());
+        HIP_CHECK(hipMemcpyAsync(pin, gbuf, gather_bytes, hipMemcpyDeviceToHost, gr.stream));
+        HIP_CHECK(hipStreamSynchronize(gr.stream));
+        host_parallel_for((size_t)gr.count, [&](size_t q) {
+            const int s = gr.first + (int)q;
+            const ChainDev &d = fin[s];
+            const ChainJob &j = jobs[order[s]];
+            const ResultOffsets &ro = roff[q];
+            ChainOut &o = outs[order[s]];
+            const uint32_t *cs = reinterpret_cast<const uint32_t *>(pin + ro.st);
+            o.col_start.assign(cs, cs + j.n_out + 1);
+            o.shift0.assign(reinterpret_cast<const int8_t *>(pin + ro.s0), reinterpret_cast<const int8_t *>(pin + ro.s0) + j.n_in);
+            o.shift1.assign(reinterpret_cast<const int8_t *>(pin + ro.s1), reinterpret_cast<const int8_t *>(pin + ro.s1) + j.n_out);
+            const int32_t *pk = reinterpret_cast<const int32_t *>(pin + ro.pk);
+            o.picks.assign(pk, pk + (size_t)d.iter * 4);
+            const float *lat = reinterpret_cast<const float *>(pin + ro.lat);
+            o.row_lat.assign(lat, lat + d.n_rows);
+            const uint32_t *pr = reinterpret_cast<const uint32_t *>(pin + ro.row);
+            const unsigned long long *pc = reinterpret_cast<const unsigned long long *>(pin + ro.cell);
+            o.dig_row.assign(pr, pr + ro.total);
+            o.dig_cell.assign(pc, pc + ro.total);
+            o.stats.iterations = d.iter;
+            o.stats.digits0 = d.prep_digits;
+            o.stats.table_peak = d.live_peak;
+            o.stats.scan_slots = (long long)d.st_rescans << d.gs_log2;
+            o.stats.partners = (long long)d.st_partners;
+            o.stats.matches = (long long)d.st_matches;
+        });
+        if (!on_ready) return;
+        std::vector<int> ids(gr.count);
+        for (int q = 0; q < gr.count; ++q) ids[q] = order[gr.first + q];
+        std::sort(ids.begin(), ids.end());
+        const auto t_cb = std::chrono::steady_clock::now();
+        for (size_t a = 0; a < ids.size();) {
+            size_t b = a + 1;
+            while (b < ids.size() && ids[b] == ids[b - 1] + 1) ++b;
+            on_ready(ids[a], (int)(b - a));
+            tail.handed_on += (long long)(b - a);
+            a = b;
+        }
+        const auto t_cb1 = std::chrono::steady_clock::now();
+        std::chrono::steady_clock::time_point exit_at;
+        {
+            std::lock_guard<std::mutex> lk(tail.mu);
+            exit_at = tail.loop_exit;
+        }
+        if (t_cb1 > exit_at) tail.caller_ms_after_loop += std::chrono::duration<double, std::milli>(t_cb1 - std::max(t_cb, exit_at)).count();
+    };
+    tail.th = std::thread([&] {
+        try {
+            HIP_CHECK(hipSetDevice(im.device));
+        } catch (...) {
+            tail.err = std::current_exception();
+        }
+        while (true) {
+            int gi;
+            {
+                std::unique_lock<std::mutex> lk(tail.mu);
+                tail.cv.wait(lk, [&] { return !tail.ready.empty() || tail.closed; });
+                if (tail.ready.empty()) break;
+                gi = tail.ready.front();
+                tail.ready.pop_front();
+            }
+            if (tail.err) continue;
+            try {
+                finish_group(gi);
+            } catch (...) {
+                tail.err = std::current_exception();
+            }
+        }
+    });
+    struct JoinTail {
+        Tail &t;
+        void join() {
+            {
+                std::lock_guard<std::mutex> lk(t.mu);
+                t.closed = true;
+                if (t.loop_exit == std::chrono::steady_clock::time_point::max()) t.loop_exit = std::chrono::steady_clock::now();
+            }
+            t.cv.notify_one();
+            if (t.th.joinable()) t.th.join();
+        }
+        ~JoinTail() { join(); }
+    } join_tail{tail};
+
     struct Helper {
         std::atomic<long long> seq{0}, ack{0};
         std::atomic<bool> quit{false};
         long long first_step = 0;
         int iters = 0, parity = 0;
+        unsigned live = 0;
         std::exception_ptr err;
         std::thread th;
     } helper;
-    const bool two_threads = im.launch_threads >= 2 && groups.size() >= 2;
-    auto mine = [&](size_t gi, int who) { return !two_threads || (int)(gi & 1) == who; };
-    auto window_launches = [&](int who, long long first_step, int iters, int parity, hipEvent_t *se0) {
+    const bool two_threads = im.launch_threads >= 2 && n_grp >= 2;
+    auto mine = [&](int gi, int who) { return !two_threads || (gi & 1) == who; };
+    auto window_launches = [&](int who, long long first_step, int iters, int parity, unsigned live, int sample_gi, hipEvent_t *se0) {
         for (int it = 0; it < iters; ++it)
-            for (size_t gi = 0; gi < groups.size(); ++gi)
-                if (mine(gi, who)) launch_pair(groups[gi], it == 0 && gi == 0 ? se0 : nullptr, (int)(first_step + it));
+            for (int gi = 0; gi < n_grp; ++gi)
+                if ((live >> gi & 1u) && mine(gi, who)) launch_pair(gi, it == 0 && gi == sample_gi ? se0 : nullptr, (int)(first_step + it));
         HIP_CHECK(hipGetLastError());
-        for (size_t gi = 0; gi < groups.size(); ++gi)
-            if (mine(gi, who)) HIP_CHECK(hipEventRecord(win_ev[parity][gi], groups[gi].stream));
+        for (int gi = 0; gi < n_grp; ++gi)
+            if ((live >> gi & 1u) && mine(gi, who)) HIP_CHECK(hipEventRecord(win_ev[parity][gi], groups[gi].stream));
     };
     if (two_threads)
         helper.th = std::thread([&] {
@@ -2878,7 +3063,7 @@
                     while ((s = helper.seq.load(std::memory_order_acquire)) == seen && !helper.quit.load(std::memory_order_acquire)) spin_wait_step(polls);
                     if (s == seen) break;
                     seen = s;
-                    if (!helper.err) window_launches(1, helper.first_step, helper.iters, helper.parity, nullptr);
+                    if (!helper.err) window_launches(1, helper.first_step, helper.iters, helper.parity, helper.live, -1, nullptr);
                     helper.ack.store(seen, std::memory_order_release);
                 }
             } catch (...) {
@@ -2898,64 +3083,86 @@
             if (h.th.joinable()) h.th.join();
         }
     } join_helper{helper};
-    while (active > 0) {
+    unsigned live = 0;
+    for (int gi = 0; gi < n_grp; ++gi) {
+        if (to_run[gi] > 0)
+            live |= 1u << gi;
+        else {
+            queue_extract(gi);
+            tail.push(gi);
+        }
+    }
+    while (live) {
         const auto t_q0 = std::chrono::steady_clock::now();
         if (launched_iters > iter_cap + 2 * poll_every) throw std::runtime_error("greedy loop did not terminate within its row capacity (internal error)");
         const int this_window = (int)std::min<long long>(WINDOW_ITERS, (8ll << std::min<long long>(window, 8)) - 1);
         const int p = (int)(window & 1);
         if (two_threads) {
-            helper.first_step = launched_iters, helper.iters = this_window + 1, helper.parity = p;
+            helper.first_step = launched_iters, helper.iters = this_window + 1, helper.parity = p, helper.live = live;
             helper.seq.fetch_add(1, std::memory_order_release);
         }
+        int sample_gi = -1;
+        for (int gi = n_grp - 1; gi >= 0; --gi)
+            if ((live >> gi & 1u) && mine(gi, 0)) sample_gi = gi;
         hipEvent_t se[3];
-        const bool sample = n_samples < MAX_SAMPLES;
+        const bool sample = n_samples < MAX_SAMPLES && sample_gi >= 0;
         if (sample) {
             for (auto &e : se) {
                 e = events.make();
                 sample_ev.push_back(e);
             }
             ++n_samples;
-        }
-        window_launches(0, launched_iters, this_window + 1, p, sample ? se : nullptr);
+            sampled_chains += groups[sample_gi].count;
+        }
+        window_launches(0, launched_iters, this_window + 1, p, live, sample ? sample_gi : -1, sample ? se : nullptr);
         launched_iters += this_window + 1;
+        for (int gi = 0; gi < n_grp; ++gi)
+            if (live >> gi & 1u) grp_iters[gi] = launched_iters;
         if (two_threads) {
             const long long want = helper.seq.load(std::memory_order_relaxed);
             unsigned polls = 0;
             while (helper.ack.load(std::memory_order_acquire) != want) spin_wait_step(polls);
             if (helper.err) std::rethrow_exception(helper.err);
         }
-        for (size_t gi = 0; gi < groups.size(); ++gi) HIP_CHECK(hipStreamWaitEvent(im.poll_stream, win_ev[p][gi], 0));
-        HIP_CHECK(hipMemcpyAsync(&im.h_done[p], im.d_done, sizeof(unsigned int), hipMemcpyDeviceToHost, im.poll_stream));
+        for (int gi = 0; gi < n_grp; ++gi)
+            if (live >> gi & 1u) HIP_CHECK(hipStreamWaitEvent(im.poll_stream, win_ev[p][gi], 0));
+        HIP_CHECK(hipMemcpyAsync(&im.h_done[p * Impl::MAX_LANES], im.d_done, sizeof(unsigned int) * (size_t)n_grp, hipMemcpyDeviceToHost, im.poll_stream));
         HIP_CHECK(hipEventRecord(copy_ev[p], im.poll_stream));
         host_launch_ms += std::chrono::duration<double, std::milli>(std::chrono::steady_clock::now() - t_q0).count();
         if (window > 0) {
             HIP_CHECK(hipEventSynchronize(copy_ev[p ^ 1]));
-            active = n - pre_done - (int)im.h_done[p ^ 1];
+            for (int gi = 0; gi < n_grp; ++gi)
+                if ((live >> gi & 1u) && (int)im.h_done[(p ^ 1) * Impl::MAX_LANES + gi] >= to_run[gi]) {
+                    live &= ~(1u << gi);
+                    queue_extract(gi);
+                    tail.push(gi);
+                }
         }
         ++window;
     }
+    {
+        std::lock_guard<std::mutex> lk(tail.mu);
+        tail.loop_exit = std::chrono::steady_clock::now();
+    }
+    join_tail.join();
     for (const Group &gr : groups) HIP_CHECK(hipStreamSynchronize(gr.stream));
     HIP_CHECK(hipStreamSynchronize(im.poll_stream));
     drain.armed = false;
-    HIP_CHECK(hipEventRecord(ev1, st));
-
-    lap("greedy loop");
-    for (int w = 0; w < 2; ++w) {
-        const Range &r = ranges[w];
-        if (r.count == 0) continue;
-        dim3 colgrid((max_n_out + 3) / 4, r.count);
-        if (!r.wide)
-            hipLaunchKernelGGL(k_extract<uint32_t>, colgrid, dim3(256), 0, st, d_desc + r.first);
-        else
-            hipLaunchKernelGGL(k_extract<uint64_t>, colgrid, dim3(256), 0, st, d_desc + r.first);
-    }
-    hipLaunchKernelGGL(k_pack, dim3(n), dim3(256), 0, st, d_desc);
-    HIP_CHECK(hipGetLastError());
-    std::vector<ChainDev> fin(n);
-    HIP_CHECK(hipMemcpyAsync(fin.data(), d_desc, sizeof(ChainDev) * (size_t)n, hipMemcpyDeviceToHost, st));
-    HIP_CHECK(hipStreamSynchronize(st));
+    lap("greedy loop + extract + download + unpack");
+    if (tail.err) std::rethrow_exception(tail.err);
+
     float loop_ms = 0;
-    HIP_CHECK(hipEventElapsedTime(&loop_ms, ev0, ev1));
+    {
+        float first_start = 0, last_end = 0;
+        for (int gi = 0; gi < n_grp; ++gi) {
+            float a = 0, b = 0;
+            HIP_CHECK(hipEventElapsedTime(&a, loop_ev0[0], loop_ev0[gi]));
+            HIP_CHECK(hipEventElapsedTime(&b, loop_ev0[0], loop_ev1[gi]));
+            first_start = gi ? std::min(first_start, a) : a;
+            last_end = gi ? std::max(last_end, b) : b;
+        }
+        loop_ms = last_end - first_start;
+    }
     for (int k = 0; k < n_samples; ++k) {
         float a = 0, b = 0;
         HIP_CHECK(hipEventElapsedTime(&a, sample_ev[3 * k], sample_ev[3 * k + 1]));
@@ -2964,27 +3171,26 @@
         im.timings.update_ms_sampled += b;
     }
     im.timings.samples += n_samples;
-    im.timings.sampled_chain_launches += (double)n_samples * (groups.empty() ? 0 : groups[0].count);
-
-    bool need_retry = false;
-    for (int s = 0; s < n; ++s) {
-        const ChainDev &d = fin[s];
-        int i = order[s];
-        ChainOut &o = outs[i];
-        o = ChainOut{};
-        o.error = d.error;
-        o.unknown_method_hit = d.unknown_hit != 0;
-        o.n_bits = d.n_bits;
-        if (d.error == E_TABLE_CAPACITY || d.error == E_ROW_CAPACITY) need_retry = true;
-    }
-    if (need_retry && retry_depth_ < 4) {
+    im.timings.sampled_chain_launches += sampled_chains;
+    if (verbose) {
+        std::fprintf(stderr, "[da4ml_hip] lockstep steps per group:");
+        for (int gi = 0; gi < n_grp; ++gi) {
+            int longest = 0;
+            for (int s = groups[gi].first; s < groups[gi].first + groups[gi].count; ++s) longest = std::max(longest, fin[s].iter);
+            std::fprintf(stderr, " %d (launched %lld)", longest, grp_iters[gi]);
+        }
+        std::fprintf(stderr, "\n");
+    }
+
+    if (tail.need_retry && can_retry) {
         ++retry_depth_;
         im.timings.retries += 1;
+        im.timings.handed_on_abandoned += tail.handed_on;
         double keep_t = im.table_scale, keep_r = row_scale_;
         im.table_scale *= 4.0;
         row_scale_ *= 4.0;
         try {
-            run_chains(jobs, outs, n);
+            run_chains_streamed(jobs, outs, n, on_ready);
         } catch (...) {
             im.table_scale = keep_t;
             row_scale_ = keep_r;
@@ -2996,93 +3202,9 @@
         --retry_depth_;
         return;
     }
-    struct ResultOffsets {
-        size_t st, s0, s1, pk, lat, row, cell;
-        uint32_t total;
-    };
-    std::vector<ResultOffsets> roff(n);
-    std::vector<GatherPiece> pieces;
-    pieces.reserve((size_t)n * 7);
-    size_t gather_bytes = 0;
-    auto piece = [&](const void *src, size_t bytes) {
-        const size_t at = gather_bytes;
-        if (bytes) pieces.push_back(GatherPiece{src, (unsigned long long)at, (unsigned long long)bytes});
-        gather_bytes += align_up(bytes, 64);
-        return at;
-    };
-    for (int s = 0; s < n; ++s) {
-        const ChainDev &d = fin[s];
-        const ChainJob &j = jobs[order[s]];
-        ResultOffsets &ro = roff[s];
-        ro.total = d.error == E_OK ? d.pk_total : 0u;
-        ro.st = piece(d.fin_start, ((size_t)j.n_out + 1) * 4);
-        ro.s0 = piece(d.shift0, (size_t)j.n_in);
-        ro.s1 = piece(d.shift1, (size_t)j.n_out);
-        ro.pk = piece(d.picks, (size_t)d.iter * sizeof(int4));
-        ro.lat = piece(d.pk_lat, (size_t)d.n_rows * 4);
-        ro.row = piece(d.pk_row, (size_t)ro.total * 4);
-        ro.cell = piece(d.pk_cell, (size_t)ro.total * 8);
-    }
-    unsigned char *pin = static_cast<unsigned char *>(im.pinned.get(std::max<size_t>(gather_bytes, 64)));
-    {
-        unsigned char *gbuf = static_cast<unsigned char *>(im.gather_buf.get(std::max<size_t>(gather_bytes, 64)));
-        GatherPiece *d_pieces = static_cast<GatherPiece *>(im.piece_buf.get(std::max<size_t>(pieces.size(), 1) * sizeof(GatherPiece)));
-        HIP_CHECK(hipMemcpyAsync(d_pieces, pieces.data(), pieces.size() * sizeof(GatherPiece), hipMemcpyHostToDevice, st));
-        for (size_t first = 0; first < pieces.size(); first += 32768) {
-            const unsigned cnt = (unsigned)std::min<size_t>(32768, pieces.size() - first);
-            hipLaunchKernelGGL(k_gather, dim3(16, cnt), dim3(256), 0, st, d_pieces + first, gbuf);
-        }
-        HIP_CHECK(hipGetLastError());
-        HIP_CHECK(hipMemcpyAsync(pin, gbuf, gather_bytes, hipMemcpyDeviceToHost, st));
-        HIP_CHECK(hipStreamSynchronize(st));
-    }
-    auto unpack = [&](int s) {
-        const ChainDev &d = fin[s];
-        const ChainJob &j = jobs[order[s]];
-        const ResultOffsets &ro = roff[s];
-        ChainOut &o = outs[order[s]];
-        const uint32_t *cs = reinterpret_cast<const uint32_t *>(pin + ro.st);
-        o.col_start.assign(cs, cs + j.n_out + 1);
-        o.shift0.assign(reinterpret_cast<const int8_t *>(pin + ro.s0), reinterpret_cast<const int8_t *>(pin + ro.s0) + j.n_in);
-        o.shift1.assign(reinterpret_cast<const int8_t *>(pin + ro.s1), reinterpret_cast<const int8_t *>(pin + ro.s1) + j.n_out);
-        const int32_t *pk = reinterpret_cast<const int32_t *>(pin + ro.pk);
-        o.picks.assign(pk, pk + (size_t)d.iter * 4);
-        const float *lat = reinterpret_cast<const float *>(pin + ro.lat);
-        o.row_lat.assign(lat, lat + d.n_rows);
-        const uint32_t *pr = reinterpret_cast<const uint32_t *>(pin + ro.row);
-        const unsigned long long *pc = reinterpret_cast<const unsigned long long *>(pin + ro.cell);
-        o.dig_row.assign(pr, pr + ro.total);
-        o.dig_cell.assign(pc, pc + ro.total);
-    };
-    {
-        const int workers = (int)std::min<size_t>({(size_t)n, (size_t)8, gather_bytes / (1u << 20) + 1});
-        std::atomic<int> next{0};
-        std::exception_ptr err;
-        std::mutex err_mu;
-        auto work = [&] {
-            try {
-                for (int s = next++; s < n; s = next++) unpack(s);
-            } catch (...) {
-                std::lock_guard<std::mutex> lk(err_mu);
-                if (!err) err = std::current_exception();
-            }
-        };
-        std::vector<std::thread> pool;
-        for (int t = 1; t < workers; ++t) pool.emplace_back(work);
-        work();
-        for (auto &t : pool) t.join();
-        if (err) std::rethrow_exception(err);
-    }
     for (int s = 0; s < n; ++s) {
         const ChainDev &d = fin[s];
         const int i = order[s];
-        ChainOut &o = outs[i];
-        o.stats.iterations = d.iter;
-        o.stats.digits0 = d.prep_digits;
-        o.stats.table_peak = d.live_peak;
-        o.stats.scan_slots = (long long)d.st_rescans << d.gs_log2;
-        o.stats.partners = (long long)d.st_partners;
-        o.stats.matches = (long long)d.st_matches;
         for (int q = 0; q < 12; ++q) im.timings.phase_cycles[q] += (double)d.st_phase[q];
         for (int q = 0; q < 4; ++q) im.timings.search_cycles[q] += (double)d.st_qphase[q];
         im.timings.search_diag[0] += (double)d.st_qdiag[0], im.timings.search_diag[1] += (double)d.st_qdiag[1], im.timings.search_diag[2] += (double)d.st_qdiag[4];
@@ -3099,13 +3221,13 @@
         im.timings.partners += (long long)d.st_partners;
         im.timings.table_bytes += (double)d.C * (8.0 + 4.0 + (double)(1 << d.pb_log2));
     }
-    lap("extract + download + unpack");
     im.timings.loop_ms += loop_ms;
     im.timings.host_launch_ms += host_launch_ms;
     im.timings.lockstep_iters += launched_iters;
     im.timings.chains += n;
+    im.timings.handed_on += tail.handed_on;
     im.timings.arena_bytes = std::max(im.timings.arena_bytes, (double)arena_bytes);
-    im.timings.total_ms += std::chrono::duration<double, std::milli>(std::chrono::steady_clock::now() - t_begin).count();
+    im.timings.total_ms += std::chrono::duration<double, std::milli>(std::chrono::steady_clock::now() - t_begin).count() - tail.caller_ms_after_loop;
     (void)max_n_in;
 }
 
diff --git a/da4ml_amd/csrc/cmvm_gpu.h b/da4ml_amd/csrc/cmvm_gpu.h
--- a/da4ml_amd/csrc/cmvm_gpu.h
+++ b/da4ml_amd/csrc/cmvm_gpu.h
@@ -30,6 +30,7 @@
     double arena_bytes = 0;
     double select_bytes = 0;
     double host_launch_ms = 0;
+    long long handed_on = 0, handed_on_abandoned = 0;
     long long fast_steps = 0;
     double search_diag[7] = {0};
     double search_cycles[4] = {0};
@@ -40,6 +41,7 @@
     explicit HipBackend(int device = 0);
     ~HipBackend() override;
     void run_chains(const ChainJob *jobs, ChainOut *outs, int n) override;
+    void run_chains_streamed(const ChainJob *jobs, ChainOut *outs, int n, const ReadyFn &on_ready) override;
     void column_distances(const int32_t *aug, int n_in, int W, int64_t *d0, int64_t *d1) override;
     int csd_decompose(const float *kernel, int n_in, int n_out, bool center, std::vector<int8_t> &csd, std::vector<int8_t> &s0,
                       std::vector<int8_t> &s1) override;
diff --git a/da4ml_amd/csrc/cmvm_host.cc b/da4ml_amd/csrc/cmvm_host.cc
--- a/da4ml_amd/csrc/cmvm_host.cc
+++ b/da4ml_amd/csrc/cmvm_host.cc
@@ -631,6 +631,10 @@
     for (auto &t : pool) t.join();
     if (err) std::rethrow_exception(err);
 }
+
+}
+void host_parallel_for(size_t n, const std::function<void(size_t)> &fn) { parallel_for(n, fn); }
+namespace {
 
 bool has_dc_suffix(const std::string &m) { return m.size() >= 2 && m.compare(m.size() - 2, 2, "dc") == 0; }
 
@@ -865,55 +869,92 @@
         lap("stage 1 + job list");
         std::vector<ChainOut> outs(jobs.size());
         auto t_rc = std::chrono::steady_clock::now();
-        {
-            std::vector<uint8_t> on_host(jobs.size(), 0);
-            parallel_for(jobs.size(), [&](size_t k) { on_host[k] = host_chain(jobs[k], outs[k]) ? 1 : 0; });
-            std::vector<ChainJob> dev_jobs;
-            std::vector<size_t> dev_idx;
-            for (size_t k = 0; k < jobs.size(); ++k)
-                if (!on_host[k]) {
-                    dev_jobs.push_back(jobs[k]);
-                    dev_idx.push_back(k);
-                }
-            if (!dev_jobs.empty()) {
-                std::vector<ChainOut> dev_outs(dev_jobs.size());
-                be.run_chains(dev_jobs.data(), dev_outs.data(), (int)dev_jobs.size());
-                for (size_t k = 0; k < dev_idx.size(); ++k) outs[dev_idx[k]] = std::move(dev_outs[k]);
-            }
-        }
-        auto t_fin = std::chrono::steady_clock::now();
-        for (size_t k = 0; k < jobs.size(); ++k)
-            if (outs[k].unknown_method_hit) {
-                Candidate &c = cands[owners[k].cand];
-                throw std::runtime_error("Unknown method: " + (owners[k].what == 2 ? c.method1 : c.method0));
-            }
         std::vector<StageResult> sols(jobs.size());
         std::vector<std::vector<int64_t>> first_op(jobs.size());
-        parallel_for(jobs.size(), [&](size_t k) { sols[k] = finalize_prepare(jobs[k], outs[k], first_op[k]); });
+        std::vector<std::exception_ptr> fin_err(jobs.size());
         size_t chunk_from = 4096;
         int chunks_per_chain = 16;
         if (const char *e = std::getenv("DA4ML_HIP_TREE_THREADS")) {
             chunks_per_chain = std::max(1, std::atoi(e)) * 4;
             chunk_from = 0;
         }
-        struct Piece {
-            int chain, j0, j1;
+        double trees_ms = 0;
+        auto finalize = [&](const std::vector<size_t> &ks) {
+            const auto t0 = std::chrono::steady_clock::now();
+            parallel_for(ks.size(), [&](size_t q) {
+                const size_t k = ks[q];
+                fin_err[k] = nullptr;
+                recycle_op_list(std::move(sols[k].ops));
+                sols[k] = StageResult{};
+                if (outs[k].unknown_method_hit) return;
+                try {
+                    sols[k] = finalize_prepare(jobs[k], outs[k], first_op[k]);
+                } catch (...) {
+                    fin_err[k] = std::current_exception();
+                }
+            });
+            struct Piece {
+                int chain, j0, j1;
+            };
+            std::vector<Piece> pieces;
+            for (size_t k : ks) {
+                if (fin_err[k] || outs[k].unknown_method_hit) continue;
+                const int n_out = jobs[k].n_out;
+                const int parts = outs[k].dig_row.size() >= chunk_from ? std::max(1, std::min(n_out, chunks_per_chain)) : 1;
+                for (int c = 0; c < parts; ++c)
+                    pieces.push_back(Piece{(int)k, (int)((long long)n_out * c / parts), (int)((long long)n_out * (c + 1) / parts)});
+            }
+            std::mutex err_mu;
+            parallel_for(pieces.size(), [&](size_t i) {
+                const Piece &pc = pieces[i];
+                try {
+                    finalize_columns(jobs[pc.chain], outs[pc.chain], sols[pc.chain], first_op[pc.chain], pc.j0, pc.j1);
+                } catch (...) {
+                    std::lock_guard<std::mutex> lk(err_mu);
+                    if (!fin_err[pc.chain]) fin_err[pc.chain] = std::current_exception();
+                }
+            });
+            trees_ms += std::chrono::duration<double, std::milli>(std::chrono::steady_clock::now() - t0).count();
         };
-        std::vector<Piece> pieces;
-        for (size_t k = 0; k < jobs.size(); ++k) {
-            const int n_out = jobs[k].n_out;
-            const int parts = outs[k].dig_row.size() >= chunk_from ? std::max(1, std::min(n_out, chunks_per_chain)) : 1;
-            for (int c = 0; c < parts; ++c)
-                pieces.push_back(Piece{(int)k, (int)((long long)n_out * c / parts), (int)((long long)n_out * (c + 1) / parts)});
-        }
-        parallel_for(pieces.size(), [&](size_t i) {
-            const Piece &pc = pieces[i];
-            finalize_columns(jobs[pc.chain], outs[pc.chain], sols[pc.chain], first_op[pc.chain], pc.j0, pc.j1);
-        });
+        {
+            std::vector<uint8_t> on_host(jobs.size(), 0);
+            parallel_for(jobs.size(), [&](size_t k) { on_host[k] = host_chain(jobs[k], outs[k]) ? 1 : 0; });
+            std::vector<ChainJob> dev_jobs;
+            std::vector<size_t> dev_idx, host_idx;
+            for (size_t k = 0; k < jobs.size(); ++k)
+                if (!on_host[k]) {
+                    dev_jobs.push_back(jobs[k]);
+                    dev_idx.push_back(k);
+                } else
+                    host_idx.push_back(k);
+            if (!dev_jobs.empty()) {
+                std::vector<ChainOut> dev_outs(dev_jobs.size());
+                be.run_chains_streamed(dev_jobs.data(), dev_outs.data(), (int)dev_jobs.size(), [&](int first, int count) {
+                    std::vector<size_t> ks;
+                    for (int k = first; k < first + count; ++k) {
+                        outs[dev_idx[k]] = std::move(dev_outs[k]);
+                        ks.push_back(dev_idx[k]);
+                    }
+                    try {
+                        finalize(ks);
+                    } catch (...) {
+                        for (size_t k : ks)
+                            if (!fin_err[k]) fin_err[k] = std::current_exception();
+                    }
+                });
+            }
+            finalize(host_idx);
+        }
+        for (size_t k = 0; k < jobs.size(); ++k)
+            if (outs[k].unknown_method_hit) {
+                Candidate &c = cands[owners[k].cand];
+                throw std::runtime_error("Unknown method: " + (owners[k].what == 2 ? c.method1 : c.method0));
+            }
+        for (size_t k = 0; k < jobs.size(); ++k)
+            if (fin_err[k]) std::rethrow_exception(fin_err[k]);
         if (std::getenv("DA4ML_HIP_VERBOSE"))
-            std::fprintf(stderr, "[da4ml_hip] round of %zu chains: run_chains %.2f ms, adder trees %.2f ms\n", jobs.size(),
-                         std::chrono::duration<double, std::milli>(t_fin - t_rc).count(),
-                         std::chrono::duration<double, std::milli>(std::chrono::steady_clock::now() - t_fin).count());
+            std::fprintf(stderr, "[da4ml_hip] round of %zu chains: chains + adder trees %.2f ms, of which adder trees %.2f ms\n", jobs.size(),
+                         std::chrono::duration<double, std::milli>(std::chrono::steady_clock::now() - t_rc).count(), trees_ms);
         lap("chains + adder trees");
         for (size_t k = 0; k < jobs.size(); ++k) {
             Candidate &c = cands[owners[k].cand];
diff --git a/da4ml_amd/csrc/cmvm_host.h b/da4ml_amd/csrc/cmvm_host.h
--- a/da4ml_amd/csrc/cmvm_host.h
+++ b/da4ml_amd/csrc/cmvm_host.h
@@ -1,6 +1,7 @@
 #pragma once
 
 #include <cstdint>
+#include <functional>
 #include <stdexcept>
 #include <string>
 #include <vector>
@@ -57,6 +58,11 @@
   public:
     virtual ~Backend() = default;
     virtual void run_chains(const ChainJob *jobs, ChainOut *outs, int n) = 0;
+    using ReadyFn = std::function<void(int first, int count)>;
+    virtual void run_chains_streamed(const ChainJob *jobs, ChainOut *outs, int n, const ReadyFn &on_ready) {
+        run_chains(jobs, outs, n);
+        if (on_ready && n > 0) on_ready(0, n);
+    }
     virtual void column_distances(const int32_t *aug, int n_in, int W, int64_t *d0, int64_t *d1) = 0;
     virtual int csd_decompose(const float *kernel, int n_in, int n_out, bool center, std::vector<int8_t> &csd,
                               std::vector<int8_t> &s0, std::vector<int8_t> &s1) = 0;
@@ -77,6 +83,8 @@
 QInt qint_add(const QInt &a, const QInt &b, int64_t shift, bool neg_a, bool neg_b);
 void cost_add(const QInt &a, const QInt &b, int64_t shift, bool sub, int adder_size, int carry_size, float &dlat,
               float &cost);
+
+void host_parallel_for(size_t n, const std::function<void(size_t)> &fn);
 
 Log2Table measure_log2_table();
 struct StepLog2Host {
```

Result: no change. 112.3 solves/s (-0.7%).
